# apache/datafusion-comet

Hardware: NVIDIA H100
Metric: rows/sec on TPC-H Q1 filter+agg (higher is better)
Workload: dtype i128

## Files before the change

### datafusion-comet_b200/comet_b200/native.py

```python
import ctypes as C
import os

import pyarrow as pa

_PKG = os.path.dirname(os.path.dirname(os.path.abspath(__file__)))
_LIB_PATH = os.path.join(_PKG, "libcomet_b200.so")
_lib = None


class CometB200Error(RuntimeError):
    def __init__(self, code, error_class, message):
        super().__init__(f"[{code}{' ' + error_class if error_class else ''}] {message}")
        self.code, self.error_class, self.message = code, error_class, message


class Unsupported(CometB200Error):
    """The plan is outside the GPU hot path; a caller keeps its CPU path (CB200_ERR_UNSUPPORTED)."""


class _Error(C.Structure):
    _fields_ = [("code", C.c_int32), ("error_class", C.c_char * 64), ("message", C.c_char * 952)]


class ArrowSchema(C.Structure):
    pass


class ArrowArray(C.Structure):
    pass


ArrowSchema._fields_ = [("format", C.c_char_p), ("name", C.c_char_p), ("metadata", C.c_char_p), ("flags", C.c_int64),
                        ("n_children", C.c_int64), ("children", C.POINTER(C.POINTER(ArrowSchema))),
                        ("dictionary", C.POINTER(ArrowSchema)), ("release", C.c_void_p), ("private_data", C.c_void_p)]
ArrowArray._fields_ = [("length", C.c_int64), ("null_count", C.c_int64), ("offset", C.c_int64), ("n_buffers", C.c_int64),
                       ("n_children", C.c_int64), ("buffers", C.POINTER(C.c_void_p)),
                       ("children", C.POINTER(C.POINTER(ArrowArray))), ("dictionary", C.POINTER(ArrowArray)),
                       ("release", C.c_void_p), ("private_data", C.c_void_p)]


class ArrowArrayStream(C.Structure):
    _fields_ = [("get_schema", C.c_void_p), ("get_next", C.c_void_p), ("get_last_error", C.c_void_p),
                ("release", C.c_void_p), ("private_data", C.c_void_p)]


class DeviceColumn(C.Structure):
    _fields_ = [("type_id", C.c_int32), ("precision", C.c_int32), ("scale", C.c_int32), ("value_width", C.c_int32),
                ("values", C.c_void_p), ("validity", C.c_void_p), ("host_values", C.c_void_p),
                ("host_validity_bytes", C.c_void_p), ("validity_bytes", C.c_void_p), ("bool_bytes", C.c_void_p),
                ("n_dict", C.c_int32), ("pad", C.c_int32)]


class Stats(C.Structure):
    _fields_ = [("kernel_launches", C.c_int64), ("pipeline_launches", C.c_int64), ("pipeline_ms", C.c_double),
                ("pipeline_rows", C.c_int64), ("h2d_bytes", C.c_int64), ("d2h_bytes", C.c_int64),
                ("scan_pruned_row_groups", C.c_int64), ("scan_pruned_rows", C.c_int64), ("agg_strategies", C.c_int64)]
AGG_DENSE, AGG_TABLE, AGG_STREAM, AGG_MIGRATED = 1, 2, 4, 8


EXPORTED = ["cb200_comm_unique_id", "cb200_comm_create", "cb200_comm_destroy", "cb200_comm_rank", "cb200_comm_world", "cb200_nccl_info", "cb200_exchange",
            "cb200_exchange_layout", "cb200_comm_allgather_small", "cb200_plan_stats", "cb200_register_memory_file", "cb200_parquet_describe", "cb200_table_add_column_bytes", "cb200_plan_dict_value", "cb200_plan_partition_starts", "cb200_compile_plan_assume", "cb200_version", "cb200_supports", "cb200_create_plan", "cb200_plan_num_columns", "cb200_execute",
            "cb200_release", "cb200_table_create", "cb200_table_add_column", "cb200_plan_bind_table",
            "cb200_table_release", "cb200_execute_device", "cb200_plan_kernel_launches", "cb200_compile_plan",
            "cb200_plan_kernel_source"]


def lib():
    global _lib
    if _lib is None:
        if not os.path.exists(_LIB_PATH):
            raise ImportError(f"{_LIB_PATH} is missing: build it with `python -c 'import __graft_entry__ as g; g.build()'` "
                              "(make -C datafusion-comet_b200/csrc).  comet_b200 has no CPU fallback.")
        l = C.CDLL(_LIB_PATH)
        l.cb200_version.restype = C.c_char_p
        l.cb200_supports.argtypes = [C.c_char_p, C.c_size_t, C.POINTER(_Error)]
        l.cb200_create_plan.restype = C.c_void_p
        l.cb200_create_plan.argtypes = [C.c_char_p, C.c_size_t, C.c_char_p, C.c_size_t, C.POINTER(C.c_void_p), C.c_int32,
                                        C.c_int32, C.c_int32, C.c_int32, C.c_int32, C.POINTER(_Error)]
        l.cb200_plan_num_columns.argtypes = [C.c_void_p]
        l.cb200_execute.restype = C.c_int64
        l.cb200_execute.argtypes = [C.c_void_p, C.POINTER(ArrowArray), C.POINTER(ArrowSchema), C.c_int32, C.POINTER(_Error)]
        l.cb200_release.argtypes = [C.c_void_p]
        l.cb200_table_create.restype = C.c_void_p
        l.cb200_table_create.argtypes = [C.c_int64]
        l.cb200_table_add_column.argtypes = [C.c_void_p, C.c_int32, C.c_int32, C.c_int32, C.c_int32, C.c_void_p, C.c_void_p,
                                             C.c_int64, C.POINTER(C.c_char_p), C.c_int32, C.POINTER(_Error)]
        l.cb200_plan_bind_table.argtypes = [C.c_void_p, C.c_int32, C.c_void_p, C.POINTER(_Error)]
        l.cb200_table_release.argtypes = [C.c_void_p]
        l.cb200_execute_device.restype = C.c_int64
        l.cb200_execute_device.argtypes = [C.c_void_p, C.POINTER(DeviceColumn), C.c_int32, C.POINTER(_Error)]
        l.cb200_plan_kernel_launches.restype = C.c_int64
        l.cb200_plan_kernel_launches.argtypes = [C.c_void_p]
        l.cb200_plan_stats.argtypes = [C.c_void_p, C.POINTER(Stats)]
        l.cb200_compile_plan.argtypes = [C.c_char_p, C.c_size_t, C.c_char_p, C.c_size_t, C.POINTER(_Error)]
        l.cb200_plan_kernel_source.argtypes = [C.c_char_p, C.c_size_t, C.c_int32, C.c_char_p, C.c_size_t, C.POINTER(_Error)]
        _lib = l
    return _lib


def _raise(err):
    cls = Unsupported if err.code == 1 else CometB200Error
    raise cls(err.code, err.error_class.decode(), err.message.decode(errors="replace"))


def version():
    return lib().cb200_version().decode()


def supports(op_bytes):
    err = _Error()
    ok = lib().cb200_supports(op_bytes, len(op_bytes), C.byref(err))
    return bool(ok), err.message.decode(errors="replace")


def compile_plan(op_bytes):
    err = _Error()
    buf = C.create_string_buffer(4096)
    n = lib().cb200_compile_plan(op_bytes, len(op_bytes), buf, 4096, C.byref(err))
    if n < 0:
        _raise(err)
    return [k for k in buf.value.decode().split(",") if k]


def compile_plan_assume(op_bytes, assume_bits, source_index=-1):
    err = _Error()
    arr = (C.c_int32 * len(assume_bits))(*assume_bits)
    cap = 1 << 20
    buf = C.create_string_buffer(cap)
    lib().cb200_compile_plan_assume.argtypes = [C.c_char_p, C.c_size_t, C.POINTER(C.c_int32), C.c_int32, C.c_int32, C.c_char_p, C.c_size_t, C.POINTER(_Error)]
    n = lib().cb200_compile_plan_assume(op_bytes, len(op_bytes), arr, len(assume_bits), source_index, buf, cap, C.byref(err))
    if n < 0:
        _raise(err)
    return buf.value.decode()


_MEMFILES = {}


def register_memory_file(name, buf):
# ... 288 lines not shown
```

### datafusion-comet_b200/csrc/abi.cpp

```cpp
#include "../../include/comet_b200.h"

#include "abi_internal.h"
#include "parquet_kernels.h"
#include "exec.h"
#include "jit.h"
#include "plan.h"
#include "proto_wire.h"

#include <cstring>
#include <functional>
#include <map>
#include <mutex>

using namespace cb200;

namespace {

struct CtxRes {
    cudaStream_t stream;
    int* d_err;
    int* h_err;
    cudaEvent_t ev0, ev1;
};
std::mutex g_pool_mu;
std::map<int, std::vector<CtxRes>> g_pool;

void parse_config(const uint8_t* cfg, size_t len, ExecContext& ctx) {
    if (!cfg || !len) return;
    PbReader r(cfg, len);
    while (r.next()) {
        if (r.field != 1 || r.wire != 2) { r.skip(); continue; }
        PbReader e = r.sub();
        std::string k, v;
        while (e.next()) {
            if (e.field == 1) k = e.bytes();
            else if (e.field == 2) v = e.bytes();
            else e.skip();
        }
        if (k == "spark.comet.b200.chunkRows") ctx.chunk_rows = std::max<int64_t>(1024, atoll(v.c_str()));
        else if (k == "spark.comet.batchSize") ctx.batch_size = atoi(v.c_str());
        else if (k == "spark.comet.b200.streamAgg.minRows") ctx.stream_agg_min_rows = atoll(v.c_str());
        else if (k == "spark.comet.b200.streamAgg.maxRatio") ctx.stream_agg_max_ratio = atof(v.c_str());
        else if (k == "spark.comet.b200.hashThreads") { int t = atoi(v.c_str()); if (t == 256 || t == 512 || t == 768 || t == 960) ctx.hash_threads = t; }
    }
}

void start(cb200_plan* p) {
    if (p->started) return;
    TraceSpan ts("plan.start");
    ExecContext& ctx = p->ctx;
    cuda_check(cudaSetDevice(ctx.device), "cudaSetDevice");
    {
        struct DevInfo { int major = 0, minor = 0, sms = 0; bool known = false; };
        static DevInfo info[64];
        static std::mutex info_mu;
        std::lock_guard<std::mutex> lk(info_mu);
        if (ctx.device < 0 || ctx.device >= 64) throw ExecError(CB200_ERR_CUDA, "", "device ordinal out of range");
        DevInfo& di = info[ctx.device];
        if (!di.known) {
            cuda_check(cudaDeviceGetAttribute(&di.major, cudaDevAttrComputeCapabilityMajor, ctx.device), "cudaDeviceGetAttribute");
            cuda_check(cudaDeviceGetAttribute(&di.minor, cudaDevAttrComputeCapabilityMinor, ctx.device), "cudaDeviceGetAttribute");
            cuda_check(cudaDeviceGetAttribute(&di.sms, cudaDevAttrMultiProcessorCount, ctx.device), "cudaDeviceGetAttribute");
            di.known = true;
        }
        if (di.major != 9 || di.minor != 0) throw ExecError(CB200_ERR_CUDA, "", "comet_b200 kernels are built for sm_90a; device is sm_" + std::to_string(di.major * 10 + di.minor));
        ctx.num_sms = di.sms;
    }
    {
        std::lock_guard<std::mutex> lk(g_pool_mu);
        auto& fl = g_pool[ctx.device];
        if (!fl.empty()) {
            CtxRes r = fl.back();
            fl.pop_back();
            ctx.stream = r.stream; ctx.d_err = r.d_err; ctx.h_err = r.h_err; ctx.ev0 = r.ev0; ctx.ev1 = r.ev1;
        }
    }
    if (!ctx.stream) {
        cuda_check(cudaStreamCreateWithFlags(&ctx.stream, cudaStreamNonBlocking), "cudaStreamCreate");
        cudaMemPool_t pool;
        if (cudaDeviceGetDefaultMemPool(&pool, ctx.device) == cudaSuccess) {
            unsigned long long keep = ~0ull;
            cudaMemPoolSetAttribute(pool, cudaMemPoolAttrReleaseThreshold, &keep);
        }
        cuda_check(cudaMalloc((void**)&ctx.d_err, 64), "cudaMalloc err");
        cuda_check(cudaMallocHost((void**)&ctx.h_err, 64), "cudaMallocHost err");
        cuda_check(cudaEventCreate(&ctx.ev0), "cudaEventCreate");
        cuda_check(cudaEventCreate(&ctx.ev1), "cudaEventCreate");
    }
    cuda_check(cudaMemsetAsync(ctx.d_err, 0, 64, ctx.stream), "memset err");
    set_alloc_stream(ctx.stream);
    p->root = build_exec(p->op, &ctx, &p->inputs);
    p->started = true;
}

DType dtype_from_ids(int type_id, int precision, int scale) {
    if (type_id < 0 || type_id > 13) throw Unsupported("type id " + std::to_string(type_id));
    DType d;
    d.id = (TypeId)type_id;
    d.precision = precision;
    d.scale = scale;
    return d;
}

}

extern "C" {

const char* cb200_version(void) { return "comet_b200 0.1.0 (sm_90a; reference apache/datafusion-comet 1.1.0 @2699f59b)"; }

int cb200_supports(const uint8_t* op_proto, size_t op_len, cb200_error* why) {
    return cb200_guarded(why, [&]() -> int {
        OperatorP op = decode_plan(op_proto, op_len);
        plan_kernels_for_build(op);
        return 1;
    }, 0);
}

cb200_plan* cb200_create_plan(const uint8_t* op_proto, size_t op_len, const uint8_t* cfg_proto, size_t cfg_len, struct ArrowArrayStream** inputs,
                              int32_t n_inputs, int32_t partition, int32_t partition_count, int32_t batch_size, int32_t device_ordinal, cb200_error* err) {
    TraceSpan ts("create_plan");
    return cb200_guarded(err, [&]() -> cb200_plan* {
        auto p = std::unique_ptr<cb200_plan>(new cb200_plan());
        p->op = decode_plan(op_proto, op_len);
        p->ctx.device = device_ordinal;
        if (batch_size > 0) p->ctx.batch_size = batch_size;
        parse_config(cfg_proto, cfg_len, p->ctx);
        p->partition = partition;
        p->partition_count = partition_count;
        for (int i = 0; i < n_inputs; i++) {
            p->inputs.streams.push_back(inputs ? inputs[i] : nullptr);
            p->inputs.tables.push_back(nullptr);
        }
        return p.release();
    }, (cb200_plan*)nullptr);
}

int32_t cb200_plan_num_columns(cb200_plan* plan) { return plan ? (int32_t)plan->op->schema.size() : -1; }

static int64_t execute_common(cb200_plan* plan, cb200_error* err, const std::function<void(Batch&)>& sink) {
    TraceSpan ts("execute");
    return cb200_guarded(err, [&]() -> int64_t {
        if (!plan) throw PlanError("null plan handle");
        if (plan->finished) return -1;
        start(plan);
        cuda_check(cudaSetDevice(plan->ctx.device), "cudaSetDevice");
        set_alloc_stream(plan->ctx.stream);
        Batch b;
        if (!plan->root->next(b)) { plan->finished = true; return -1; }
        plan->last = std::move(b);
        sink(plan->last);
        return plan->last.n_rows;
    }, (int64_t)-2);
}

int64_t cb200_execute(cb200_plan* plan, struct ArrowArray* out_arrays, struct ArrowSchema* out_schemas, int32_t n_cols, cb200_error* err) {
    if (plan && plan->export_pending) {
        TraceSpan ts("execute(slice)");
        return cb200_guarded(err, [&]() -> int64_t {
            cuda_check(cudaSetDevice(plan->ctx.device), "cudaSetDevice");
            set_alloc_stream(plan->ctx.stream);
            const int64_t n = std::min<int64_t>(std::max(plan->ctx.batch_size, 1), plan->last.n_rows - plan->export_pos);
            export_batch(plan->last, &plan->ctx, out_arrays, out_schemas, n_cols, plan->export_pos, n);
            plan->export_pos += n;
            plan->export_pending = plan->export_pos < plan->last.n_rows;
            return n;
        }, (int64_t)-2);
    }
    int64_t first = 0;
    const int64_t rc = execute_common(plan, err, [&](Batch& b) {
        const bool whole = plan->op->kind == OpKind::ShuffleWriter;
        first = whole ? b.n_rows : std::min<int64_t>(std::max(plan->ctx.batch_size, 1), b.n_rows);
        export_batch(b, &plan->ctx, out_arrays, out_schemas, n_cols, 0, first);
        plan->export_pos = first;
        plan->export_pending = first < b.n_rows;
    });
    return rc < 0 ? rc : first;
}

int64_t cb200_execute_device(cb200_plan* plan, cb200_device_column* cols, int32_t n_cols, cb200_error* err) {
    if (plan && plan->export_pending)
        return cb200_guarded(err, [&]() -> int64_t { throw PlanError("cb200_execute_device: the current batch is still being handed out by cb200_execute"); }, (int64_t)-2);
    return execute_common(plan, err, [&](Batch& b) {
        if ((int)b.cols.size() != n_cols) throw PlanError("execute_device: plan produces " + std::to_string(b.cols.size()) + " columns");
        for (int i = 0; i < n_cols; i++) {
            Column& c = b.cols[(size_t)i];
            cb200_device_column& o = cols[i];
            memset(&o, 0, sizeof(o));
            o.type_id = (int)c.type.id;
            o.precision = c.type.precision;
            o.scale = c.type.scale;
            o.value_width = c.type.id == TypeId::Bool ? 1 : c.type.arrow_width();
            if (c.on_host) {
                o.host_values = c.h_data.data();
                o.host_validity_bytes = c.h_valid.empty() ? nullptr : c.h_valid.data();
            } else {
                o.values = c.data ? c.data->ptr : nullptr;
                o.validity = c.validity ? c.validity->ptr : nullptr;
                o.validity_bytes = c.valid_bytes ? c.valid_bytes->ptr : nullptr;
                o.bool_bytes = c.bool_bytes ? c.bool_bytes->ptr : nullptr;
                if (c.is_dict) { o.n_dict = (int)c.dict->values.size(); o.value_width = phys_bytes(c.phys == Phys::I32 ? Phys::Dict32 : c.phys); }
            }
        }
    });
}

void cb200_release(cb200_plan* plan) {
    if (!plan) return;
    TraceSpan ts("release");
    try {
        if (plan->started) cudaSetDevice(plan->ctx.device);
        plan->last = Batch();
        plan->root.reset();
        if (plan->ctx.stream) {
            cudaStreamSynchronize(plan->ctx.stream);
            std::lock_guard<std::mutex> lk(g_pool_mu);
            g_pool[plan->ctx.device].push_back(CtxRes{plan->ctx.stream, plan->ctx.d_err, plan->ctx.h_err, plan->ctx.ev0, plan->ctx.ev1});
        }
        for (auto* s : plan->inputs.streams) if (s && s->release) s->release(s);
    } catch (...) {
    }
    delete plan;
}

cb200_table* cb200_table_create(int64_t n_rows) {
    auto* t = new cb200_table();
    t->t = std::make_shared<DeviceTable>();
    t->t->n_rows = n_rows;
    return t;
}

int cb200_table_add_column(cb200_table* t, int32_t type_id, int32_t precision, int32_t scale, int32_t value_width, const void* dev_values,
                           const void* dev_validity, int64_t null_count, const char* const* dict_values, int32_t n_dict, cb200_error* err) {
    return cb200_guarded(err, [&]() -> int {
        if (!t) throw PlanError("null table handle");
        Column c;
        c.type = dtype_from_ids(type_id, precision, scale);
        size_t n = (size_t)t->t->n_rows;
        if (n_dict > 0) {
            if (!c.type.is_string()) throw PlanError("dictionary values on a non-string column");
            c.is_dict = true;
            c.dict = std::make_shared<Dictionary>();
            for (int i = 0; i < n_dict; i++) c.dict->values.push_back(dict_values[i]);
            c.phys = value_width == 1 ? Phys::I8 : value_width == 2 ? Phys::I16 : Phys::I32;
            if (value_width != 1 && value_width != 2 && value_width != 4) throw PlanError("dictionary codes must be 1, 2 or 4 bytes wide");
        } else if (c.type.is_string()) {
            throw Unsupported("device string columns must be dictionary-encoded");
        } else if (c.type.is_decimal() && value_width == 8) {
            if (c.type.precision > 18) throw PlanError("8-byte decimals need precision <= 18");
            c.phys = Phys::I64;
        } else {
            int w = c.type.arrow_width();
            if (value_width != w) throw PlanError("value_width " + std::to_string(value_width) + " does not match " + c.type.str());
            switch (c.type.id) {
            case TypeId::Bool: c.phys = Phys::Bitmap; break;
            case TypeId::Int8: c.phys = Phys::I8; break;
            case TypeId::Int16: c.phys = Phys::I16; break;
            case TypeId::Int32: case TypeId::Date: c.phys = Phys::I32; break;
            case TypeId::Float32: c.phys = Phys::F32; break;
            case TypeId::Float64: c.phys = Phys::F64; break;
            case TypeId::Decimal: c.phys = Phys::I128; break;
            default: c.phys = Phys::I64; break;
            }
        }
        if (((uintptr_t)dev_values & 15) || ((uintptr_t)dev_validity & 15)) throw PlanError("device buffers must be 16-byte aligned");
        size_t bytes = value_width == 0 ? (n + 7) / 8 : n * (size_t)value_width;
        c.data = std::make_shared<DeviceBuf>((void*)dev_values, bytes);
        if (dev_validity && null_count != 0) c.validity = std::make_shared<DeviceBuf>((void*)dev_validity, (n + 7) / 8);
        c.null_count = null_count;
        t->t->cols.push_back(c);
        return 0;
    }, -1);
}

const char* cb200_plan_dict_value(cb200_plan* plan, int32_t col, int32_t i, int32_t* len) {
    if (!plan || col < 0 || col >= (int)plan->last.cols.size()) return nullptr;
    const Column& c = plan->last.cols[(size_t)col];
    if (!c.is_dict || !c.dict || i < 0 || i >= (int)c.dict->values.size()) return nullptr;
    if (len) *len = (int32_t)c.dict->values[(size_t)i].size();
    return c.dict->values[(size_t)i].data();
}

int cb200_table_add_column_bytes(cb200_table* t, int32_t type_id, int32_t precision, int32_t scale, int32_t value_width, const void* dev_values,
                                 const void* dev_validity_bytes, const char* const* dict_values, int32_t n_dict, cb200_error* err) {
    return cb200_guarded(err, [&]() -> int {
        if (!t) throw PlanError("null table handle");
        size_t n = (size_t)t->t->n_rows;
        bool is_bool = type_id == (int)TypeId::Bool;
        int rc = cb200_table_add_column(t, type_id, precision, scale, is_bool ? 0 : value_width, is_bool ? nullptr : dev_values, nullptr, 0, dict_values, n_dict, err);
        if (rc != 0) throw PlanError(err ? err->message : "add_column failed");
        Column& c = t->t->cols.back();
        if (is_bool) {
            if (value_width != 1) throw PlanError("byte-per-row booleans need value_width 1");
            c.data = nullptr;
            c.bool_bytes = std::make_shared<DeviceBuf>((void*)dev_values, n);
            t->t->needs_packing = true;
        }
        if (dev_validity_bytes) {
            c.valid_bytes = std::make_shared<DeviceBuf>((void*)dev_validity_bytes, n);
            c.null_count = -1;
            t->t->needs_packing = true;
        }
        return 0;
    }, -1);
}

int cb200_plan_bind_table(cb200_plan* plan, int32_t input_index, cb200_table* t, cb200_error* err) {
    return cb200_guarded(err, [&]() -> int {
        if (!plan || !t) throw PlanError("null handle");
        if (plan->started) throw PlanError("tables must be bound before the first execute");
        if (input_index < 0 || input_index >= (int)plan->inputs.tables.size()) throw PlanError("input index out of range");
        plan->inputs.tables[(size_t)input_index] = t->t;
        return 0;
    }, -1);
}

void cb200_table_release(cb200_table* t) { delete t; }

int32_t cb200_plan_partition_starts(cb200_plan* plan, int64_t* starts, int32_t cap) {
    if (!plan) return -1;
    const auto& ps = plan->ctx.partition_starts;
    for (size_t i = 0; i < ps.size() && (int32_t)i < cap; i++) starts[i] = ps[i];
    return (int32_t)ps.size();
}

int64_t cb200_plan_kernel_launches(cb200_plan* plan) { return plan ? plan->ctx.kernel_launches : -1; }

int64_t cb200_release_cached_memory(int32_t device_ordinal) {
    try {
        if (cudaSetDevice(device_ordinal) != cudaSuccess) return 0;
        return (int64_t)release_cached_device_memory();
    } catch (...) { return 0; }
}

int cb200_plan_stats(cb200_plan* plan, cb200_stats* out) {
    if (!plan || !out) return -1;
    const ExecContext& c = plan->ctx;
    out->kernel_launches = c.kernel_launches;
    out->pipeline_launches = c.pipeline_launches;
    out->pipeline_ms = c.pipeline_ms;
    out->pipeline_rows = c.pipeline_rows;
    out->h2d_bytes = c.h2d_bytes;
    out->d2h_bytes = c.d2h_bytes;
    out->scan_pruned_row_groups = c.scan_pruned_row_groups;
    out->scan_pruned_rows = c.scan_pruned_rows;
    out->agg_strategies = c.agg_strategies;
    return 0;
}

int cb200_compile_plan(const uint8_t* op_proto, size_t op_len, char* keys_out, size_t keys_cap, cb200_error* err) {
    return cb200_guarded(err, [&]() -> int {
        OperatorP op = decode_plan(op_proto, op_len);
        auto ks = plan_kernels_for_build(op);
        std::string keys;
        for (auto& g : ks) {
            jit_get(g, false);
            keys += (keys.empty() ? "" : ",") + g.key;
        }
        if (keys_out && keys_cap) snprintf(keys_out, keys_cap, "%s", keys.c_str());
        return (int)ks.size();
    }, -1);
}

int cb200_compile_plan_assume(const uint8_t* op_proto, size_t op_len, const int32_t* assume_bits, int32_t n_assume, int32_t source_index,
                              char* src_out, size_t src_cap, cb200_error* err) {
    return cb200_guarded(err, [&]() -> int {
        OperatorP op = decode_plan(op_proto, op_len);
        std::vector<int> as(assume_bits, assume_bits + n_assume);
        auto ks = plan_kernels_for_build(op, as);
        for (auto& g : ks) jit_get(g, false);
        if (src_out && src_cap && source_index >= 0 && source_index < (int)ks.size()) snprintf(src_out, src_cap, "%s", ks[(size_t)source_index].source.c_str());
        return (int)ks.size();
    }, -1);
}

int cb200_register_memory_file(const char* name, const void* data, size_t len) {
    if (!name) return -1;
    register_memory_file(name, (const uint8_t*)data, len);
    return 0;
}

int64_t cb200_snappy_decompress(const uint8_t* comp, size_t comp_len, uint8_t* out, size_t uncompressed_len, int32_t device_ordinal, int32_t* path_taken,
                                cb200_error* err) {
    return cb200_guarded(err, [&]() -> int64_t {
        if (!comp || (!out && uncompressed_len) || comp_len >= ((size_t)1 << 31) || uncompressed_len >= ((size_t)1 << 31)) throw PlanError("cb200_snappy_decompress: bad arguments");
        cuda_check(cudaSetDevice(device_ordinal), "cudaSetDevice");
        cudaStream_t st = nullptr;
        set_alloc_stream(st);
        DeviceBuf dcomp(comp_len + 64), dout(uncompressed_len + 64), dpage(sizeof(PqPage)), derr(64);
        const int n_segs = (int)((uncompressed_len + PQ_SNAPPY_SEG - 1) / PQ_SNAPPY_SEG);
        DeviceBuf dck((size_t)(n_segs + 1) * 4);
        PqPage pg;
        memset(&pg, 0, sizeof(pg));
        pg.body = (unsigned char*)dout.ptr;
        pg.body_bytes = (int)uncompressed_len;
        pg.comp = (const unsigned char*)dcomp.ptr;
        pg.comp_bytes = (int)comp_len;
        pg.seg_base = 0;
        pg.n_segs = n_segs;
        cuda_check(cudaMemsetAsync(dcomp.ptr, 0, comp_len + 64, st), "memset");
        cuda_check(cudaMemcpyAsync(dcomp.ptr, comp, comp_len, cudaMemcpyHostToDevice, st), "copy in");
        cuda_check(cudaMemcpyAsync(dpage.ptr, &pg, sizeof(pg), cudaMemcpyHostToDevice, st), "copy page");
        cuda_check(cudaMemsetAsync(derr.ptr, 0, 64, st), "memset err");
        launch_pq_snappy_segmented((PqPage*)dpage.ptr, 1, (unsigned*)dck.ptr, n_segs, (int*)derr.ptr, st);
        int e = 0;
        cuda_check(cudaMemcpyAsync(&e, derr.ptr, 4, cudaMemcpyDeviceToHost, st), "read err");
        cuda_check(cudaMemcpyAsync(&pg, dpage.ptr, sizeof(pg), cudaMemcpyDeviceToHost, st), "read page");
        if (uncompressed_len) cuda_check(cudaMemcpyAsync(out, dout.ptr, uncompressed_len, cudaMemcpyDeviceToHost, st), "copy out");
        cuda_check(cudaStreamSynchronize(st), "sync");
        if (path_taken) *path_taken = (pg.flags & PQ_PAGE_SN_SERIAL) ? 1 : 0;
        if (e) throw ExecError(14, "", "malformed Snappy stream (device error flags " + std::to_string(e) + ")");
        return (int64_t)uncompressed_len;
    }, (int64_t)-1);
}

int cb200_parquet_describe(const char* path, char* out, size_t cap, cb200_error* err) {
    return cb200_guarded(err, [&]() -> int {
        std::string s = describe_parquet(path ? path : "");
        if (out && cap) snprintf(out, cap, "%s", s.c_str());
        return (int)s.size();
    }, -1);
}

int cb200_plan_kernel_source(const uint8_t* op_proto, size_t op_len, int32_t index, char* out, size_t cap, cb200_error* err) {
    return cb200_guarded(err, [&]() -> int {
        OperatorP op = decode_plan(op_proto, op_len);
        auto ks = plan_kernels_for_build(op);
        if (index < 0 || index >= (int)ks.size()) throw PlanError("kernel index out of range");
        const std::string& s = ks[(size_t)index].source;
// ... 7 lines not shown
```

### datafusion-comet_b200/csrc/agg.cpp

```cpp
#include "exec_internal.h"
#include "../../include/comet_b200.h"

#include "aot_kernels.h"
#include "ranges.h"

#include <algorithm>
#include <mutex>

namespace cb200 {

static std::mutex g_profile_mu;
static std::map<std::string, std::vector<int>> g_range_profile;

namespace {

enum class Strategy { Undecided, Dense, Table, Stream };
enum Level { SAFE = 0, TYPE = 1, TIGHT = 2 };
constexpr int DENSE_MAX_GROUPS = 64;

constexpr int GK = CB_GID_RANGES;
struct HashFlags { int w[CB_HFLAG_WORDS]; };
int64_t round_ids(int64_t n) { return (n + GK - 1) / GK * GK; }

using ValueMasks = uint64_t[CB_MAX_COLS * 2];

uint64_t identity_word(int kind) { return kind == W_MIN ? 0x7fffffffffffffffull : kind == W_MAX ? 0x8000000000000000ull : 0; }

std::vector<int> decode_gid(int g, const std::vector<int>& cards) {
    std::vector<int> code(cards.size());
    for (int k = (int)cards.size() - 1; k >= 0; k--) { code[(size_t)k] = g % cards[(size_t)k]; g /= cards[(size_t)k]; }
    return code;
}

int grid_for(const ExecContext* ctx, int n_tiles) { return std::max(1, std::min(ctx->num_sms, n_tiles)); }

struct Kernel {
    PipelineSpec spec;
    GeneratedKernel g;
    std::shared_ptr<CompiledModule> mod;
};

void launch_named(ExecContext* ctx, const Kernel& k, const char* name, dim3 grid, dim3 block, void** args) {
    cuda_check(cudaLaunchKernel((const void*)k.mod->kernel(name), grid, block, args, 0, ctx->stream), name);
    ctx->kernel_launches++;
}

struct DenseState {
    std::vector<int> cards;
    std::vector<bool> has_null;
    DeviceBufP totals, spill, partials;
    int groups = 0;

    void regroup(ExecContext* ctx, int n_words, const std::vector<int>& word_kinds, const std::vector<int>& new_cards) {
        int new_groups = 1;
        for (int c : new_cards) new_groups *= c;
        std::vector<uint64_t> oldt((size_t)groups * n_words * 2), newt((size_t)new_groups * n_words * 2);
        cuda_check(cudaMemcpy(oldt.data(), totals->ptr, oldt.size() * 8, cudaMemcpyDeviceToHost), "regroup D2H");
        for (size_t i = 0; i < (size_t)new_groups * n_words; i++) newt[i * 2] = identity_word(word_kinds[i % (size_t)n_words]);
        for (int g = 0; g < groups; g++) {
            const std::vector<int> code = decode_gid(g, cards);
            int ng = 0, mul = 1;
            for (int k = (int)cards.size() - 1; k >= 0; k--) {
                int cd = code[(size_t)k];
                if (has_null[(size_t)k] && cd == cards[(size_t)k] - 1) cd = new_cards[(size_t)k] - 1;
                ng += cd * mul;
                mul *= new_cards[(size_t)k];
            }
            memcpy(&newt[(size_t)ng * n_words * 2], &oldt[(size_t)g * n_words * 2], (size_t)n_words * 16);
        }
        totals = std::make_shared<DeviceBuf>(newt.size() * 8);
        cuda_check(cudaMemcpyAsync(totals->ptr, newt.data(), newt.size() * 8, cudaMemcpyHostToDevice, ctx->stream), "regroup H2D");
        cuda_check(cudaStreamSynchronize(ctx->stream), "regroup sync");
        groups = new_groups;
    }

    void finalize(ExecContext* ctx, const Kernel& last, cb::FinParams fp, bool ungrouped, const std::vector<DType>& schema,
                  const std::vector<DictionaryP>& key_dicts, Batch& out) const {
        TraceSpan ts("agg.finalize");
        const GeneratedKernel& g = last.g;
        const int ng = groups;
        fp.totals = (cb::u64*)totals->ptr;
        fp.n_groups = ng;
        std::vector<size_t> off_v, off_n;
        size_t total_bytes = 0;
        auto take = [&](size_t n) { size_t o = total_bytes; total_bytes += (n + 15) / 16 * 16; return o; };
        for (size_t i = 0; i < g.out_cols.size(); i++) { off_v.push_back(take((size_t)ng * g.out_bytes[i])); off_n.push_back(take((size_t)ng)); }
        size_t off_present = take((size_t)ng);
        auto dbuf = std::make_shared<DeviceBuf>(total_bytes);
        for (size_t i = 0; i < g.out_cols.size(); i++) {
            fp.out[i] = (cb::u8*)dbuf->ptr + off_v[i];
            fp.outv[i] = (cb::u8*)dbuf->ptr + off_n[i];
        }
        fp.present = (cb::u8*)dbuf->ptr + off_present;
        void* args[] = {&fp};
        cuda_check(cudaLaunchKernel((const void*)last.mod->kernel(g.finalize_entry), dim3((ng + 127) / 128), dim3(128), args, 0, ctx->stream), "finalize launch");
        ctx->kernel_launches++;
        std::vector<uint8_t> hbuf(total_bytes);
        cuda_check(cudaMemcpyAsync(hbuf.data(), dbuf->ptr, total_bytes, cudaMemcpyDeviceToHost, ctx->stream), "agg results D2H"); ctx->d2h_bytes += (int64_t)(total_bytes);
        ctx->check_device_errors();
        const uint8_t* pres = hbuf.data() + off_present;
        std::vector<int> rows;
        for (int gi = 0; gi < ng; gi++) if (ungrouped || pres[(size_t)gi]) rows.push_back(gi);
        out.n_rows = (int64_t)rows.size();
        out.cols.clear();
        for (size_t k = 0; k < key_dicts.size(); k++) {
            Column c;
            c.type = schema[k];
            c.on_host = true;
            bool any_null = false;
            std::vector<int> codes;
            for (int gi : rows) codes.push_back(decode_gid(gi, cards)[k]);
            c.h_valid.assign(rows.size(), 1);
            const bool is_bool = c.type.id == TypeId::Bool;
            if (!is_bool) c.h_offsets.push_back(0);
            for (size_t r = 0; r < rows.size(); r++) {
                const bool isnull = has_null[k] && codes[r] == cards[k] - 1;
                if (isnull) { c.h_valid[r] = 0; any_null = true; }
                if (is_bool) c.h_data.push_back(isnull ? 0 : (uint8_t)codes[r]);
                else {
                    if (!isnull) { const std::string& s = key_dicts[k]->values.at((size_t)codes[r]); c.h_data.insert(c.h_data.end(), s.begin(), s.end()); }
                    c.h_offsets.push_back((int32_t)c.h_data.size());
                }
            }
            if (!any_null) c.h_valid.clear();
            out.cols.push_back(c);
        }
        for (size_t i = 0; i < g.out_cols.size(); i++) {
            Column c;
            c.type = g.out_cols[i].type;
            c.on_host = true;
            int w = g.out_bytes[i];
            const uint8_t* all = hbuf.data() + off_v[i];
            const uint8_t* allv = hbuf.data() + off_n[i];
            c.h_data.resize(rows.size() * w);
            c.h_valid.resize(rows.size());
            bool any_null = false;
            for (size_t r = 0; r < rows.size(); r++) {
                memcpy(&c.h_data[r * w], &all[(size_t)rows[r] * w], (size_t)w);
                c.h_valid[r] = allv[(size_t)rows[r]];
                if (!c.h_valid[r]) any_null = true;
            }
            if (!any_null) c.h_valid.clear();
            out.cols.push_back(c);
        }
    }
};

struct IdRows {
    DeviceBufP hkey_of_gid, htotals, hflags;
    int64_t max_groups = 0;

    void ensure_flags(ExecContext* ctx) {
        if (hflags) return;
        hflags = std::make_shared<DeviceBuf>(sizeof(HashFlags));
        cuda_check(cudaMemsetAsync(hflags->ptr, 0, sizeof(HashFlags), ctx->stream), "memset hash flags");
    }
    void write_flags(ExecContext* ctx, const HashFlags& hf) {
        cuda_check(cudaMemcpyAsync(hflags->ptr, &hf, sizeof(hf), cudaMemcpyHostToDevice, ctx->stream), "write hash flags");
        cuda_check(cudaStreamSynchronize(ctx->stream), "flags sync");
    }
    int64_t read_flags(ExecContext* ctx, HashFlags& hf, int64_t cnt[GK]) {
        memset(&hf, 0, sizeof(hf));
        if (hflags) {
            cuda_check(cudaMemcpyAsync(&hf, hflags->ptr, sizeof(hf), cudaMemcpyDeviceToHost, ctx->stream), "read hash flags"); ctx->d2h_bytes += (int64_t)sizeof(hf);
            cuda_check(cudaStreamSynchronize(ctx->stream), "hash flags sync");
        }
        const int64_t R = max_groups / GK;
        int64_t total = 0;
        bool overshoot = false;
        for (int r = 0; r < GK; r++) {
            if (hf.w[CB_HFLAG_CTR + r] > R || hf.w[CB_HFLAG_CTR + r] < 0) overshoot = true;
            cnt[r] = std::min<int64_t>(std::max(hf.w[CB_HFLAG_CTR + r], 0), R);
            if (hf.w[CB_HFLAG_CTR + r] < 0) cnt[r] = R;
            total += cnt[r];
        }
        if (overshoot && hflags) {
            for (int r = 0; r < GK; r++) hf.w[CB_HFLAG_CTR + r] = (int)cnt[r];
            write_flags(ctx, hf);
        }
        return total;
    }
    static void init_totals(ExecContext* ctx, const Kernel& k, cb::u64* totals, int64_t first, int64_t n) {
        if (n <= 0) return;
        const int n_words = k.g.n_words;
        if (std::none_of(k.g.word_kinds.begin(), k.g.word_kinds.end(), identity_word)) {
            cuda_check(cudaMemsetAsync(totals + first * n_words * 2, 0, (size_t)n * n_words * 16, ctx->stream), "memset totals");
        } else {
            long long f = first, nn = n;
            void* a1[] = {&totals, &f, &nn};
            launch_named(ctx, k, "cb_hash_init", dim3((unsigned)((n + 255) / 256)), dim3(256), a1);
        }
    }
    void grow(ExecContext* ctx, const Kernel& k, const int64_t cnt[GK], int64_t nm, bool zero_fill) {
        cudaStream_t st = ctx->stream;
        const int n_words = k.g.n_words, key_words = k.g.key_words;
        if (nm + 2 >= INT32_MAX) throw ExecError(16, "", "more than 2^31 groups in one partition; lower spark.comet.b200.chunkRows");
        const int64_t Ro = max_groups / GK, Rn = nm / GK;
        auto ntot = std::make_shared<DeviceBuf>((size_t)(nm + 2) * n_words * 16);
        auto nkog = std::make_shared<DeviceBuf>((size_t)nm * 8 * key_words + 16);
        cb::u64* tp = (cb::u64*)ntot->ptr;
        if (zero_fill) init_totals(ctx, k, tp, 0, nm + 2);
        else if (!htotals) init_totals(ctx, k, tp, nm, 2);
        if (htotals) {
            for (int r = 0; r < GK; r++) {
                if (cnt[r] <= 0) continue;
                cuda_check(cudaMemcpyAsync(tp + (size_t)r * Rn * n_words * 2, (cb::u64*)htotals->ptr + (size_t)r * Ro * n_words * 2, (size_t)cnt[r] * n_words * 16,
                                           cudaMemcpyDeviceToDevice, st), "copy totals");
                cuda_check(cudaMemcpyAsync((cb::u64*)nkog->ptr + (size_t)r * Rn * key_words, (cb::u64*)hkey_of_gid->ptr + (size_t)r * Ro * key_words,
                                           (size_t)cnt[r] * 8 * key_words, cudaMemcpyDeviceToDevice, st), "copy group keys");
            }
            cuda_check(cudaMemcpyAsync(tp + (size_t)nm * n_words * 2, (cb::u64*)htotals->ptr + (size_t)max_groups * n_words * 2, (size_t)2 * n_words * 16,
                                       cudaMemcpyDeviceToDevice, st), "copy reserved groups");
        }
        cuda_check(cudaStreamSynchronize(st), "table growth");
        htotals = ntot; hkey_of_gid = nkog; max_groups = nm;
    }

    void finalize(ExecContext* ctx, const Kernel& last, cb::FinParams fp, const std::vector<DictionaryP>& key_dicts, Batch& out) {
        TraceSpan ts("agg.finalize_hash");
        const GeneratedKernel& g = last.g;
        HashFlags hfl;
        int64_t cnt[GK];
        const int64_t ng = read_flags(ctx, hfl, cnt);
        const int* flags = hfl.w;
        const int64_t n_out = ng + ((flags[0] & CB_HF_SENTINEL) ? 1 : 0) + ((flags[0] & CB_HF_NULL_GROUP) ? 1 : 0);
        fp.totals = (cb::u64*)htotals->ptr;
        fp.hkeys = (const cb::u64*)hkey_of_gid->ptr;
        fp.sentinel_used = flags[0] & CB_HF_SENTINEL;
        fp.null_group_used = (flags[0] & CB_HF_NULL_GROUP) ? 1 : 0;
        fp.n_hash_groups = (int)ng;
        fp.max_groups = (int)max_groups;
        fp.gid_range = (int)(max_groups / GK);
        int64_t run = 0;
        for (int r = 0; r < GK; r++) { fp.gid_prefix[r] = (int)run; run += cnt[r]; }
        fp.gid_prefix[GK] = (int)run;
        fp.n_groups = (int)n_out;
        if (g.out_cols.size() > CB_MAX_OUT) throw Unsupported("too many output columns");
        out.n_rows = n_out;
        out.cols.clear();
        std::vector<DeviceBufP> vbytes;
        size_t rows_alloc = (size_t)std::max<int64_t>(n_out, 1);
        for (size_t i = 0; i < g.out_cols.size(); i++) {
            Column c;
            c.type = g.out_cols[i].type;
            c.phys = c.type.id == TypeId::Bool ? Phys::I8 : (c.type.is_string() ? Phys::I32 : phys_of(c.type));
            c.data = std::make_shared<DeviceBuf>(rows_alloc * g.out_bytes[i]);
            vbytes.push_back(std::make_shared<DeviceBuf>(rows_alloc));
            fp.out[i] = (cb::u8*)c.data->ptr;
            fp.outv[i] = (cb::u8*)vbytes.back()->ptr;
            if ((int)i < g.n_key_cols && c.type.is_string()) { c.is_dict = true; c.dict = key_dicts[i]; }
            out.cols.push_back(c);
        }
        auto present = std::make_shared<DeviceBuf>(rows_alloc);
        fp.present = (cb::u8*)present->ptr;
        if (n_out > 0) {
            void* args[] = {&fp};
            launch_named(ctx, last, g.finalize_entry.c_str(), dim3((unsigned)((n_out + 127) / 128)), dim3(128), args);
            for (size_t i = 0; i < out.cols.size(); i++) {
                Column& c = out.cols[i];
                c.valid_bytes = vbytes[i];
                c.validity = std::make_shared<DeviceBuf>((size_t)(n_out + 31) / 32 * 4 + 8);
                launch_bytes_to_bitmap((const unsigned char*)vbytes[i]->ptr, n_out, (uint32_t*)c.validity->ptr, ctx->stream);
                ctx->kernel_launches++;
                c.null_count = -1;
                if (c.type.id == TypeId::Bool) c.bool_bytes = c.data;
            }
        }
        ctx->check_device_errors();
    }
};

struct KeyTable {
    DeviceBufP hkeys;
    int64_t hcap = 0;

    void ensure(ExecContext* ctx, const Kernel& k, IdRows& rows, int64_t incoming, int64_t remaining, int64_t rows_scanned, bool merging) {
        cudaStream_t st = ctx->stream;
        rows.ensure_flags(ctx);
        HashFlags hf;
        int64_t cnt[GK];
        const int64_t cur = rows.read_flags(ctx, hf, cnt);
        const int64_t need = cur + incoming;
        if (need + 2 >= INT32_MAX) throw ExecError(16, "", "more than 2^31 groups in one partition; lower spark.comet.b200.chunkRows");
        bool relocated = false;
        if (need > rows.max_groups) {
            int64_t nm = std::max<int64_t>(need, rows.max_groups + rows.max_groups / 4);
            if (remaining > 0 && rows_scanned == 0 && merging) {
                nm = std::max(nm, need + remaining);
            }
            if (remaining > 0 && rows_scanned > 0 && cur > 0) {
                const double ratio = std::min(1.0, 1.3 * (double)cur / (double)rows_scanned);
                const int64_t est = cur + incoming + (int64_t)(ratio * (double)remaining);
                nm = std::max(nm, std::min<int64_t>(est, cur + incoming + remaining));
            }
            if (nm + 2 + GK >= INT32_MAX) nm = INT32_MAX - 3 - GK;
            relocated = cur > 0;
            rows.grow(ctx, k, cnt, round_ids(nm), true);
        }
        int64_t cap = std::max<int64_t>(hcap, 1 << 16);
        while (cap < 2 * std::max(need, rows.max_groups)) cap <<= 1;
        if (cap != hcap || relocated) {
            auto nkeys = cap != hcap ? std::make_shared<DeviceBuf>((size_t)cap * 16) : hkeys;
            cuda_check(cudaMemsetAsync(nkeys->ptr, 0xff, (size_t)cap * 16, st), "memset key slots");
            if (cur > 0) {
                const cb::u64* kog = (const cb::u64*)rows.hkey_of_gid->ptr;
                int rr = (int)(rows.max_groups / GK);
                const int* ctr = (const int*)rows.hflags->ptr + CB_HFLAG_CTR;
                cb::u64* kp = (cb::u64*)nkeys->ptr;
                cb::u32 mask = (cb::u32)(cap - 1);
                void* a2[] = {&kog, &rr, &ctr, &kp, &mask};
                launch_named(ctx, k, "cb_hash_rehash", dim3((unsigned)((rows.max_groups + 255) / 256)), dim3(256), a2);
                cuda_check(cudaStreamSynchronize(st), "rehash");
            }
            hkeys = nkeys; hcap = cap;
        }
    }
};

struct StreamState {
    double ratio = 1.0;
    DeviceBufP reserved_snap;

    void ensure_rows(ExecContext* ctx, const Kernel& k, IdRows& rows, const int64_t cnt[GK], int64_t want_groups) {
        rows.ensure_flags(ctx);
        if (rows.htotals && want_groups <= rows.max_groups) return;
        rows.grow(ctx, k, cnt, round_ids(std::max<int64_t>(want_groups, rows.max_groups + rows.max_groups / 2)), false);
    }
    void snapshot_reserved(ExecContext* ctx, const IdRows& rows, int n_words, bool restore) {
        const size_t bytes = (size_t)2 * n_words * 16;
        if (!reserved_snap || reserved_snap->bytes < bytes) reserved_snap = std::make_shared<DeviceBuf>(bytes);
        cb::u64* tail = (cb::u64*)rows.htotals->ptr + (size_t)rows.max_groups * n_words * 2;
        if (restore) cuda_check(cudaMemcpyAsync(tail, reserved_snap->ptr, bytes, cudaMemcpyDeviceToDevice, ctx->stream), "restore reserved groups");
        else cuda_check(cudaMemcpyAsync(reserved_snap->ptr, tail, bytes, cudaMemcpyDeviceToDevice, ctx->stream), "snapshot reserved groups");
    }
};

struct AggNode : FusedBase {
    std::vector<ExprP> keys;
    std::vector<AggExpr> aggs;
    std::vector<std::vector<int>> state_cols;
    AggMode mode = AggMode::Partial;
    bool ungrouped = false;
    bool emitted = false;
    std::vector<Batch> outq;
    size_t outq_pos = 0;
    std::vector<int> assume_bits;

    std::vector<bool> key_has_null;
    std::vector<DictionaryP> key_dicts;
    struct DevDict { StringDictDev d; std::vector<DeviceBufP> bufs; int host_known = 0; };
    std::vector<std::shared_ptr<DevDict>> dev_dicts;

    int n_words = 0, key_words = 1;
    std::vector<int> word_kinds;
    Kernel last;
    bool have_totals() const { return last.mod != nullptr; }

    Strategy strategy = Strategy::Undecided;
    DenseState dense;
    KeyTable table;
    IdRows rows;

    std::vector<int> observed_bits;
    int64_t rows_scanned = 0;
    std::string profile_key;
    DeviceBufP vmask;
    StreamState stream;

    int assume_for(int child_col, Level lv) const {
        const DType& t = child->schema[(size_t)child_col];
        if (!t.is_decimal() || lv == SAFE || mode != AggMode::Partial) return 0;
        int k = r_bitlen(r_prec_max(t.precision));
        if ((size_t)child_col < assume_bits.size() && assume_bits[(size_t)child_col] > 0) k = std::min(k, assume_bits[(size_t)child_col]);
        if (lv == TIGHT && !observed_bits.empty() && observed_bits[(size_t)child_col] >= 0) k = std::min(k, observed_bits[(size_t)child_col] + 2);
        return std::min(k, 126);
    }

    PipelineSpec make_spec(const Batch* b, Strategy st, int n_groups, Level lv = TYPE) const {
        const bool hash = st == Strategy::Table || st == Strategy::Stream;
        PipelineSpec s;
        s.cols = stage_cols(b);
        for (auto& c : s.cols) c.assume_bits = assume_for(c.src_index, lv);
        s.predicates = to_slots(predicates, slot_of);
        s.sink = SinkKind::Agg;
        s.mode = mode;
        s.ungrouped = ungrouped;
        s.hash = hash;
        s.keys = to_slots(keys, slot_of);
        for (size_t k = 0; k < keys.size(); k++) s.key_nullable.push_back(b ? key_has_null[k] : false);
        for (auto& a : aggs) {
            AggExpr c = a;
            if (mode == AggMode::Partial) {
                c.children = to_slots(a.children, slot_of);
                if (a.filter) c.filter = to_slots({a.filter}, slot_of)[0];
            }
            s.aggs.push_back(c);
        }
        for (auto& sc : state_cols) {
            std::vector<int> v;
            for (int ci : sc) v.push_back(slot_of.at(ci));
            s.state_slots.push_back(v);
        }
        if (hash) {
            s.threads = ctx->hash_threads;
            s.tile = 2 * ctx->hash_threads;
            s.stream = st == Strategy::Stream;
        }
        GeneratedKernel probe = generate_pipeline(s);
        size_t acc = (!ungrouped && !hash) ? (size_t)std::max(n_groups, 1) * probe.n_words * s.threads * 8 : 0;
        while (acc + 2 * (size_t)probe.stage_bytes + 1024 > SMEM_BUDGET && s.threads > 32) {
            s.threads /= 2;
            acc /= 2;
        }
        if (acc + 2 * (size_t)probe.stage_bytes + 1024 > SMEM_BUDGET)
            throw Unsupported("too many groups x aggregates for the thread-private accumulators of the dense path");
        s.stages = (int)std::max<size_t>(2, std::min<size_t>(6, (SMEM_BUDGET - 1024 - acc) / (size_t)probe.stage_bytes));
        return s;
    }

    std::vector<PipelineSpec> build_specs() const override {
        bool hash = false;
        for (auto& k : keys) if (!k->type.is_string() && k->type.id != TypeId::Bool) hash = true;
        std::vector<PipelineSpec> out{make_spec(nullptr, hash ? Strategy::Table : Strategy::Dense, ungrouped ? 1 : 6)};
        if (hash && mode == AggMode::Partial) out.push_back(make_spec(nullptr, Strategy::Stream, 6));
        return out;
    }

    Kernel compile(const PipelineSpec& spec) {
        Kernel k{spec, generate_pipeline(spec), nullptr};
        k.mod = jit_get(k.g, true);
        if (have_totals() && (k.g.n_words != n_words || k.g.word_kinds != word_kinds)) throw ExecError(15, "", "internal: accumulator layout changed between launches");
        if (have_totals() && k.g.key_words != key_words) throw ExecError(15, "", "internal: group key packing changed between launches");
        n_words = k.g.n_words;
        word_kinds = k.g.word_kinds;
        key_words = k.g.key_words;
        return k;
    }

    void clear_vmask() {
        if (!vmask) vmask = std::make_shared<DeviceBuf>(CB_MAX_COLS * 16);
        cuda_check(cudaMemsetAsync(vmask->ptr, 0, CB_MAX_COLS * 16, ctx->stream), "memset vmask");
    }
    void copy_vmask(ValueMasks& masks) {
        cuda_check(cudaMemcpyAsync(masks, vmask->ptr, sizeof(ValueMasks), cudaMemcpyDeviceToHost, ctx->stream), "read value masks"); ctx->d2h_bytes += (int64_t)(sizeof(ValueMasks));
    }
    static std::vector<int> mask_bits(const PipelineSpec& spec, const ValueMasks& masks) {
        std::vector<int> seen(spec.cols.size(), -1);
        for (size_t i = 0; i < spec.cols.size(); i++) {
            if (!spec.cols[i].type.is_decimal()) continue;
            uint64_t lo = masks[2 * i], hi = masks[2 * i + 1];
            seen[i] = hi ? 64 + r_bitlen(hi) : r_bitlen(lo);
        }
        return seen;
    }
    void observe(const std::vector<int>& seen) {
        for (size_t i = 0; i < seen.size(); i++)
            if (seen[i] >= 0) observed_bits[(size_t)used_cols[i]] = std::max(observed_bits[(size_t)used_cols[i]], seen[i]);
    }

    int prepare_key(Batch& b, size_t k) {
        int ci = keys[k]->index;
        Column& c = b.cols[ci];
        if (c.type.id == TypeId::Bool) return 2;
        if (!c.type.is_string()) return -1;
        if (c.is_dict) {
            key_dicts[k] = c.dict;
            return (int)c.dict->values.size();
        }
        if (!dev_dicts[k]) {
            auto dd = std::make_shared<DevDict>();
            const int64_t cap = 1 << 16;
            const int max_codes = 4096;
            const int64_t bytes_cap = 1 << 20;
            auto alloc = [&](size_t n) { auto bfr = std::make_shared<DeviceBuf>(n); cuda_check(cudaMemsetAsync(bfr->ptr, 0, bfr->bytes, ctx->stream), "memset dict"); dd->bufs.push_back(bfr); return bfr->ptr; };
            dd->d.tags = (unsigned long long*)alloc((size_t)cap * 8);
            dd->d.slot_code = (int*)alloc((size_t)cap * 4);
            dd->d.capacity = cap;
            dd->d.n_codes = (int*)alloc(64);
            dd->d.bytes_used = (unsigned long long*)((char*)dd->d.n_codes + 16);
            dd->d.err = (int*)((char*)dd->d.n_codes + 32);
            dd->d.max_codes = max_codes;
            dd->d.code_off = (long long*)alloc((size_t)max_codes * 8);
            dd->d.code_len = (int*)alloc((size_t)max_codes * 4);
            dd->d.bytes = (unsigned char*)alloc((size_t)bytes_cap);
            dd->d.bytes_cap = bytes_cap;
            dev_dicts[k] = dd;
            key_dicts[k] = std::make_shared<Dictionary>();
        }
        DevDict& dd = *dev_dicts[k];
        if (!c.offsets || !c.chars) throw Unsupported("string key column without offsets/chars buffers");
        auto row_slot = std::make_shared<DeviceBuf>((size_t)b.n_rows * 4);
        auto codes = std::make_shared<DeviceBuf>((size_t)b.n_rows * 4);
        launch_dict_encode(dd.d, (const int*)c.offsets->ptr, (const unsigned char*)c.chars->ptr, c.validity ? (const unsigned char*)c.validity->ptr : nullptr,
                           b.n_rows, (int*)row_slot->ptr, (int*)codes->ptr, ctx->stream);
        ctx->kernel_launches += 2;
        int hdr[12];
        cuda_check(cudaMemcpyAsync(hdr, dd.d.n_codes, sizeof(hdr), cudaMemcpyDeviceToHost, ctx->stream), "dict header");
        cuda_check(cudaStreamSynchronize(ctx->stream), "dict encode");
        int n_codes = hdr[0], derr = hdr[8];
        if (derr & CB_DICT_FULL) throw Unsupported("plain Utf8 group key with more distinct values than the device dictionary holds (dictionary-encode the column)");
        if (derr & CB_DICT_COLLISION) throw ExecError(14, "", "64-bit hash collision between distinct group key strings");
        if (n_codes > dd.host_known) {
            std::vector<long long> off((size_t)n_codes);
            std::vector<int> len((size_t)n_codes);
            cuda_check(cudaMemcpy(off.data(), dd.d.code_off, (size_t)n_codes * 8, cudaMemcpyDeviceToHost), "dict offsets");
            cuda_check(cudaMemcpy(len.data(), dd.d.code_len, (size_t)n_codes * 4, cudaMemcpyDeviceToHost), "dict lengths");
            for (int i = dd.host_known; i < n_codes; i++) {
                std::string s((size_t)len[(size_t)i], '\0');
                if (len[(size_t)i]) cuda_check(cudaMemcpy(&s[0], dd.d.bytes + off[(size_t)i], (size_t)len[(size_t)i], cudaMemcpyDeviceToHost), "dict bytes");
                key_dicts[k]->values.push_back(s);
            }
            dd.host_known = n_codes;
        }
        c.data = codes;
        c.phys = Phys::I32;
        c.is_dict = true;
        c.dict = key_dicts[k];
        return n_codes;
    }

    void consume(Batch& b) {
        std::vector<int> nc(keys.size());
        std::vector<bool> hn(keys.size());
        for (size_t k = 0; k < keys.size(); k++) {
            int card = prepare_key(b, k);
            const Column& c = b.cols[keys[k]->index];
            hn[k] = key_has_null[k] || c.validity != nullptr;
            nc[k] = card < 0 ? -1 : std::max(card, 1) + (hn[k] ? 1 : 0);
            if (!dense.cards.empty() && nc[k] >= 0) nc[k] = std::max(nc[k], dense.cards[k]);
        }
        bool densifiable = true;
        for (int c : nc) if (c < 0) densifiable = false;
        int n_groups = 1;
        if (densifiable) for (int c : nc) { n_groups *= c; if (n_groups > 1 << 20) break; }
        const bool needs_hash = !ungrouped && (!densifiable || n_groups > DENSE_MAX_GROUPS);
        key_has_null = hn;
        if (observed_bits.empty()) observed_bits.assign(child->schema.size(), -1);
        if (strategy == Strategy::Undecided || (strategy == Strategy::Dense && needs_hash)) {
            if (strategy == Strategy::Dense) {
                leave_dense();
                ctx->agg_strategies |= CB200_AGG_MIGRATED;
            }
            strategy = !needs_hash ? Strategy::Dense : sample_stream(b) ? Strategy::Stream : Strategy::Table;
            ctx->agg_strategies |= strategy == Strategy::Dense ? CB200_AGG_DENSE : strategy == Strategy::Stream ? CB200_AGG_STREAM : CB200_AGG_TABLE;
        }
        if (strategy == Strategy::Dense) consume_dense(b, nc, n_groups);
        else if (strategy == Strategy::Table) consume_table(b);
        else consume_stream(b);
    }

    void consume_dense(Batch& b, const std::vector<int>& nc, int n_groups) {
        if (have_totals() && nc != dense.cards) {
            if (n_words == 0) throw ExecError(15, "", "internal: regroup before layout");
            dense.regroup(ctx, n_words, word_kinds, nc);
        }
        dense.cards = nc;
        dense.has_null = key_has_null;
        const int64_t SAMPLE = 1 << 20;
        bool have_obs = false;
        for (int ci : used_cols) if (child->schema[(size_t)ci].is_decimal() && observed_bits[(size_t)ci] >= 0) have_obs = true;
        if (mode == AggMode::Partial && !have_obs && b.n_rows > 2 * SAMPLE) {
            profile_key = pipeline_signature(make_spec(&b, Strategy::Dense, n_groups, SAFE));
            std::lock_guard<std::mutex> lk(g_profile_mu);
            auto it = g_range_profile.find(profile_key);
            if (it != g_range_profile.end() && it->second.size() == observed_bits.size()) {
                observed_bits = it->second;
                for (int ci : used_cols) if (child->schema[(size_t)ci].is_decimal() && observed_bits[(size_t)ci] >= 0) have_obs = true;
            }
        }
        if (mode != AggMode::Partial) {
            run_range(b, 0, b.n_rows, n_groups, SAFE);
        } else if (!have_obs && b.n_rows > 2 * SAMPLE) {
            run_range(b, 0, SAMPLE, n_groups, TYPE);
            run_range(b, SAMPLE, b.n_rows, n_groups, TIGHT);
        } else {
            run_range(b, 0, b.n_rows, n_groups, have_obs ? TIGHT : TYPE);
        }
        if (!profile_key.empty()) {
            std::lock_guard<std::mutex> lk(g_profile_mu);
            if (g_range_profile.size() > 256) g_range_profile.clear();
            g_range_profile[profile_key] = observed_bits;
        }
    }

    void leave_dense() {
        if (mode == AggMode::Final) throw Unsupported("group cardinality grew past the dense path mid-stream in a Final aggregate");
        if (have_totals()) {
            Batch early;
            dense.finalize(ctx, last, certified_params(), ungrouped, schema, key_dicts, early);
            if (early.n_rows > 0) outq.push_back(std::move(early));
        }
        last = Kernel();
        dense = DenseState();
        n_words = 0; word_kinds.clear(); rows_scanned = 0;
    }

    void run_range(Batch& b, int64_t row0, int64_t row1, int n_groups, Level lv) {
        TraceSpan tsr("agg.run_range");
        while (true) {
            Kernel k;
            {
                TraceSpan ts("agg.codegen+jit");
                k = compile(make_spec(&b, Strategy::Dense, n_groups, lv));
            }
            const int64_t max_rows = (int64_t)ctx->num_sms * k.g.threads * (1ll << CB_RPT_LOG2) / 1024 * 1024;
            int64_t r0 = row0;
            while (r0 < row1 && launch_one(b, r0, std::min(row1, r0 + max_rows), n_groups, k)) r0 += max_rows;
            if (r0 >= row1) return;
            if (lv == SAFE) throw ExecError(15, "", "internal: value-mask validation failed without assumptions");
            lv = lv == TIGHT ? TYPE : SAFE;
            row0 = r0;
        }
    }

    bool launch_one(Batch& b, int64_t r0, int64_t r1, int n_groups, const Kernel& k) {
        cudaStream_t st = ctx->stream;
        size_t tot_bytes = (size_t)n_groups * n_words * 16;
        if (!have_totals()) {
            dense.totals = std::make_shared<DeviceBuf>(tot_bytes);
            dense.groups = n_groups;
        }
        if (!dense.spill || dense.spill->bytes < tot_bytes) {
            dense.spill = std::make_shared<DeviceBuf>(tot_bytes);
            cuda_check(cudaMemsetAsync(dense.spill->ptr, 0, dense.spill->bytes, st), "memset spill");
        }
        clear_vmask();
        cb::PipeParams p;
        fill_inputs(p, b, k.g.tile, r0, r1);
        int grid = grid_for(ctx, p.n_tiles);
        size_t part_bytes = (size_t)grid * tot_bytes;
        if (!dense.partials || dense.partials->bytes < part_bytes) dense.partials = std::make_shared<DeviceBuf>(part_bytes);
        p.n_groups = n_groups;
        for (size_t i = 0; i < dense.cards.size() && i < CB_MAX_KEYS; i++) p.key_card[i] = dense.cards[i];
        p.partials = (cb::u8*)dense.partials->ptr;
        p.spill = (cb::u64*)dense.spill->ptr;
        p.vmask = (cb::u64*)vmask->ptr;
        launch(k.mod->kernel(k.g.entry), dim3(grid), dim3(k.g.threads + 32), k.g.dyn_smem(n_groups), &p);
        ctx->pipeline_rows += r1 - r0;
        ValueMasks masks;
        copy_vmask(masks);
        ctx->check_device_errors();
        const std::vector<int> seen = mask_bits(k.spec, masks);
        bool ok = true;
        for (size_t i = 0; i < seen.size(); i++)
            if (k.spec.cols[i].assume_bits > 0 && seen[i] > k.spec.cols[i].assume_bits) ok = false;
        observe(seen);
        if (!ok) {
            cuda_check(cudaMemsetAsync(dense.spill->ptr, 0, dense.spill->bytes, st), "memset spill");
            return false;
        }
        rows_scanned += r1 - r0;
        cb::FinParams fp;
        memset(&fp, 0, sizeof(fp));
        fp.partials = (const cb::u64*)dense.partials->ptr;
        fp.spill = (cb::u64*)dense.spill->ptr;
        fp.totals = (cb::u64*)dense.totals->ptr;
        fp.n_ctas = grid;
        fp.n_groups = n_groups;
        fp.first = have_totals() ? 0 : 1;
        fp.err = ctx->d_err;
        int total_words = n_groups * n_words;
        void* args[] = {&fp};
        cuda_check(cudaLaunchKernel((const void*)k.mod->kernel("cb_fold"), dim3((total_words + 127) / 128), dim3(128), args, 0, st), "fold launch");
        ctx->kernel_launches++;
        last = k;
        return true;
    }

    void launch_id_rows(Batch& b, int64_t r0, int64_t r1, const Kernel& k, bool with_table) {
        clear_vmask();
        cb::PipeParams p;
        fill_inputs(p, b, k.g.tile, r0, r1);
        p.hkeys = with_table ? (cb::u64*)table.hkeys->ptr : nullptr;
        p.hkey_of_gid = (cb::u64*)rows.hkey_of_gid->ptr;
        p.htotals = (cb::u64*)rows.htotals->ptr;
        p.hmask = with_table ? (cb::u32)(table.hcap - 1) : 0;
        p.max_groups = (cb::i32)rows.max_groups;
        p.hflags = (cb::i32*)rows.hflags->ptr;
        p.vmask = (cb::u64*)vmask->ptr;
        p.n_groups = 2;
        launch(k.mod->kernel(k.g.entry), dim3(grid_for(ctx, p.n_tiles)), dim3(k.g.threads + 32), k.g.dyn_smem(0), &p);
    }

    void consume_table(Batch& b) {
        const Kernel k = compile(make_spec(&b, Strategy::Table, 2, SAFE));
        {
            TraceSpan ts("hash.ensure_table");
            table.ensure(ctx, k, rows, b.n_rows, child->rows_hint(), rows_scanned, mode != AggMode::Partial);
        }
        launch_id_rows(b, 0, b.n_rows, k, true);
        ctx->pipeline_rows += b.n_rows;
        ValueMasks masks;
        int flags[8];
        copy_vmask(masks);
        cuda_check(cudaMemcpyAsync(flags, rows.hflags->ptr, sizeof(flags), cudaMemcpyDeviceToHost, ctx->stream), "read hash flags"); ctx->d2h_bytes += (int64_t)(sizeof(flags));
        ctx->check_device_errors();
        if (flags[0] & CB_HF_FULL) throw ExecError(15, "", "internal: hash table full");
        if (flags[0] & CB_HF_WIDE_KEY) throw Unsupported("decimal(p > 18) group key whose value does not fit 64 bits");
        observe(mask_bits(k.spec, masks));
        rows_scanned += b.n_rows;
        last = k;
    }

    int64_t stream_launch(Batch& b, int64_t r0, int64_t r1, const Kernel& k, HashFlags& hf, int64_t cnt[GK]) {
        launch_id_rows(b, r0, r1, k, false);
        ValueMasks masks;
        copy_vmask(masks);
        ctx->check_device_errors();
        const int64_t total = rows.read_flags(ctx, hf, cnt);
        if (hf.w[0] & CB_HF_WIDE_KEY) throw Unsupported("decimal(p > 18) group key whose value does not fit 64 bits");
        if (!(hf.w[0] & CB_HF_FULL)) observe(mask_bits(k.spec, masks));
        return total;
    }
    bool sample_stream(Batch& b) {
        if (mode != AggMode::Partial || ctx->stream_agg_min_rows < 0) return false;
        if (b.n_rows + std::max<int64_t>(child->rows_hint(), 0) < ctx->stream_agg_min_rows || b.n_rows == 0) return false;
        const Kernel k = compile(make_spec(&b, Strategy::Stream, 2, SAFE));
        const int64_t sample = std::min<int64_t>(b.n_rows, 1 << 20);
        HashFlags hf;
        int64_t cnt[GK] = {0};
        stream.ensure_rows(ctx, k, rows, cnt, 2 * sample + 4096);
        const int64_t runs = stream_launch(b, 0, sample, k, hf, cnt);
        stream.ratio = (hf.w[0] & CB_HF_FULL) ? 1.0 : (double)runs / (double)sample;
        memset(&hf, 0, sizeof(hf));
        rows.write_flags(ctx, hf);
        IdRows::init_totals(ctx, k, (cb::u64*)rows.htotals->ptr, rows.max_groups, 2);
        if (stream.ratio <= ctx->stream_agg_max_ratio) return true;
        rows = IdRows();
        n_words = 0; word_kinds.clear();
        return false;
    }
    void consume_stream(Batch& b) {
        const Kernel k = compile(make_spec(&b, Strategy::Stream, 2, SAFE));
        HashFlags before, hf;
        int64_t cnt0[GK], cnt[GK];
        const int64_t cur = rows.read_flags(ctx, before, cnt0);
        const int64_t remaining = std::max<int64_t>(child->rows_hint(), 0);
        int64_t want = cur + std::min<int64_t>(b.n_rows, (int64_t)(1.25 * stream.ratio * (double)b.n_rows) + 65536);
        if (!rows.htotals || want > rows.max_groups) want += std::min<int64_t>(remaining, (int64_t)(1.25 * stream.ratio * (double)remaining));
        int64_t handed_out;
        while (true) {
            {
                TraceSpan ts("stream.ensure_rows");
                stream.ensure_rows(ctx, k, rows, cnt0, want);
            }
            stream.snapshot_reserved(ctx, rows, n_words, false);
            handed_out = stream_launch(b, 0, b.n_rows, k, hf, cnt);
            if (!(hf.w[0] & CB_HF_FULL)) break;
            stream.snapshot_reserved(ctx, rows, n_words, true);
            for (int r = 0; r < GK; r++) before.w[CB_HFLAG_CTR + r] = (int)cnt0[r];
            rows.write_flags(ctx, before);
            want = cur + b.n_rows + GK;
        }
        ctx->pipeline_rows += b.n_rows;
        if (b.n_rows > 0) stream.ratio = std::max(stream.ratio, (double)(handed_out - cur) / (double)b.n_rows);
        rows_scanned += b.n_rows;
        last = k;
    }

    u128r certificate(size_t ai) const {
        const AggExpr& a = aggs[ai];
        if (!(a.kind == AggKind::Sum || a.kind == AggKind::Avg) || !a.datatype.is_decimal()) return 0;
        std::vector<u128r> bounds(child->schema.size(), RSAT);
        for (size_t c = 0; c < bounds.size(); c++)
            if (child->schema[c].is_decimal() && !observed_bits.empty())
                bounds[c] = observed_bits[c] < 0 ? 0 : (observed_bits[c] >= 127 ? RSAT : (u128r)1 << observed_bits[c]);
        if (mode == AggMode::Partial) return expr_maxabs(*a.children[0], bounds);
        return bounds[(size_t)state_cols[ai][0]];
    }
    cb::FinParams certified_params() const {
        cb::FinParams fp;
        memset(&fp, 0, sizeof(fp));
        fp.err = ctx->d_err;
        for (size_t ai = 0; ai < aggs.size() && ai < CB_MAX_OUT; ai++) {
            const u128r b = certificate(ai);
            fp.cert_b[ai][0] = b >= RSAT ? ~0ull : (uint64_t)b;
            fp.cert_b[ai][1] = b >= RSAT ? ~0ull : (uint64_t)(b >> 64);
            const bool direct = mode != AggMode::Partial || aggs[ai].children[0]->kind == ExprKind::Bound;
            if (b < RSAT && b != 0 && direct) fp.cert_b[ai][1] |= 1ull << 63;
        }
        return fp;
    }

    bool next(Batch& out) override {
        if (!emitted) aggregate_input();
        if (outq_pos >= outq.size()) return false;
        out = std::move(outq[outq_pos++]);
        return true;
    }
    void aggregate_input() {
        if (keys.size() > CB_MAX_KEYS) throw Unsupported("more than 4 group keys");
        key_has_null.assign(keys.size(), false);
        key_dicts.assign(keys.size(), nullptr);
        dev_dicts.assign(keys.size(), nullptr);
        Batch in;
        while (child->next(in)) {
            if (in.n_rows == 0) continue;
            consume(in);
            ctx->check_device_errors();
        }
        emitted = true;
        if (!have_totals()) {
            if (!ungrouped) return;
            last = compile(make_spec(nullptr, Strategy::Dense, 1));
            std::vector<uint64_t> id((size_t)n_words * 2, 0);
            for (int w = 0; w < n_words; w++) id[(size_t)w * 2] = identity_word(word_kinds[(size_t)w]);
            dense.totals = std::make_shared<DeviceBuf>(id.size() * 8);
            cuda_check(cudaMemcpyAsync(dense.totals->ptr, id.data(), id.size() * 8, cudaMemcpyHostToDevice, ctx->stream), "identity totals");
            cuda_check(cudaStreamSynchronize(ctx->stream), "identity totals sync");
            dense.groups = 1;
        }
        Batch result;
        if (strategy == Strategy::Table || strategy == Strategy::Stream) rows.finalize(ctx, last, certified_params(), key_dicts, result);
        else dense.finalize(ctx, last, certified_params(), ungrouped, schema, key_dicts, result);
        outq.push_back(std::move(result));
    }
};

}

ExecNodeP make_agg_node(const OperatorP& agg_op, const ExecNodeP& src, const std::vector<ExprP>& preds, const std::vector<ExprP>& cols, ExecContext* ctx,
                        const std::vector<int>& assume_bits) {
    auto n = std::make_shared<AggNode>();
    n->ctx = ctx;
    n->child = src;
    n->schema = agg_op->schema;
    n->predicates = preds;
    n->mode = agg_op->mode;
    n->ungrouped = agg_op->grouping.empty();
    n->assume_bits = assume_bits;
    std::vector<ExprP> roots = preds;
    for (auto& gexp : agg_op->grouping) {
        ExprP k = substitute(gexp, cols);
        if (k->kind != ExprKind::Bound) throw Unsupported("computed group keys (only plain column keys are fused)");
        n->keys.push_back(k);
        roots.push_back(k);
    }
    size_t state_at = agg_op->grouping.size();
    for (auto& a : agg_op->aggs) {
        AggExpr c = a;
        if (agg_op->mode == AggMode::Partial) {
            for (auto& ch : c.children) { ch = substitute(ch, cols); roots.push_back(ch); }
            if (c.filter) { c.filter = substitute(c.filter, cols); roots.push_back(c.filter); }
        } else {
            std::vector<int> sc;
            for (size_t k = 0; k < agg_state_types(a).size(); k++) {
                ExprP e = cols.at(state_at++);
                if (e->kind != ExprKind::Bound) throw Unsupported("final aggregate over computed state columns");
                sc.push_back(e->index);
                roots.push_back(e);
            }
            n->state_cols.push_back(sc);
        }
        n->aggs.push_back(c);
    }
    n->assign_slots(roots);
    if (n->used_cols.empty()) {
        int best = -1, best_w = 1 << 30;
        for (size_t c = 0; c < src->schema.size(); c++) {
            const DType& t = src->schema[c];
            if (t.is_string()) continue;
            int w = std::max(1, phys_bytes(phys_of(t)));
            if (w < best_w) { best = (int)c; best_w = w; }
        }
        if (best < 0) throw Unsupported("COUNT(*) over a child with only string columns");
        n->used_cols.push_back(best);
        n->slot_of[best] = 0;
    }
    return n;
}

}
```

### datafusion-comet_b200/csrc/codegen.cpp

```cpp
#include "codegen.h"
#include <mutex>
#include "ranges.h"

#include <climits>
#include <cstring>
#include <functional>
#include <sstream>

namespace cb200 {

int phys_bytes(Phys p) {
    switch (p) {
    case Phys::Bitmap: return 0;
    case Phys::I8: return 1;
    case Phys::I16: return 2;
    case Phys::I32: case Phys::F32: case Phys::Dict32: return 4;
    case Phys::I64: case Phys::F64: return 8;
    case Phys::I128: return 16;
    }
    return 0;
}

size_t GeneratedKernel::dyn_smem(int n_groups) const {
    size_t s = (entry == "cb_pipeline_agg" ? 128 : 256) + (size_t)stages * stage_bytes;
// ... 702 lines not shown
    GeneratedKernel g = generate_pipeline_uncached(spec);
    std::lock_guard<std::mutex> lk(g_memo_mu);
    if (g_memo.size() > 4096) g_memo.clear();
    g_memo[sig] = g;
    return g;
}

namespace {
GeneratedKernel generate_pipeline_uncached(const PipelineSpec& spec) {
    GeneratedKernel g;
    g.threads = spec.threads;
    g.tile = spec.tile;
    g.stages = spec.stages;
    g.stage_bytes = stage_bytes_of(spec);
    if (spec.cols.empty()) throw Unsupported("pipeline without input columns");
    if (spec.cols.size() > 24) throw Unsupported("more than 24 staged input columns");

    Emitter em(spec);
    if (spec.sink == SinkKind::Agg && spec.hash) em.base_guard = "in_range";
    std::string keep = "true";
    for (auto& p : spec.predicates) {
        Val v = em.emit(*p);
        keep += " && " + (v.n.empty() ? v.v : "(!" + v.n + " && " + v.v + ")");
    }
    std::ostringstream tu;

    if (spec.sink == SinkKind::Count) {
        em.body << "    return " << keep << ";\n";
        if (spec.ltile <= 0 || spec.tile % spec.ltile) throw PlanError("count pass: stage tile must be a multiple of the logical tile");
        tu << header(spec, "#define CB_KERNEL_SELECT 1\n#define CB_SELECT_COUNT 1\n#define CB_NOUT 0\n#define CB_LTILE " + std::to_string(spec.ltile) + "\n");
        tu << "#include \"cb_kernels.cuh\"\nnamespace cb {\n";
        tu << "CB_D bool cb_row_keep(const Tile& t, int r, i64 grow, const PipeParams& p) {\n    (void)grow; (void)p;\n" << em.body.str() << "}\n} // namespace cb\n";
        g.entry = "cb_select_count";
    } else if (spec.sink == SinkKind::Select) {
        if (spec.outputs.size() > 16) throw Unsupported("more than 16 output columns");
        em.body << "    if (!(" << keep << ")) return false;\n";
        std::ostringstream defs;
        defs << "#define CB_KERNEL_SELECT 1\n#define CB_NOUT " << spec.outputs.size() << "\n#define CB_SEL_MASKED " << (spec.masked ? 1 : 0) << "\n";
        std::vector<Val> outs;
        for (size_t i = 0; i < spec.outputs.size(); i++) {
            Val v = em.emit(*spec.outputs[i]);
            if (v.type.is_string() && spec.outputs[i]->kind != ExprKind::Bound) throw Unsupported("string expressions in a fused projection");
            outs.push_back(v);
            em.body << "    " << to_slot(v, "o.v[" + std::to_string(i) + "]") << " o.valid[" << i << "] = "
                    << (v.n.empty() ? "true" : "!" + v.n) << ";\n";
            OutCol oc;
            oc.type = v.type;
            oc.nullable = v.nullable();
            g.out_cols.push_back(oc);
            g.out_bytes.push_back(v.type.is_string() ? 4 : out_width(v.type));
        }
        em.body << "    return true;\n";
        tu << header(spec, defs.str());
        tu << "constexpr __host__ __device__ int cb_out_bytes(int c) { return ";
        for (size_t i = 0; i < outs.size(); i++) tu << "c == " << i << " ? " << g.out_bytes[i] << " : ";
        tu << "0; }\n";
        tu << "constexpr __host__ __device__ bool cb_out_nullable(int c) { return ";
        for (size_t i = 0; i < outs.size(); i++) tu << "c == " << i << " ? " << (g.out_cols[i].nullable ? "true" : "false") << " : ";
        tu << "false; }\n";
        tu << "#include \"cb_kernels.cuh\"\nnamespace cb {\n";
        tu << "CB_D bool cb_row_select(const Tile& t, int r, i64 grow, const PipeParams& p, SelOut& o) {\n    (void)grow; (void)p;\n"
           << em.body.str() << "}\n} // namespace cb\n";
        g.entry = "cb_pipeline_select";
    } else {
        if (spec.hash) {
            em.body << "    const bool keep_ = in_range && (" << keep << ");\n";
            em.base_guard = "keep_";
        } else em.body << "    (void)in_range;\n    if (!(" << keep << ")) return;\n";
        SlotPlan slots;
        std::vector<AggLayout> layout(spec.aggs.size());
        const bool H = spec.hash;
        auto upd = [&](const std::string& op, const std::string& cond, int w, const std::string& val = "") {
            std::ostringstream o;
            const std::string ws = std::to_string(w);
            if (H) {
                if (op == "count") o << "acc.h_count(" << cond << ", " << ws << ");";
                else if (op == "wrap") o << "acc.h_add_wrap(" << cond << ", " << ws << ", " << val << ");";
                else if (op == "wide") o << "acc.h_add_i64_wide(" << cond << ", " << ws << ", " << val << ");";
                else if (op == "i128") o << "acc.h_add_i128(" << cond << ", " << ws << ", " << val << ");";
                else if (op == "f64") o << "acc.h_add_f64(" << cond << ", " << ws << ", " << val << ");";
                else if (op == "min") o << "acc.h_min(" << cond << ", " << ws << ", " << val << ");";
                else o << "acc.h_max(" << cond << ", " << ws << ", " << val << ");";
            } else {
                o << "if (" << cond << ") ";
                if (op == "count") o << "acc.add_i64_wrap(g, " << ws << ", 1);";
                else if (op == "wrap") o << "acc.add_i64_wrap(g, " << ws << ", " << val << ");";
                else if (op == "wide") o << "acc.add_i64_wide(g, " << ws << ", " << val << ");";
                else if (op == "i128") o << "acc.add_i128(g, " << ws << ", " << val << ");";
                else if (op == "f64") o << "acc.add_f64(g, " << ws << ", " << val << ");";
                else if (op == "min") o << "acc.min_i64(g, " << ws << ", " << val << ");";
                else o << "acc.max_i64(g, " << ws << ", " << val << ");";
            }
            em.body << "    " << o.str() << "\n";
        };
        auto absval = [&](const std::string& iv) { return "cb::i128_abs_of_i64(" + iv + ")"; };
        std::string gid = "0";
        std::string null_group_cond;
        std::ostringstream unpack;
        if (spec.hash) {
            struct KeyPlan { Val v; int bits; bool nullable; int word; };
            std::vector<KeyPlan> kp;
            int n_words_k = 1, used = 0;
            for (size_t k = 0; k < spec.keys.size(); k++) {
                KeyPlan q;
                q.v = em.emit(*spec.keys[k]);
                const DType& kt = spec.keys[k]->type;
                q.bits = key_bits(kt);
                q.nullable = true;
                if (q.bits == 0) throw Unsupported("group key of type " + kt.str() + " cannot be packed into 64-bit hash key words");
                if (q.bits == 64 && spec.keys.size() == 1) {
                    null_group_cond = q.v.n;
                    q.nullable = false;
                }
                int need = q.bits + (q.nullable ? 1 : 0);
                if (need > 64) {
                    if (used > 0) { n_words_k++; used = 0; }
                    q.word = n_words_k - 1;
                    used = 64;
                    kp.push_back(q);
                    continue;
                }
                if (used + need > 64) { n_words_k++; used = 0; }
                q.word = n_words_k - 1;
                used += need;
                kp.push_back(q);
            }
            std::vector<size_t> wide_nullable;
            for (size_t k = 0; k < kp.size(); k++) if (kp[k].nullable && kp[k].bits == 64) wide_nullable.push_back(k);
            int flags_word = -1;
            if (!wide_nullable.empty()) flags_word = n_words_k++;
            if (n_words_k > 4) throw Unsupported("group keys need more than 256 packed bits");
            g.key_words = n_words_k;
            std::vector<std::string> pk(n_words_k);
            for (int w = 0; w < n_words_k; w++) { pk[w] = em.fresh("pk"); em.body << "    cb::u64 " << pk[w] << " = 0;\n"; }
            std::vector<std::string> unpack_steps;
            for (size_t k = 0; k < kp.size(); k++) {
                const KeyPlan& q = kp[k];
                const Val& kv = q.v;
                const DType& kt = spec.keys[k]->type;
                const int bits = q.bits;
                const bool wide_null = q.nullable && bits == 64;
                const bool inline_null = q.nullable && !wide_null;
                const std::string& packed = pk[q.word];
                const std::string isn = kv.n.empty() ? "false" : kv.n;
                std::string raw;
                if (kt.is_decimal()) {
                    if (kv.narrow) raw = "(cb::u64)" + kv.v;
                    else {
                        const std::string valid = kv.n.empty() ? "" : " && !" + kv.n;
                        em.body << "    if (keep_" << valid << " && !cb::i128_fits_i64(" << kv.v << ")) atomicOr(p.hflags, 4);\n";
                        raw = kv.v + ".lo";
                    }
                } else if (kt.id == TypeId::Bool) raw = "(" + kv.v + " ? 1ull : 0ull)";
                else raw = "(cb::u64)(cb::i64)" + kv.v;
                std::string mask = bits == 64 ? "0xffffffffffffffffull" : u64lit((1ull << bits) - 1);
                if (q.nullable && !kv.n.empty()) raw = "(" + kv.n + " ? 0ull : " + raw + ")";
                if (bits == 64) em.body << "    " << packed << " = " << raw << ";\n";
                else em.body << "    " << packed << " = (" << packed << " << " << bits << ") | (" << raw << " & " << mask << ");\n";
                if (inline_null) em.body << "    " << packed << " = (" << packed << " << 1) | (" << isn << " ? 1ull : 0ull);\n";
                if (wide_null) em.body << "    " << pk[flags_word] << " = (" << pk[flags_word] << " << 1) | (" << isn << " ? 1ull : 0ull);\n";
                std::ostringstream u;
                std::string kc = std::to_string(k), kwv = "k" + std::to_string(q.word);
                u << "    {\n";
                if (inline_null) u << "      bool isnull = (" << kwv << " & 1ull) != 0; " << kwv << " >>= 1;\n";
                else if (wide_null) u << "      bool isnull = (k" << flags_word << " & 1ull) != 0; k" << flags_word << " >>= 1;\n";
                else u << "      bool isnull = null_group;\n";
                if (bits == 64) u << "      cb::u64 raw = " << kwv << "; " << kwv << " = 0;\n";
                else u << "      cb::u64 raw = " << kwv << " & " << mask << "; " << kwv << " >>= " << bits << ";\n";
                if (kt.is_decimal()) u << "      cb::fin_store_i128(fp, " << kc << ", g, cb::i128_from_i64((cb::i64)raw), !isnull);\n";
                else if (kt.id == TypeId::Bool) u << "      cb::fin_store_u8(fp, " << kc << ", g, (int)raw, !isnull);\n";
                else if (bits == 64) u << "      cb::fin_store_i64(fp, " << kc << ", g, (cb::i64)raw, !isnull);\n";
                else {
                    int w = kt.is_string() ? 4 : kt.arrow_width();
                    std::string sx = bits == 8 ? "(cb::i32)(signed char)raw" : bits == 16 ? "(cb::i32)(short)raw" : "(cb::i32)raw";
                    u << "      cb::fin_store_i32(fp, " << kc << ", g, " << sx << ", !isnull, " << w << ");\n";
                }
                u << "    }\n";
                unpack_steps.push_back(u.str());
            }
            for (int w = 0; w < n_words_k; w++) unpack << "    cb::u64 k" << w << " = kw[" << w << "]; (void)k" << w << ";\n";
            for (auto it = unpack_steps.rbegin(); it != unpack_steps.rend(); ++it) unpack << *it;
            {
                std::string arr = em.fresh("kw");
                em.body << "    cb::u64 " << arr << "[" << n_words_k << "] = {";
                for (int w = 0; w < n_words_k; w++) em.body << (w ? ", " : "") << pk[w];
                em.body << "};\n";
                if (!null_group_cond.empty()) em.body << "    if (keep_ && " << null_group_cond << ") atomicOr(p.hflags, 8);\n";
                em.body << "    acc.begin(keep_, " << arr << ", " << (null_group_cond.empty() ? "false" : null_group_cond) << ");\n";
            }
        } else if (!spec.ungrouped) {
            for (size_t k = 0; k < spec.keys.size(); k++) {
                Val kv = em.emit(*spec.keys[k]);
                std::string code = kv.type.id == TypeId::Bool && spec.cols[spec.keys[k]->index].phys == Phys::Bitmap ? "(" + kv.v + " ? 1 : 0)" : kv.v;
                if (kv.nullable()) code = "(" + kv.n + " ? p.key_card[" + std::to_string(k) + "] - 1 : " + code + ")";
                gid = "(" + gid + ") * p.key_card[" + std::to_string(k) + "] + " + code;
            }
        }
        if (!spec.hash) em.body << "    const int g = " << gid << ";\n";
        int w_rows = slots.add(W_WRAP64, "cnt|true");
        upd("count", "true", w_rows);

        for (size_t ai = 0; ai < spec.aggs.size(); ai++) {
            const AggExpr& a = spec.aggs[ai];
            AggLayout& L = layout[ai];
            if (spec.mode == AggMode::Partial) {
                std::string cond = "true";
                if (a.filter) {
                    Val f = em.emit(*a.filter);
                    cond = f.n.empty() ? f.v : "(!" + f.n + " && " + f.v + ")";
                }
                std::vector<Val> cv;
                for (auto& c : a.children) cv.push_back(em.emit(*c));
                for (auto& v : cv) if (v.nullable()) cond += " && !" + v.n;
                std::string condkey = cond;
                const Val& v = cv[0];
                std::string use = cond == "true" ? "true" : em.declb(cond);
                auto cnt_slot = [&]() {
                    std::string k = "cnt|" + condkey;
                    bool first = slots.dedup.count(std::to_string((int)W_WRAP64) + "|" + k) == 0;
                    int w = slots.add(W_WRAP64, k);
                    if (first) upd("count", use, w);
                    return w;
                };
                switch (a.kind) {
                case AggKind::Count:
                    L.w_cnt = cnt_slot();
                    break;
                case AggKind::Sum: case AggKind::Avg: {
                    bool dec = a.datatype.is_decimal();
                    bool f64 = !dec && (a.kind == AggKind::Avg || a.datatype.is_float());
                    L.w_cnt = cnt_slot();
                    if (dec) {
                        bool first = slots.dedup.count(std::to_string((int)W_SUM128) + "|sum|" + v.v + "|" + condkey) == 0;
                        L.w_sum = slots.add(W_SUM128, "sum|" + v.v + "|" + condkey);
                        if (first) {
                            u128r vb = em.bound_of(*a.children[0]);
                            if (spec.hash) upd(v.narrow ? "wide" : "i128", use, L.w_sum, v.v);
                            else if (v.narrow && vb < (R63 >> CB_RPT_LOG2)) upd("wrap", use, L.w_sum, v.v);
                            else if (v.narrow) upd("wide", use, L.w_sum, v.v);
                            else upd("i128", use, L.w_sum, v.v);
                        }
                    } else if (f64) {
                        L.is_f64_sum = true;
                        std::string dv = v.type.id == TypeId::Float64 ? v.v : "(double)" + v.v;
                        bool first = slots.dedup.count(std::to_string((int)W_DD_HI) + "|dd|" + dv + "|" + condkey) == 0;
                        L.w_sum = slots.add(W_DD_HI, "dd|" + dv + "|" + condkey, 2);
                        if (first) upd("f64", use, L.w_sum, dv);
                    } else if (a.eval_mode != EvalMode::Legacy) {
                        std::string iv = "(cb::i64)" + v.v;
                        bool first = slots.dedup.count(std::to_string((int)W_SUM128) + "|csum|" + v.v + "|" + condkey) == 0;
                        L.w_sum = slots.add(W_SUM128, "csum|" + v.v + "|" + condkey);
                        L.w_abs = slots.add(W_SUM128, "cabs|" + v.v + "|" + condkey);
                        if (first) { upd("wide", use, L.w_sum, iv); upd("i128", use, L.w_abs, absval(iv)); }
                    } else {
                        bool first = slots.dedup.count(std::to_string((int)W_WRAP64) + "|isum|" + v.v + "|" + condkey) == 0;
                        L.w_sum = slots.add(W_WRAP64, "isum|" + v.v + "|" + condkey);
                        if (first) upd("wrap", use, L.w_sum, "(cb::i64)" + v.v);
                    }
                    break;
                }
                case AggKind::Min: case AggKind::Max: {
                    L.w_cnt = cnt_slot();
                    std::string key = v.type.is_decimal() ? (v.narrow ? v.v : "(cb::i64)" + v.v + ".lo")
                                      : v.type.id == TypeId::Float64 ? "cb::f64_total_key((cb::u64)__double_as_longlong(" + v.v + "))"
                                                                     : "(cb::i64)" + v.v;
                    bool mn = a.kind == AggKind::Min;
                    std::string sk = std::string(mn ? "min|" : "max|") + v.v + "|" + condkey;
                    bool first = slots.dedup.count(std::to_string((int)(mn ? W_MIN : W_MAX)) + "|" + sk) == 0;
                    L.w_minmax = slots.add(mn ? W_MIN : W_MAX, sk);
                    if (first) upd(mn ? "min" : "max", use, L.w_minmax, key);
                    break;
                }
                }
            } else {
                const std::vector<int>& sc = spec.state_slots.at(ai);
                auto col = [&](int i) { Expr b; b.kind = ExprKind::Bound; b.index = sc[i]; b.type = spec.cols[sc[i]].type; return em.emit(b); };
                std::string tag = "agg" + std::to_string(ai);
                switch (a.kind) {
                case AggKind::Count: {
                    Val c = col(0);
                    L.w_cnt = slots.add(W_WRAP64, tag + "cnt");
                    upd("wrap", c.n.empty() ? "true" : "!" + c.n, L.w_cnt, c.v);
                    break;
                }
                case AggKind::Sum:
                    if (a.datatype.is_decimal()) {
                        Val s = col(0), e = col(1);
                        std::string snull = s.n.empty() ? "false" : s.n;
                        L.w_sum = slots.add(W_SUM128, tag + "sum");
                        L.w_cnt = slots.add(W_WRAP64, tag + "cnt");
                        L.w_bad = slots.add(W_WRAP64, tag + "bad");
                        std::string bad = em.declb("!" + e.v + " && " + snull), ok = em.declb("!" + e.v + " && !(" + snull + ")");
                        upd("count", bad, L.w_bad);
                        upd("i128", ok, L.w_sum, Emitter::W(s));
                        upd("count", ok, L.w_cnt);
                    } else if (a.datatype.is_integer() && a.eval_mode != EvalMode::Legacy) {
                        Val s = col(0);
                        std::string snull = s.n.empty() ? "false" : s.n;
                        L.w_sum = slots.add(W_SUM128, tag + "sum");
                        L.w_abs = slots.add(W_SUM128, tag + "abs");
                        L.w_cnt = slots.add(W_WRAP64, tag + "cnt");
                        std::string ok;
                        if (a.eval_mode == EvalMode::Try) {
                            Val e = col(1);
                            L.w_bad = slots.add(W_WRAP64, tag + "bad");
                            upd("count", em.declb("!" + e.v + " && " + snull), L.w_bad);
                            ok = em.declb("!" + e.v + " && !(" + snull + ")");
                        } else ok = em.declb("!(" + snull + ")");
                        upd("wide", ok, L.w_sum, s.v);
                        upd("i128", ok, L.w_abs, absval(s.v));
                        upd("count", ok, L.w_cnt);
                    } else if (a.datatype.is_integer()) {
                        Val s = col(0);
                        L.w_sum = slots.add(W_WRAP64, tag + "sum");
                        L.w_cnt = slots.add(W_WRAP64, tag + "cnt");
                        const std::string ok = s.n.empty() ? "true" : "!" + s.n;
                        upd("wrap", ok, L.w_sum, s.v);
                        upd("count", ok, L.w_cnt);
                    } else {
                        Val s = col(0);
                        L.is_f64_sum = true;
                        L.w_sum = slots.add(W_DD_HI, tag + "sum", 2);
                        L.w_cnt = slots.add(W_WRAP64, tag + "cnt");
// ... 203 lines not shown
```

### datafusion-comet_b200/csrc/codegen.h

```cpp
#pragma once
#include "plan.h"

#include <map>
#include <string>
#include <vector>

namespace cb200 {

enum class Phys { Bitmap, I8, I16, I32, I64, F32, F64, I128, Dict32 };
int phys_bytes(Phys p);

struct SourceCol {
    int src_index;
    DType type;
    Phys phys;
    bool has_validity;
    int assume_bits = 0;
};

#define CB_RPT_LOG2 14

enum class SinkKind { Select, Agg, Count };

enum WordKind { W_SUM128 = 0, W_DD_HI = 1, W_DD_LO = 2, W_WRAP64 = 3, W_MIN = 4, W_MAX = 5 };

struct OutCol {
    DType type;
    bool nullable;
};

struct PipelineSpec {
    std::vector<SourceCol> cols;
    std::vector<ExprP> predicates;
    SinkKind sink = SinkKind::Select;
    std::vector<ExprP> outputs;
    std::vector<ExprP> keys;
    std::vector<bool> key_nullable;
    std::vector<AggExpr> aggs;
    std::vector<std::vector<int>> state_slots;
    AggMode mode = AggMode::Partial;
    bool ungrouped = false;
    bool hash = false;
    bool masked = false;
    bool stream = false;
    int tile = 512, stages = 3, threads = 256;
    int ltile = 0;
};

struct GeneratedKernel {
    std::string source;
    std::string key;
    std::string entry;
    std::string finalize_entry;
    int stage_bytes = 0;
    int n_words = 0;
    std::vector<int> word_kinds;
    std::vector<OutCol> out_cols;
    std::vector<int> out_bytes;
    int threads = 256, tile = 512, stages = 3;
    bool hash = false;
    bool ungrouped = false;
    int n_key_cols = 0;
    int key_words = 1;
    size_t dyn_smem(int n_groups) const;
};

GeneratedKernel generate_pipeline(const PipelineSpec& spec);
std::string pipeline_signature(const PipelineSpec& spec);

}
```

### datafusion-comet_b200/csrc/device/cb_kernels.cuh

```cuda
#ifndef CB_KERNELS_CUH
#define CB_KERNELS_CUH

namespace cb {

}
#include "cb_params.h"
namespace cb {

CB_D u32 smem_u32(const void* p) { return (u32)__cvta_generic_to_shared(p); }
CB_D void mbar_init(u64* bar, u32 count) {
    asm volatile("mbarrier.init.shared::cta.b64 [%0], %1;" ::"r"(smem_u32(bar)), "r"(count));
}
CB_D void mbar_fence_init() { asm volatile("fence.mbarrier_init.release.cluster;" ::: "memory"); }
CB_D void mbar_expect_tx(u64* bar, u32 bytes) {
    asm volatile("mbarrier.arrive.expect_tx.shared::cta.b64 _, [%0], %1;" ::"r"(smem_u32(bar)), "r"(bytes) : "memory");
}
CB_D void mbar_wait(u64* bar, u32 parity) {
    asm volatile(
        "{\n"
        ".reg .pred p;\n"
        "CB_WAIT_%=:\n"
        "mbarrier.try_wait.parity.shared::cta.b64 p, [%0], %1;\n"
        "@p bra CB_DONE_%=;\n"
        "bra CB_WAIT_%=;\n"
// ... 549 lines not shown
                out[((size_t)g * CB_WORDS + w) * 2 + 1] = t.b;
            }
            consumer_bar();
        }
    }
#endif
}

}
#endif


#ifdef CB_KERNEL_AGG
namespace cb {


CB_D void set_err_raw(i32* err, int bit) { atomicOr(err, 1 << bit); }
CB_D i128 fin_i128(const u64* T, int w) { return mk128(T[w * 2], (i64)T[w * 2 + 1]); }
CB_D double fin_dd(const u64* T, int w) { return __longlong_as_double((i64)T[w * 2]); }
CB_D void fin_store_i128(const FinParams& fp, int c, int g, i128 v, bool valid) {
    reinterpret_cast<i128*>(fp.out[c])[g] = v; fp.outv[c][g] = valid ? 1 : 0;
}
CB_D void fin_store_i64(const FinParams& fp, int c, int g, i64 v, bool valid) {
    reinterpret_cast<i64*>(fp.out[c])[g] = v; fp.outv[c][g] = valid ? 1 : 0;
}
CB_D void fin_store_f64(const FinParams& fp, int c, int g, double v, bool valid) {
    reinterpret_cast<double*>(fp.out[c])[g] = v; fp.outv[c][g] = valid ? 1 : 0;
}
CB_D void fin_store_f32(const FinParams& fp, int c, int g, float v, bool valid) {
    reinterpret_cast<float*>(fp.out[c])[g] = v; fp.outv[c][g] = valid ? 1 : 0;
}
CB_D void fin_store_u8(const FinParams& fp, int c, int g, int v, bool valid) {
    fp.out[c][g] = (u8)v; fp.outv[c][g] = valid ? 1 : 0;
}
CB_D void fin_store_i32(const FinParams& fp, int c, int g, i32 v, bool valid, int width) {
    if (width == 4) reinterpret_cast<i32*>(fp.out[c])[g] = v;
    else if (width == 2) reinterpret_cast<short*>(fp.out[c])[g] = (short)v;
    else reinterpret_cast<signed char*>(fp.out[c])[g] = (signed char)v;
    fp.outv[c][g] = valid ? 1 : 0;
}

CB_D void cb_finalize_group(const FinParams& fp, int g, const u64* T);
#if CB_HASH
CB_D void cb_unpack_key(const FinParams& fp, int g, const u64* kw, bool null_group);

extern "C" __global__ void cb_hash_init(u64* totals, long long first, long long n) {
    long long i = (long long)blockIdx.x * blockDim.x + threadIdx.x;
    if (i >= n) return;
    i += first;
#pragma unroll
    for (int w = 0; w < CB_WORDS; w++) { totals[(i * CB_WORDS + w) * 2] = acc_identity(cb_word_kind(w)); totals[(i * CB_WORDS + w) * 2 + 1] = 0; }
}
extern "C" __global__ void cb_hash_rehash(const u64* key_of_gid, int range_rows, const i32* counters, u64* hkeys, u32 mask) {
    const long long idx = (long long)blockIdx.x * blockDim.x + threadIdx.x;
    if (idx >= (long long)range_rows * CB_GID_RANGES) return;
    const int r = (int)(idx / range_rows), l = (int)(idx % range_rows);
    if (l >= counters[r]) return;
    const int g = (int)idx;
#if CB_KEY_WORDS > 1
    u64 kw[CB_KEY_WORDS];
#pragma unroll
    for (int i = 0; i < CB_KEY_WORDS; i++) kw[i] = key_of_gid[(size_t)g * CB_KEY_WORDS + i];
    const u64 key = Acc::key_tag(kw);
    u32 s = (u32)(key ^ (key >> 32)) & mask;
#else
    u64 key = key_of_gid[g];
    u32 s = (u32)Acc::mix64(key) & mask;
#endif
    while (true) {
        u64 prev = atomicCAS((unsigned long long*)&hkeys[2 * (size_t)s], (unsigned long long)CB_EMPTY_KEY, (unsigned long long)key);
        if (prev == CB_EMPTY_KEY) { *((i32*)&hkeys[2 * (size_t)s + 1]) = g; return; }
        s = (s + 1u) & mask;
    }
}
#endif

extern "C" __global__ void cb_fold(const __grid_constant__ FinParams fp) {
    int idx = blockIdx.x * blockDim.x + threadIdx.x;
    int total = fp.n_groups * CB_WORDS;
    if (idx >= total) return;
    int w = idx % CB_WORDS;
    int kind = cb_word_kind(w);
    if (kind == 2) return;
    u64 a, b;
    if (fp.first) { a = acc_identity(kind); b = 0; if (kind == 0) b = 0; }
    else { a = fp.totals[idx * 2]; b = fp.totals[idx * 2 + 1]; }
    for (int c = 0; c < fp.n_ctas; c++) {
        const u64* P = fp.partials + ((size_t)c * total + idx) * 2;
        u64 pa = P[0], pb = P[1];
        if (kind == 0) { i128 s = i128_add(mk128(a, (i64)b), mk128(pa, (i64)pb)); a = s.lo; b = (u64)s.hi; }
        else if (kind == 1) {
            dd A, B;
            A.hi = __longlong_as_double((i64)a); A.lo = __longlong_as_double((i64)b);
            B.hi = __longlong_as_double((i64)pa); B.lo = __longlong_as_double((i64)pb);
            dd_add_dd(A, B);
            a = (u64)__double_as_longlong(A.hi); b = (u64)__double_as_longlong(A.lo);
        }
        else if (kind == 3) a += pa;
        else if (kind == 4) a = (u64)(((i64)pa < (i64)a) ? (i64)pa : (i64)a);
        else a = (u64)(((i64)pa > (i64)a) ? (i64)pa : (i64)a);
    }
    if (kind == 0) {
        i128 s = i128_add(mk128(a, (i64)b), mk128(fp.spill[idx * 2], (i64)fp.spill[idx * 2 + 1]));
        a = s.lo; b = (u64)s.hi;
        fp.spill[idx * 2] = 0; fp.spill[idx * 2 + 1] = 0;
    }
    fp.totals[idx * 2] = a;
    fp.totals[idx * 2 + 1] = b;
}

extern "C" __global__ void cb_finalize(const __grid_constant__ FinParams fp) {
    int g = blockIdx.x * blockDim.x + threadIdx.x;
    if (g >= fp.n_groups) return;
    const u64* T = fp.totals + (size_t)g * CB_WORDS * 2;
#if CB_HASH
    int gid = g;
    bool is_sentinel = false, is_null_group = false;
    if (g < fp.n_hash_groups) {
        int lo = 0, hi = CB_GID_RANGES - 1;
        while (lo < hi) { const int mid = (lo + hi + 1) >> 1; if (fp.gid_prefix[mid] <= g) lo = mid; else hi = mid - 1; }
        gid = lo * fp.gid_range + (g - fp.gid_prefix[lo]);
    }
    if (g >= fp.n_hash_groups) {
        int extra = g - fp.n_hash_groups;
        if (fp.sentinel_used && extra == 0) is_sentinel = true;
        else is_null_group = true;
        gid = is_sentinel ? fp.max_groups : fp.max_groups + 1;
    }
    const u64* TH = fp.totals + (size_t)gid * CB_WORDS * 2;
    fp.present[g] = 1;
    u64 kw[CB_KEY_WORDS];
#pragma unroll
    for (int i = 0; i < CB_KEY_WORDS; i++) kw[i] = (is_sentinel || is_null_group) ? (is_sentinel ? CB_EMPTY_KEY : 0ull) : fp.hkeys[(size_t)gid * CB_KEY_WORDS + i];
    cb_unpack_key(fp, g, kw, is_null_group);
    cb_finalize_group(fp, g, TH);
    return;
#else
    fp.present[g] = (i64)T[CB_W_ROWS * 2] > 0 ? 1 : 0;
#endif
    cb_finalize_group(fp, g, T);
}

}
#endif

#ifdef CB_KERNEL_SELECT
namespace cb {

#ifndef CB_SEL_MASKED
#define CB_SEL_MASKED 0
#endif
#define CB_BAR_BYTES 256
#ifndef CB_LTILE
#define CB_LTILE CB_TILE
#endif
constexpr int SEL_NW = CB_THREADS / 32;
constexpr int SEL_RPW = CB_LTILE / SEL_NW;
constexpr int SEL_ROUNDS = SEL_RPW / 32;
constexpr int SEL_SUB = CB_TILE / CB_LTILE;
static_assert(CB_LTILE % (SEL_NW * 32) == 0 && CB_TILE % CB_LTILE == 0, "tile must be a multiple of 32 rows per warp");

#define CB_SELECT_PROLOGUE()                                                                                          \
    extern __shared__ __align__(128) u8 smem[];                                                                       \
    constexpr int SB = stage_bytes();                                                                                 \
    u64* full = reinterpret_cast<u64*>(smem);                                                                         \
    u64* empty = full + CB_STAGES;                                                                                    \
// ... 170 lines not shown
```

### datafusion-comet_b200/csrc/device/cb_params.h

```cpp
#ifndef CB_PARAMS_H
#define CB_PARAMS_H
#include "cb_math.h"
namespace cb {

#define CB_MAX_COLS 24
#define CB_MAX_OUT 24
#define CB_MAX_KEYS 4

#define CB_SCAN_CHUNK 4096

struct PipeParams {
    const u8* col[CB_MAX_COLS];
    const u8* val[CB_MAX_COLS];
    i64 n_rows;
    i32 n_tiles;
    i32 n_groups;
    i32 key_card[CB_MAX_KEYS];
    u8* out[CB_MAX_OUT];
    u32* out_valid[CB_MAX_OUT];
    u32* sel_off;
    u32* sel_chunk;
    u32* sel_mask;
    i64* out_count;
    u8* partials;
    u64* spill;
    i32* err;
    u64* vmask;
    u64* hkeys;
    u64* hkey_of_gid;
    u64* htotals;
    u32 hmask;
    i32 max_groups;
    i32* hflags;
};
#define CB_GID_RANGES 64
#define CB_HFLAG_CTR 16
#define CB_HFLAG_WORDS (CB_HFLAG_CTR + CB_GID_RANGES)
#define CB_HF_SENTINEL 1
#define CB_HF_FULL 2
#define CB_HF_WIDE_KEY 4
#define CB_HF_NULL_GROUP 8


struct FinParams {
    const u64* partials;
    u64* spill;
    u64* totals;
    i32 n_ctas, n_groups, first;
    u8* out[CB_MAX_OUT];
    u8* outv[CB_MAX_OUT];
    u8* present;
    i32* err;
    const u64* hkeys;
    i32 n_hash_groups;
    i32 max_groups;
    i32 sentinel_used;
    i32 null_group_used;
    i32 gid_range;
    i32 gid_prefix[CB_GID_RANGES + 1];
    u64 cert_b[CB_MAX_OUT][2];
};

}
#endif
```

### datafusion-comet_b200/csrc/exec.cpp

```cpp
#include "exec_internal.h"

#include "aot_kernels.h"

#include <algorithm>
#include <cstdlib>
#include <ctime>
#include <mutex>

namespace cb200 {

enum { ERR_I128_OVERFLOW = 0, ERR_ANSI_OVERFLOW = 1, ERR_ORDER_DEPENDENT = 2, ERR_DIVIDE_BY_ZERO = 3, ERR_ARROW_DIVIDE_BY_ZERO = 4 };

bool trace_on() {
    static int on = -1;
    if (on < 0) { const char* e = getenv("CB200_TRACE"); on = (e && *e && *e != '0') ? 1 : 0; }
    return on == 1;
}
double now_ms() {
    struct timespec ts;
    clock_gettime(CLOCK_MONOTONIC, &ts);
    return ts.tv_sec * 1e3 + ts.tv_nsec * 1e-6;
}
TraceSpan::TraceSpan(const char* n) : name(n), t0(trace_on() ? now_ms() : 0) {}
TraceSpan::~TraceSpan() {
    if (trace_on()) { static const double tz = now_ms(); const double t1 = now_ms(); fprintf(stderr, "[cb200 trace] %-28s %8.3f ms   (ends at +%.3f ms)\n", name, t1 - t0, t1 - tz); }
}

void cuda_check(cudaError_t e, const char* what) {
    if (e != cudaSuccess) throw ExecError(2, "", std::string("CUDA error in ") + what + ": " + cudaGetErrorString(e));
}

static thread_local cudaStream_t tl_alloc_stream = nullptr;
void set_alloc_stream(cudaStream_t s) { tl_alloc_stream = s; }

namespace {
struct CachedBlock { void* ptr; cudaStream_t stream; cudaEvent_t ev; };
struct BlockCache {
    std::mutex mu;
    std::multimap<size_t, CachedBlock> free_blocks;
    size_t cached_bytes = 0;
};
BlockCache g_block_cache[64];
const size_t BLOCK_CACHE_MIN = 1 << 20;
size_t block_cache_limit() {
    static size_t lim = 0;
    if (!lim) { const char* e = getenv("CB200_BLOCK_CACHE_BYTES"); lim = e && *e ? (size_t)atoll(e) : (size_t)32 << 30; if (!lim) lim = 1; }
    return lim;
}
size_t size_class(size_t n) {
    size_t p2 = (size_t)1 << 20;
    while ((p2 << 1) <= n) p2 <<= 1;
    const size_t step = p2 >> 3;
    return (n + step - 1) / step * step;
}
int current_device() { int d = 0; cudaGetDevice(&d); return d >= 0 && d < 64 ? d : 0; }
size_t block_cache_flush(int dev) {
    BlockCache& c = g_block_cache[dev];
    std::multimap<size_t, CachedBlock> take;
    size_t freed = 0;
    {
        std::lock_guard<std::mutex> lk(c.mu);
        take.swap(c.free_blocks);
        freed = c.cached_bytes;
        c.cached_bytes = 0;
    }
    for (auto& kv : take) { cudaEventSynchronize(kv.second.ev); cudaFreeAsync(kv.second.ptr, nullptr); cudaEventDestroy(kv.second.ev); }
    return freed;
}
}
size_t release_cached_device_memory() { return block_cache_flush(current_device()); }

DeviceBuf::DeviceBuf(size_t n) {
    bytes = (n + 255) / 256 * 256 + 256;
    stream = tl_alloc_stream;
    if (bytes >= BLOCK_CACHE_MIN) {
        bytes = size_class(bytes);
        BlockCache& c = g_block_cache[current_device()];
        CachedBlock blk{nullptr, nullptr, nullptr};
        {
            std::lock_guard<std::mutex> lk(c.mu);
            auto it = c.free_blocks.find(bytes);
            if (it != c.free_blocks.end()) { blk = it->second; c.free_blocks.erase(it); c.cached_bytes -= bytes; }
        }
        if (blk.ptr) {
            if (blk.stream != stream) cudaStreamWaitEvent(stream, blk.ev, 0);
            cudaEventDestroy(blk.ev);
            ptr = blk.ptr;
            return;
        }
    }
    cudaError_t e = cudaMallocAsync(&ptr, bytes, stream);
    if (e == cudaErrorMemoryAllocation) {
        cudaGetLastError();
        block_cache_flush(current_device());
        cudaStreamSynchronize(stream);
        e = cudaMallocAsync(&ptr, bytes, stream);
    }
    cuda_check(e, "cudaMallocAsync");
}
DeviceBuf::~DeviceBuf() {
    if (!(owned && ptr)) return;
    if (bytes >= BLOCK_CACHE_MIN && bytes == size_class(bytes)) {
        BlockCache& c = g_block_cache[current_device()];
        cudaEvent_t ev = nullptr;
        if (cudaEventCreateWithFlags(&ev, cudaEventDisableTiming) == cudaSuccess && cudaEventRecord(ev, stream) == cudaSuccess) {
            std::lock_guard<std::mutex> lk(c.mu);
            if (c.cached_bytes + bytes <= block_cache_limit()) {
                c.free_blocks.insert({bytes, CachedBlock{ptr, stream, ev}});
                c.cached_bytes += bytes;
                return;
            }
        }
        if (ev) cudaEventDestroy(ev);
    }
    cudaFreeAsync(ptr, stream);
}

void ExecContext::collect_timing() {
    if (!ev_pending) return;
    float ms = 0;
    if (cudaEventElapsedTime(&ms, ev0, ev1) == cudaSuccess) { pipeline_ms += ms; pipeline_launches++; }
    ev_pending = false;
}

void ExecContext::check_device_errors() {
    cuda_check(cudaMemcpyAsync(h_err, d_err, sizeof(int), cudaMemcpyDeviceToHost, stream), "error flag copy");
    cuda_check(cudaStreamSynchronize(stream), "stream sync");
    collect_timing();
    int e = *h_err;
    if (!e) return;
    cudaMemsetAsync(d_err, 0, sizeof(int), stream);
    if (e & (1 << ERR_ANSI_OVERFLOW))
        throw ExecError(10, "ARITHMETIC_OVERFLOW", "[ARITHMETIC_OVERFLOW] overflow in ANSI mode");
    if (e & (1 << ERR_DIVIDE_BY_ZERO))
        throw ExecError(10, "DIVIDE_BY_ZERO", "[DIVIDE_BY_ZERO] Division by zero. Use `try_divide` to tolerate divisor being 0 and return NULL instead. "
                                              "If necessary set \"spark.sql.ansi.enabled\" to \"false\" to bypass this error.");
    if (e & (1 << ERR_ARROW_DIVIDE_BY_ZERO)) throw ExecError(11, "", "Arrow error: Divide by zero error");
    if (e & (1 << ERR_I128_OVERFLOW))
        throw ExecError(11, "", "Arrow error: Arithmetic overflow: Overflow happened on decimal arithmetic");
    if (e & (1 << ERR_ORDER_DEPENDENT))
        throw ExecError(12, "", "SUM/AVG overflow here depends on the row order (some orderings of these rows overflow, others do not); "
                                "the reference adds in row order -- the row-ordered fallback is not built yet, so the plan is refused rather than guessed");
    throw ExecError(13, "", "device error flags " + std::to_string(e));
}

static DType dtype_from_format(const char* f) {
    std::string s = f ? f : "";
    if (s == "b") return mk_type(TypeId::Bool);
    if (s == "c") return mk_type(TypeId::Int8);
    if (s == "s") return mk_type(TypeId::Int16);
    if (s == "i") return mk_type(TypeId::Int32);
    if (s == "l") return mk_type(TypeId::Int64);
    if (s == "f") return mk_type(TypeId::Float32);
    if (s == "g") return mk_type(TypeId::Float64);
    if (s == "u") return mk_type(TypeId::String);
    if (s == "z") return mk_type(TypeId::Binary);
    if (s == "tdD") return mk_type(TypeId::Date);
    if (s.rfind("tsu:", 0) == 0) return mk_type(s.size() > 4 ? TypeId::Timestamp : TypeId::TimestampNtz);
    if (s.rfind("d:", 0) == 0) {
        int p = 0, sc = 0, bits = 128;
        if (sscanf(s.c_str(), "d:%d,%d,%d", &p, &sc, &bits) < 2) throw PlanError("bad decimal format " + s);
        if (bits != 128) throw Unsupported("decimal bit width " + std::to_string(bits));
        return mk_decimal(p, sc);
    }
    throw Unsupported("Arrow format '" + s + "' is outside the GPU hot path");
}

struct SchemaOnlySource : ExecNode {
    bool next(Batch&) override { return false; }
};

struct StreamSource : ExecNode {
    ExecContext* ctx;
    ArrowArrayStream* stream;
    bool schema_checked = false, eof = false;
    std::vector<bool> col_is_dict;
    std::vector<int> dict_index_width;
    std::vector<DictionaryP> dicts;

    StreamSource(ExecContext* c, ArrowArrayStream* s, const std::vector<DType>& fields) : ctx(c), stream(s) { schema = fields; }
    ~StreamSource() override {
        if (stream && stream->release) stream->release(stream);
    }

    void check_schema() {
        ArrowSchema sc;
        memset(&sc, 0, sizeof(sc));
        if (stream->get_schema(stream, &sc) != 0) {
            const char* m = stream->get_last_error ? stream->get_last_error(stream) : nullptr;
            throw ExecError(3, "", std::string("Failed to import ArrowArrayStream schema: ") + (m ? m : "?"));
        }
        if (sc.n_children != (int64_t)schema.size()) {
            int64_t n = sc.n_children;
            if (sc.release) sc.release(&sc);
            throw PlanError("scan declares " + std::to_string(schema.size()) + " fields but the stream has " + std::to_string(n));
        }
        col_is_dict.assign(schema.size(), false);
        dict_index_width.assign(schema.size(), 4);
        dicts.assign(schema.size(), nullptr);
        for (size_t i = 0; i < schema.size(); i++) {
            ArrowSchema* ch = sc.children[i];
            if (ch->dictionary) {
                DType vt = dtype_from_format(ch->dictionary->format);
                DType it = dtype_from_format(ch->format);
                if (!vt.is_string() || !it.is_integer()) throw Unsupported("dictionary column that is not int -> utf8");
                if (!schema[i].is_string()) throw PlanError("scan field " + std::to_string(i) + " is " + schema[i].str() + " but the stream column is a string dictionary");
                col_is_dict[i] = true;
                dict_index_width[i] = it.arrow_width();
                if (it.arrow_width() == 8) throw Unsupported("int64 dictionary indices");
                dicts[i] = std::make_shared<Dictionary>();
            } else {
                DType t = dtype_from_format(ch->format);
                bool ok = t == schema[i] || (t.is_decimal() && schema[i].is_decimal() && t.scale == schema[i].scale) ||
                          (t.id == TypeId::Timestamp && schema[i].id == TypeId::TimestampNtz) || (t.id == TypeId::TimestampNtz && schema[i].id == TypeId::Timestamp);
                if (!ok) throw PlanError("scan field " + std::to_string(i) + " is " + schema[i].str() + " but the stream column is " + t.str());
            }
        }
        if (sc.release) sc.release(&sc);
        schema_checked = true;
    }

    bool next(Batch& out) override {
        if (!schema_checked) check_schema();
        if (eof) return false;
        std::vector<ArrowArray> arrs;
        int64_t total = 0;
        while (total < ctx->chunk_rows) {
            ArrowArray a;
            memset(&a, 0, sizeof(a));
            if (stream->get_next(stream, &a) != 0) {
                const char* m = stream->get_last_error ? stream->get_last_error(stream) : nullptr;
                for (auto& x : arrs) if (x.release) x.release(&x);
                throw ExecError(3, "", std::string("ArrowArrayStream get_next failed: ") + (m ? m : "?"));
            }
            if (!a.release) { eof = true; break; }
            if (a.length > 0) { total += a.length; arrs.push_back(a); }
            else a.release(&a);
        }
        if (arrs.empty()) return false;
        try {
            upload(arrs, total, out);
        } catch (...) {
            for (auto& x : arrs) if (x.release) x.release(&x);
            throw;
        }
        cuda_check(cudaStreamSynchronize(ctx->stream), "H2D copies");
        for (auto& x : arrs) if (x.release) x.release(&x);
        return true;
    }

    std::vector<int32_t> unify_dict(size_t col, const ArrowArray* d) {
        Dictionary& g = *dicts[col];
        const int32_t* off = (const int32_t*)d->buffers[1] + d->offset;
        const char* chars = (const char*)d->buffers[2];
        std::vector<int32_t> remap((size_t)d->length);
        bool identity = true;
        for (int64_t k = 0; k < d->length; k++) {
            std::string v(chars + off[k], (size_t)(off[k + 1] - off[k]));
            auto it = std::find(g.values.begin(), g.values.end(), v);
            int32_t code;
            if (it == g.values.end()) { code = (int32_t)g.values.size(); g.values.push_back(v); }
            else code = (int32_t)(it - g.values.begin());
            remap[(size_t)k] = code;
            if (code != k) identity = false;
        }
        if (identity) remap.clear();
        return remap;
    }

    cudaError_t h2d(void* dst, const void* src, size_t n) {
        ctx->h2d_bytes += (int64_t)n;
        return cudaMemcpyAsync(dst, src, n, cudaMemcpyHostToDevice, ctx->stream);
    }

    void upload(std::vector<ArrowArray>& arrs, int64_t total, Batch& out) {
        TraceSpan ts("source.upload");
        out.n_rows = total;
        out.cols.clear();
        out.cols.resize(schema.size());
        cudaStream_t st = ctx->stream;
        for (size_t c = 0; c < schema.size(); c++) {
            Column& col = out.cols[c];
            col.type = schema[c];
            bool any_nulls = false;
            for (auto& a : arrs) {
                ArrowArray* ch = a.children[c];
                if (ch->null_count != 0 && ch->buffers[0]) any_nulls = true;
            }
            if (any_nulls) {
                col.validity = std::make_shared<DeviceBuf>((size_t)(total + 7) / 8 + 8);
                cuda_check(cudaMemsetAsync(col.validity->ptr, 0, col.validity->bytes, st), "memset validity");
            }
            std::vector<DeviceBufP> temps;
            if (col_is_dict[c]) {
                col.is_dict = true;
                col.dict = dicts[c];
                int w = dict_index_width[c];
                bool need_remap = false;
                std::vector<std::vector<int32_t>> remaps;
                for (auto& a : arrs) {
                    remaps.push_back(unify_dict(c, a.children[c]->dictionary));
                    if (!remaps.back().empty()) need_remap = true;
                }
                if (!need_remap) {
                    col.phys = w == 1 ? Phys::I8 : w == 2 ? Phys::I16 : Phys::I32;
                    col.data = std::make_shared<DeviceBuf>((size_t)total * w);
                } else {
                    col.phys = Phys::I32;
                    col.data = std::make_shared<DeviceBuf>((size_t)total * 4);
                }
                int64_t row = 0;
                for (size_t k = 0; k < arrs.size(); k++) {
                    ArrowArray* ch = arrs[k].children[c];
                    const char* src = (const char*)ch->buffers[1] + ch->offset * w;
                    if (!need_remap) {
                        cuda_check(h2d((char*)col.data->ptr + row * w, src, (size_t)ch->length * w), "H2D dict codes");
                    } else {
                        auto tmp = std::make_shared<DeviceBuf>((size_t)ch->length * w);
                        temps.push_back(tmp);
                        cuda_check(h2d(tmp->ptr, src, (size_t)ch->length * w), "H2D dict codes");
                        std::vector<int32_t> table = remaps[k];
                        if (table.empty()) { table.resize((size_t)ch->dictionary->length); for (size_t i = 0; i < table.size(); i++) table[i] = (int32_t)i; }
                        auto dt = std::make_shared<DeviceBuf>(table.size() * 4 + 4);
                        temps.push_back(dt);
                        cuda_check(h2d(dt->ptr, table.data(), table.size() * 4), "H2D remap table");
                        cuda_check(cudaStreamSynchronize(st), "remap table copy");
                        launch_remap_codes(tmp->ptr, w, ch->length, (const int*)dt->ptr, (int)table.size(), (int*)col.data->ptr + row, st);
                    }
                    row += ch->length;
                }
            } else if (schema[c].is_string()) {
                int64_t total_chars = 0;
                for (auto& a : arrs) {
                    ArrowArray* ch = a.children[c];
                    const int32_t* off = (const int32_t*)ch->buffers[1] + ch->offset;
                    total_chars += off[ch->length] - off[0];
                }
                if (total_chars > INT32_MAX) throw Unsupported("more than 2 GiB of string data in one chunk");
                col.offsets = std::make_shared<DeviceBuf>((size_t)(total + 1) * 4);
                col.chars = std::make_shared<DeviceBuf>((size_t)total_chars + 16);
                std::vector<int32_t> offs((size_t)total + 1);
                int64_t row = 0;
                int32_t base = 0;
                for (auto& a : arrs) {
                    ArrowArray* ch = a.children[c];
                    const int32_t* off = (const int32_t*)ch->buffers[1] + ch->offset;
                    for (int64_t i = 0; i < ch->length; i++) offs[(size_t)(row + i)] = base + (off[i] - off[0]);
                    int32_t nchars = off[ch->length] - off[0];
                    if (nchars) cuda_check(h2d((char*)col.chars->ptr + base, (const char*)ch->buffers[2] + off[0], (size_t)nchars), "H2D chars");
                    base += nchars;
                    row += ch->length;
                }
                offs[(size_t)total] = base;
                cuda_check(h2d(col.offsets->ptr, offs.data(), offs.size() * 4), "H2D offsets");
                cuda_check(cudaStreamSynchronize(st), "offsets copy");
                col.phys = Phys::I32;
            } else {
                col.phys = phys_of(schema[c]);
                int w = schema[c].arrow_width();
                if (w == 0) {
                    col.data = std::make_shared<DeviceBuf>((size_t)(total + 7) / 8 + 8);
                    cuda_check(cudaMemsetAsync(col.data->ptr, 0, col.data->bytes, st), "memset bool");
                    int64_t row = 0;
                    for (auto& a : arrs) {
                        ArrowArray* ch = a.children[c];
                        append_bits((uint32_t*)col.data->ptr, row, (const uint8_t*)ch->buffers[1], ch->offset, ch->length, temps);
                        row += ch->length;
                    }
                } else {
                    col.data = std::make_shared<DeviceBuf>((size_t)total * w);
                    int64_t row = 0;
                    for (auto& a : arrs) {
                        ArrowArray* ch = a.children[c];
                        cuda_check(h2d((char*)col.data->ptr + row * w, (const char*)ch->buffers[1] + ch->offset * w, (size_t)ch->length * w), "H2D column");
                        row += ch->length;
                    }
                }
            }
            if (any_nulls) {
                int64_t row = 0, nulls = 0;
                for (auto& a : arrs) {
                    ArrowArray* ch = a.children[c];
                    bool has = ch->null_count != 0 && ch->buffers[0];
                    append_bits((uint32_t*)col.validity->ptr, row, has ? (const uint8_t*)ch->buffers[0] : nullptr, ch->offset, ch->length, temps);
                    nulls += has ? (ch->null_count < 0 ? 1 : ch->null_count) : 0;
                    row += ch->length;
                }
                col.null_count = nulls;
            }
            if (!temps.empty()) cuda_check(cudaStreamSynchronize(st), "temp buffers");
        }
    }

    void append_bits(uint32_t* dst, int64_t row, const uint8_t* src, int64_t src_off, int64_t n, std::vector<DeviceBufP>& temps) {
        if (n <= 0) return;
        if (src && (row & 7) == 0 && (src_off & 7) == 0 && ((n & 7) == 0)) {
            cuda_check(h2d((char*)dst + (row >> 3), src + (src_off >> 3), (size_t)(n >> 3)), "H2D bitmap");
            return;
        }
        const uint8_t* dsrc = nullptr;
        int64_t doff = 0;
        if (src) {
            int64_t b0 = src_off >> 3, b1 = (src_off + n + 7) >> 3;
            auto tmp = std::make_shared<DeviceBuf>((size_t)(b1 - b0) + 8);
            temps.push_back(tmp);
            cuda_check(h2d(tmp->ptr, src + b0, (size_t)(b1 - b0)), "H2D bitmap");
            dsrc = (const uint8_t*)tmp->ptr;
            doff = src_off & 7;
        }
        launch_bitmap_append(dst, row, dsrc, doff, n, ctx->stream);
    }
};

struct TableSource : ExecNode {
    std::shared_ptr<DeviceTable> table;
    ExecContext* ctx = nullptr;
    bool done = false;
    TableSource(std::shared_ptr<DeviceTable> t, const std::vector<DType>& fields, ExecContext* c) : table(std::move(t)), ctx(c) {
        schema = fields;
        if (table->cols.size() != fields.size()) throw PlanError("bound device table has " + std::to_string(table->cols.size()) + " columns, scan declares " + std::to_string(fields.size()));
    }
    int64_t pos = 0;
    bool packed = false;
    int64_t rows_hint() const override { return table->n_rows - pos; }
    bool next(Batch& out) override {
        if (done) return false;
        if (table->needs_packing && !packed) {
            size_t n = (size_t)table->n_rows;
            for (auto& c : table->cols) {
                if (c.valid_bytes && !c.validity) {
                    c.validity = std::make_shared<DeviceBuf>((n + 31) / 32 * 4 + 8);
                    launch_bytes_to_bitmap((const unsigned char*)c.valid_bytes->ptr, table->n_rows, (uint32_t*)c.validity->ptr, ctx->stream);
                    ctx->kernel_launches++;
                }
                if (c.bool_bytes && !c.data) {
                    c.data = std::make_shared<DeviceBuf>((n + 31) / 32 * 4 + 8);
                    launch_bytes_to_bitmap((const unsigned char*)c.bool_bytes->ptr, table->n_rows, (uint32_t*)c.data->ptr, ctx->stream);
                    ctx->kernel_launches++;
                }
            }
            packed = true;
        }
        const int64_t chunk = std::max<int64_t>(1024, ctx->chunk_rows / 1024 * 1024);
        const int64_t r0 = pos, r1 = std::min(table->n_rows, pos + chunk);
        pos = r1;
        if (pos >= table->n_rows) done = true;
        out.n_rows = r1 - r0;
        out.cols = table->cols;
        if (r0 > 0 || r1 < table->n_rows) {
            for (auto& c : out.cols) {
                auto slice = [&](DeviceBufP& b, size_t num, size_t den) {
                    if (!b) return;
                    auto v = std::make_shared<DeviceBuf>((char*)b->ptr + (size_t)r0 * num / den, (size_t)(r1 - r0) * num / den + 1);
                    v->owner = b;
                    b = v;
                };
                const int w = phys_bytes(c.is_dict && c.phys == Phys::I32 ? Phys::Dict32 : c.phys);
                if (w == 0) slice(c.data, 1, 8);
                else slice(c.data, (size_t)w, 1);
                slice(c.validity, 1, 8);
                slice(c.valid_bytes, 1, 1);
                slice(c.bool_bytes, 1, 1);
                if (c.null_count > 0) c.null_count = -1;
            }
        }
        return out.n_rows > 0;
    }
};


struct SelectNode : FusedBase {
    std::vector<ExprP> outputs;
    DeviceBufP sel_off, sel_chunk, counters;
// ... 103 lines not shown
                c.null_count = -1;
            }
        }
        const int grid = std::min(ctx->num_sms, p.n_tiles);
        int64_t kept = in.n_rows;
        int64_t* h_kept = nullptr;
        if (!predicates.empty()) {
            GeneratedKernel cg = generate_pipeline(make_count_spec(&in));
            auto cmod = jit_get(cg, true);
            cb::PipeParams cp;
            fill_inputs_of(cp, in, pred_cols, cg.tile);
            const size_t m = (size_t)p.n_tiles * (size_t)(g.threads / 32);
            const size_t n_chunks = (m + CB_SCAN_CHUNK - 1) / CB_SCAN_CHUNK;
            if (!sel_off || sel_off->bytes < m * 4) sel_off = std::make_shared<DeviceBuf>(m * 4 + m / 2);
            if (!sel_chunk || sel_chunk->bytes < (n_chunks + 1) * 4) sel_chunk = std::make_shared<DeviceBuf>((n_chunks + 1) * 4 + n_chunks * 2);
            if (!counters) counters = std::make_shared<DeviceBuf>(64);
            cp.sel_off = (cb::u32*)sel_off->ptr;
            if (masked()) {
                const size_t words = (size_t)p.n_tiles * (size_t)g.tile / 32 + 64;
                if (!sel_mask || sel_mask->bytes < words * 4) sel_mask = std::make_shared<DeviceBuf>(words * 4 + words);
                cp.sel_mask = (cb::u32*)sel_mask->ptr;
                p.sel_mask = cp.sel_mask;
            }
            launch(cmod->kernel(cg.entry), dim3(std::min(ctx->num_sms, cp.n_tiles)), dim3(cg.threads + 32), cg.dyn_smem(0), &cp);
            launch_scan_u32((unsigned*)sel_off->ptr, (long long)m, CB_SCAN_CHUNK, (unsigned*)sel_chunk->ptr, (long long*)counters->ptr, st);
            ctx->kernel_launches += 2;
            p.sel_off = (cb::u32*)sel_off->ptr;
            p.sel_chunk = (cb::u32*)sel_chunk->ptr;
            h_kept = (int64_t*)ctx->h_err + 1;
            cuda_check(cudaMemcpyAsync(h_kept, counters->ptr, 8, cudaMemcpyDeviceToHost, st), "read kept count"); ctx->d2h_bytes += (int64_t)(8);
        }
        launch(mod->kernel(g.entry), dim3(grid), dim3(g.threads + 32), g.dyn_smem(0), &p);
        ctx->pipeline_rows += in.n_rows;
        ctx->check_device_errors();
        if (h_kept) kept = *h_kept;
        out.n_rows = kept;
    }
};


struct PartitionNode : ExecNode {
    ExecContext* ctx;
    ExecNodeP child;
    std::vector<int> key_cols;
    int n_parts = 1;

    bool next(Batch& out) override {
        Batch in;
        if (!child->next(in)) return false;
        TraceSpan ts("partition");
        to_device(in);
        int64_t n = in.n_rows;
        cudaStream_t st = ctx->stream;
        HashKeyCols kc;
        memset(&kc, 0, sizeof(kc));
        if (key_cols.size() > 8) throw Unsupported("more than 8 hash-partition keys");
        std::vector<DeviceBufP> keep;
        for (int ci : key_cols) {
            const Column& c = in.cols[(size_t)ci];
            HashKeyCol& k = kc.col[kc.n++];
            k.data = c.data ? c.data->ptr : nullptr;
            k.validity = c.validity ? (const unsigned char*)c.validity->ptr : nullptr;
            switch (c.type.id) {
            case TypeId::Bool: k.kind = HK_BOOL; break;
            case TypeId::Int8: k.kind = HK_I8; break;
            case TypeId::Int16: k.kind = HK_I16; break;
            case TypeId::Int32: case TypeId::Date: k.kind = HK_I32; break;
            case TypeId::Int64: case TypeId::Timestamp: case TypeId::TimestampNtz: k.kind = HK_I64; break;
            case TypeId::Float32: k.kind = HK_F32; break;
            case TypeId::Float64: k.kind = HK_F64; break;
            case TypeId::Decimal:
                if (c.phys == Phys::I64) k.kind = c.type.precision <= 18 ? HK_DEC_SMALL_64 : HK_DEC_LARGE_64;
                else k.kind = c.type.precision <= 18 ? HK_DEC_SMALL_128 : HK_DEC_LARGE_128;
                break;
            case TypeId::String: case TypeId::Binary:
                if (c.is_dict) {
                    k.kind = c.phys == Phys::I8 ? HK_DICT8 : c.phys == Phys::I16 ? HK_DICT16 : HK_DICT32;
                    std::vector<int32_t> off{0};
                    std::string chars;
                    for (auto& v : c.dict->values) { chars += v; off.push_back((int32_t)chars.size()); }
                    auto doff = std::make_shared<DeviceBuf>(off.size() * 4), dch = std::make_shared<DeviceBuf>(chars.size() + 16);
                    cuda_check(cudaMemcpyAsync(doff->ptr, off.data(), off.size() * 4, cudaMemcpyHostToDevice, st), "dict offsets");
                    if (!chars.empty()) cuda_check(cudaMemcpyAsync(dch->ptr, chars.data(), chars.size(), cudaMemcpyHostToDevice, st), "dict chars");
                    cuda_check(cudaStreamSynchronize(st), "dict upload");
                    keep.push_back(doff); keep.push_back(dch);
                    k.dict_offsets = (const int*)doff->ptr;
                    k.dict_chars = (const unsigned char*)dch->ptr;
                } else {
                    if (!c.offsets || !c.chars) throw Unsupported("string partition key without offsets/chars");
                    k.kind = HK_UTF8;
                    k.dict_offsets = (const int*)c.offsets->ptr;
                    k.dict_chars = (const unsigned char*)c.chars->ptr;
                }
                break;
            default: throw Unsupported("hash partitioning on " + c.type.str());
            }
        }
        size_t nb = (size_t)(n + 1023) / 1024 + 1;
        auto pids = std::make_shared<DeviceBuf>((size_t)n * 4 + 16);
        auto hist = std::make_shared<DeviceBuf>(nb * n_parts * 4);
        auto base = std::make_shared<DeviceBuf>(nb * n_parts * 8);
        auto starts = std::make_shared<DeviceBuf>((size_t)(n_parts + 1) * 8);
        auto row_idx = std::make_shared<DeviceBuf>((size_t)n * 8 + 16);
        cuda_check(cudaMemsetAsync(starts->ptr, 0, (size_t)(n_parts + 1) * 8, st), "memset starts");
        auto chunk_tmp = std::make_shared<DeviceBuf>((size_t)(partition_chunks(n) + 1) * n_parts * 8);
        launch_partition(kc, n, (unsigned)n_parts, nullptr, (unsigned*)pids->ptr, (int*)hist->ptr, (long long*)base->ptr, (long long*)chunk_tmp->ptr,
                         (long long*)starts->ptr, (long long*)row_idx->ptr, st);
        ctx->kernel_launches += 6;
        out.n_rows = n;
        out.cols.clear();
        for (auto& c : in.cols) {
            Column o = c;
            if (c.offsets) throw Unsupported("repartitioning plain string columns (dictionary-encode them first)");
            int w = phys_bytes(c.is_dict && c.phys == Phys::I32 ? Phys::Dict32 : c.phys);
            if (w == 0) {
                auto bytes = std::make_shared<DeviceBuf>((size_t)n + 16);
                launch_gather_bits(c.data->ptr, (const long long*)row_idx->ptr, n, bytes->ptr, st);
                o.data = std::make_shared<DeviceBuf>((size_t)(n + 31) / 32 * 4 + 8);
                launch_bytes_to_bitmap((const unsigned char*)bytes->ptr, n, (uint32_t*)o.data->ptr, st);
                o.bool_bytes = bytes;
                ctx->kernel_launches += 2;
            } else {
                o.data = std::make_shared<DeviceBuf>((size_t)std::max<int64_t>(n, 1) * w);
                launch_gather(c.data->ptr, w, (const long long*)row_idx->ptr, n, o.data->ptr, st);
                ctx->kernel_launches++;
                if (c.type.id == TypeId::Bool) o.bool_bytes = o.data;
            }
            if (c.validity) {
                auto bytes = std::make_shared<DeviceBuf>((size_t)n + 16);
                launch_gather_bits(c.validity->ptr, (const long long*)row_idx->ptr, n, bytes->ptr, st);
                o.validity = std::make_shared<DeviceBuf>((size_t)(n + 31) / 32 * 4 + 8);
                launch_bytes_to_bitmap((const unsigned char*)bytes->ptr, n, (uint32_t*)o.validity->ptr, st);
                o.valid_bytes = bytes;
                ctx->kernel_launches += 2;
            }
            out.cols.push_back(o);
        }
        ctx->partition_starts.assign((size_t)n_parts + 1, 0);
        cuda_check(cudaMemcpyAsync(ctx->partition_starts.data(), starts->ptr, (size_t)(n_parts + 1) * 8, cudaMemcpyDeviceToHost, st), "starts D2H"); ctx->d2h_bytes += (int64_t)((size_t)(n_parts + 1) * 8);
        ctx->check_device_errors();
        return true;
    }

    void to_device(Batch& b) {
        for (auto& c : b.cols) {
            if (!c.on_host) continue;
            size_t n = (size_t)b.n_rows;
            if (c.type.is_string()) {
                auto d = std::make_shared<Dictionary>();
                std::vector<int32_t> codes(n);
                for (size_t r = 0; r < n; r++) {
                    std::string v((const char*)c.h_data.data() + c.h_offsets[r], (size_t)(c.h_offsets[r + 1] - c.h_offsets[r]));
                    auto it = std::find(d->values.begin(), d->values.end(), v);
                    if (it == d->values.end()) { codes[r] = (int32_t)d->values.size(); d->values.push_back(v); }
                    else codes[r] = (int32_t)(it - d->values.begin());
                }
                c.data = std::make_shared<DeviceBuf>(n * 4 + 16);
                if (n) cuda_check(cudaMemcpyAsync(c.data->ptr, codes.data(), n * 4, cudaMemcpyHostToDevice, ctx->stream), "keys H2D");
                cuda_check(cudaStreamSynchronize(ctx->stream), "keys H2D sync");
                c.is_dict = true; c.dict = d; c.phys = Phys::I32;
            } else if (c.type.id == TypeId::Bool) {
                std::vector<uint8_t> bits((n + 7) / 8 + 8, 0);
                for (size_t r = 0; r < n; r++) if (c.h_data[r]) bits[r >> 3] |= (uint8_t)(1u << (r & 7));
                c.data = std::make_shared<DeviceBuf>(bits.size());
                cuda_check(cudaMemcpyAsync(c.data->ptr, bits.data(), bits.size(), cudaMemcpyHostToDevice, ctx->stream), "bool H2D");
                cuda_check(cudaStreamSynchronize(ctx->stream), "bool H2D sync");
                c.phys = Phys::Bitmap;
            } else {
                c.data = std::make_shared<DeviceBuf>(c.h_data.size() + 16);
                if (!c.h_data.empty()) cuda_check(cudaMemcpyAsync(c.data->ptr, c.h_data.data(), c.h_data.size(), cudaMemcpyHostToDevice, ctx->stream), "col H2D");
                cuda_check(cudaStreamSynchronize(ctx->stream), "col H2D sync");
                c.phys = phys_of(c.type);
            }
            if (!c.h_valid.empty()) {
                std::vector<uint8_t> bits((n + 7) / 8 + 8, 0);
                for (size_t r = 0; r < n; r++) if (c.h_valid[r]) bits[r >> 3] |= (uint8_t)(1u << (r & 7));
                c.validity = std::make_shared<DeviceBuf>(bits.size());
                cuda_check(cudaMemcpyAsync(c.validity->ptr, bits.data(), bits.size(), cudaMemcpyHostToDevice, ctx->stream), "validity H2D");
                cuda_check(cudaStreamSynchronize(ctx->stream), "validity H2D sync");
            }
            c.on_host = false;
        }
    }
};

static ExprP bound_ref(int i, const DType& t) {
    auto e = std::make_shared<Expr>();
    e->kind = ExprKind::Bound;
    e->index = i;
    e->type = t;
    return e;
}

static ExecNodeP build_node(const OperatorP& op, ExecContext* ctx, PlanInputs* inputs, bool build_only, const std::vector<int>& assume);

static ExecNodeP build_source(const OperatorP& op, ExecContext* ctx, PlanInputs* inputs, bool build_only, const std::vector<int>& assume) {
    const bool scan = op->kind == OpKind::Scan || op->kind == OpKind::ShuffleScan;
    if (build_only && (scan || op->kind == OpKind::NativeScan)) {
        auto s = std::make_shared<SchemaOnlySource>();
        s->schema = op->schema;
        return s;
    }
    if (scan) {
        if (inputs->streams.empty() && inputs->tables.empty()) throw PlanError("No input for scan");
        ArrowArrayStream* st = inputs->streams.empty() ? nullptr : inputs->streams.front();
        std::shared_ptr<DeviceTable> tb = inputs->tables.empty() ? nullptr : inputs->tables.front();
        if (!inputs->streams.empty()) inputs->streams.erase(inputs->streams.begin());
        if (!inputs->tables.empty()) inputs->tables.erase(inputs->tables.begin());
        if (tb) return std::make_shared<TableSource>(tb, op->schema, ctx);
        if (!st) throw PlanError("No input for scan");
        return std::make_shared<StreamSource>(ctx, st, op->schema);
    }
    if (op->kind == OpKind::NativeScan) return make_native_scan(op, ctx);
    return build_node(op, ctx, inputs, build_only, assume);
}

static ExecNodeP build_node(const OperatorP& op, ExecContext* ctx, PlanInputs* inputs, bool build_only, const std::vector<int>& assume) {
    OperatorP cur = op;
    OperatorP agg_op;
    if (cur->kind == OpKind::ShuffleWriter) {
        auto n = std::make_shared<PartitionNode>();
        n->ctx = ctx;
        n->child = build_node(cur->children[0], ctx, inputs, build_only, assume);
        n->schema = cur->schema;
        n->n_parts = cur->num_partitions;
        for (auto& e : cur->hash_exprs) {
            if (e->kind != ExprKind::Bound) throw Unsupported("computed hash-partition keys (only plain column keys)");
            n->key_cols.push_back(e->index);
        }
        return n;
    }
    if (cur->kind == OpKind::HashAgg) { agg_op = cur; cur = cur->children[0]; }
    std::vector<OperatorP> chain;
    while (cur->kind == OpKind::Filter || cur->kind == OpKind::Projection) { chain.push_back(cur); cur = cur->children[0]; }
    if (!agg_op && chain.empty()) return build_source(cur, ctx, inputs, build_only, assume);
    ExecNodeP src = build_source(cur, ctx, inputs, build_only, assume);
    std::vector<ExprP> cols;
    for (size_t i = 0; i < src->schema.size(); i++) cols.push_back(bound_ref((int)i, src->schema[i]));
    std::vector<ExprP> preds;
    for (auto it = chain.rbegin(); it != chain.rend(); ++it) {
        const OperatorP& o = *it;
        if (o->kind == OpKind::Filter) preds.push_back(substitute(o->predicate, cols));
        else {
            std::vector<ExprP> nc;
            for (auto& e : o->project_list) nc.push_back(substitute(e, cols));
            cols = nc;
        }
    }
    if (!preds.empty()) src->push_filters(preds);
    if (agg_op) return make_agg_node(agg_op, src, preds, cols, ctx, assume);
    auto n = std::make_shared<SelectNode>();
    n->ctx = ctx;
    n->child = src;
    n->schema = op->schema;
    n->predicates = preds;
    n->outputs = cols;
    for (auto& e : cols)
        if (e->type.is_string() && e->kind != ExprKind::Bound) throw Unsupported("string expressions through a fused filter/projection (only column references)");
    std::vector<ExprP> roots = preds;
    for (auto& e : cols) roots.push_back(e);
    n->assign_slots(roots);
    n->assign_pred_slots();
    if (n->used_cols.empty()) throw Unsupported("projection of constants only");
    return n;
}

ExecNodeP build_exec(const OperatorP& op, ExecContext* ctx, PlanInputs* inputs) { return build_node(op, ctx, inputs, false, {}); }

std::vector<GeneratedKernel> plan_kernels_for_build(const OperatorP& op, const std::vector<int>& assume) {
    ExecContext defaults;
    std::vector<GeneratedKernel> out;
    for (ExecNodeP n = build_node(op, &defaults, nullptr, true, assume); n;) {
        if (auto f = std::dynamic_pointer_cast<FusedBase>(n)) {
            for (const PipelineSpec& s : f->build_specs()) out.push_back(generate_pipeline(s));
            n = f->child;
        } else {
            auto pn = std::dynamic_pointer_cast<PartitionNode>(n);
            n = pn ? pn->child : nullptr;
        }
    }
    return out;
}

namespace {
struct ArrayHolder {
    std::vector<std::vector<uint8_t>> bufs;
    const void* ptrs[3] = {nullptr, nullptr, nullptr};
};
void release_array(ArrowArray* a) {
    delete (ArrayHolder*)a->private_data;
    a->release = nullptr;
}
struct SchemaHolder {
    std::string format, name;
};
void release_schema(ArrowSchema* s) {
    delete (SchemaHolder*)s->private_data;
    s->release = nullptr;
}
std::string arrow_format(const DType& t) {
    switch (t.id) {
    case TypeId::Bool: return "b";
    case TypeId::Int8: return "c";
    case TypeId::Int16: return "s";
    case TypeId::Int32: return "i";
    case TypeId::Int64: return "l";
    case TypeId::Float32: return "f";
    case TypeId::Float64: return "g";
    case TypeId::String: return "u";
    case TypeId::Binary: return "z";
    case TypeId::Date: return "tdD";
    case TypeId::Timestamp: return "tsu:UTC";
    case TypeId::TimestampNtz: return "tsu:";
    case TypeId::Decimal: return "d:" + std::to_string(t.precision) + "," + std::to_string(t.scale);
    default: throw Unsupported("export of " + t.str());
    }
}
std::vector<uint8_t> pack_bits(const uint8_t* bytes, size_t n) {
    std::vector<uint8_t> out((n + 7) / 8 + 8, 0);
    for (size_t i = 0; i < n; i++) if (bytes[i]) out[i >> 3] |= (uint8_t)(1u << (i & 7));
    return out;
}
}

static std::vector<uint8_t> fetch_bits(ExecContext* ctx, const void* dev_bitmap, int64_t row0, size_t n) {
    const size_t first = (size_t)row0 >> 3, shift = (size_t)row0 & 7, nbytes = (shift + n + 7) / 8;
    std::vector<uint8_t> raw(nbytes + 9, 0);
    if (n) {
        cuda_check(cudaMemcpyAsync(raw.data(), (const uint8_t*)dev_bitmap + first, nbytes, cudaMemcpyDeviceToHost, ctx->stream), "D2H validity");
        cuda_check(cudaStreamSynchronize(ctx->stream), "D2H sync");
        ctx->d2h_bytes += (int64_t)nbytes;
    }
    if (shift == 0) { raw.resize((n + 7) / 8 + 8); return raw; }
    std::vector<uint8_t> out((n + 7) / 8 + 8, 0);
    for (size_t i = 0; i < (n + 7) / 8; i++) out[i] = (uint8_t)((raw[i] >> shift) | (raw[i + 1] << (8 - shift)));
    return out;
}

void export_batch(Batch& b, ExecContext* ctx, ArrowArray* out_arrays, ArrowSchema* out_schemas, int n_cols, int64_t row0, int64_t n_rows) {
    TraceSpan ts("export_batch");
    if ((int)b.cols.size() != n_cols) throw PlanError("executePlan: caller passed " + std::to_string(n_cols) + " output slots, plan produces " + std::to_string(b.cols.size()) + " columns");
    if (row0 < 0 || n_rows < 0 || row0 + n_rows > b.n_rows) throw PlanError("export_batch: slice out of range");
    const size_t n = (size_t)n_rows, r0 = (size_t)row0;
    for (int i = 0; i < n_cols; i++) {
        Column& c = b.cols[(size_t)i];
        auto* h = new ArrayHolder();
        int64_t null_count = 0;
        std::vector<uint8_t> validity, data, offs;
        if (c.on_host) {
            if (!c.h_valid.empty()) {
                validity = pack_bits(c.h_valid.data() + r0, n);
                for (size_t r = 0; r < n; r++) null_count += c.h_valid[r0 + r] ? 0 : 1;
            }
            if (c.type.is_string()) {
                offs.resize((n + 1) * 4);
                const int32_t* ho = (const int32_t*)c.h_offsets.data();
                int32_t* o = (int32_t*)offs.data();
                for (size_t r = 0; r <= n; r++) o[r] = ho[r0 + r] - ho[r0];
                data.assign(c.h_data.begin() + ho[r0], c.h_data.begin() + ho[r0 + n]);
                data.resize(data.size() + 8);
            } else if (c.type.id == TypeId::Bool) data = pack_bits(c.h_data.data() + r0, n);
            else {
                const size_t w = (size_t)c.type.arrow_width();
                data.assign(c.h_data.begin() + (ptrdiff_t)(r0 * w), c.h_data.begin() + (ptrdiff_t)((r0 + n) * w));
                data.resize(data.size() + 8);
            }
        } else if (c.is_dict) {
            std::vector<int32_t> codes(n + 1);
            if (n) cuda_check(cudaMemcpyAsync(codes.data(), (const uint8_t*)c.data->ptr + r0 * 4, n * 4, cudaMemcpyDeviceToHost, ctx->stream), "D2H key codes");
            cuda_check(cudaStreamSynchronize(ctx->stream), "D2H sync");
            ctx->d2h_bytes += (int64_t)n * 4;
            std::vector<uint8_t> vb = c.validity && n ? fetch_bits(ctx, c.validity->ptr, row0, n) : std::vector<uint8_t>((n + 7) / 8 + 8, 0xff);
            offs.resize((n + 1) * 4);
            int32_t* o = (int32_t*)offs.data();
            o[0] = 0;
            for (size_t r = 0; r < n; r++) {
                bool valid = (vb[r >> 3] >> (r & 7)) & 1;
                if (valid) { const std::string& sv = c.dict->values.at((size_t)codes[r]); data.insert(data.end(), sv.begin(), sv.end()); }
                else null_count++;
                o[r + 1] = (int32_t)data.size();
            }
            data.resize(data.size() + 8);
            if (null_count) validity = vb;
        } else {
            if (c.type.is_string()) throw Unsupported("export of device string columns");
            int w = c.type.id == TypeId::Bool ? 1 : c.type.arrow_width();
            std::vector<uint8_t> raw(n * (size_t)w + 8);
            if (n) cuda_check(cudaMemcpyAsync(raw.data(), (const uint8_t*)c.data->ptr + r0 * (size_t)w, n * (size_t)w, cudaMemcpyDeviceToHost, ctx->stream), "D2H output");
            ctx->d2h_bytes += (int64_t)(n * (size_t)w);
            cuda_check(cudaStreamSynchronize(ctx->stream), "D2H sync");
            if (c.validity) {
                validity = fetch_bits(ctx, c.validity->ptr, row0, n);
                for (size_t r = 0; r < n; r++) null_count += ((validity[r >> 3] >> (r & 7)) & 1) ? 0 : 1;
                if (null_count == 0) validity.clear();
            }
            if (c.type.id == TypeId::Bool) data = pack_bits(raw.data(), n);
            else data = std::move(raw);
        }
        bool is_str = c.type.is_string();
        h->bufs.push_back(std::move(validity));
        if (is_str) h->bufs.push_back(std::move(offs));
        h->bufs.push_back(std::move(data));
        h->ptrs[0] = h->bufs[0].empty() ? nullptr : h->bufs[0].data();
        h->ptrs[1] = h->bufs[1].data();
        if (is_str) h->ptrs[2] = h->bufs[2].data();
        ArrowArray& a = out_arrays[i];
        memset(&a, 0, sizeof(a));
        a.length = (int64_t)n;
        a.null_count = null_count;
        a.offset = 0;
        a.n_buffers = is_str ? 3 : 2;
        a.buffers = h->ptrs;
        a.release = release_array;
        a.private_data = h;
        auto* sh = new SchemaHolder();
        sh->format = arrow_format(c.type);
        sh->name = "col_" + std::to_string(i);
        ArrowSchema& s = out_schemas[i];
        memset(&s, 0, sizeof(s));
        s.format = sh->format.c_str();
        s.name = sh->name.c_str();
        s.flags = ARROW_FLAG_NULLABLE;
        s.release = release_schema;
        s.private_data = sh;
    }
}

}
```

### datafusion-comet_b200/csrc/exec.h

```cpp
#pragma once
#include "arrow_abi.h"
#include "codegen.h"
#include "jit.h"
#include "plan.h"

#include <cuda_runtime.h>
#include <memory>
#include <string>
#include <vector>

namespace cb200 {

struct ExecError : std::runtime_error {
    int code;
    std::string error_class;
    ExecError(int c, const std::string& cls, const std::string& msg) : std::runtime_error(msg), code(c), error_class(cls) {}
};

void cuda_check(cudaError_t e, const char* what);

struct TraceSpan {
    const char* name;
    double t0;
    explicit TraceSpan(const char* n);
    ~TraceSpan();
};
bool trace_on();
double now_ms();
void set_alloc_stream(cudaStream_t s);
size_t release_cached_device_memory();

struct DeviceBuf {
    void* ptr = nullptr;
    size_t bytes = 0;
    bool owned = true;
    cudaStream_t stream = nullptr;
    std::shared_ptr<void> owner;
    DeviceBuf() {}
    DeviceBuf(size_t n);
    DeviceBuf(void* p, size_t n) : ptr(p), bytes(n), owned(false) {}
    ~DeviceBuf();
    DeviceBuf(const DeviceBuf&) = delete;
    DeviceBuf& operator=(const DeviceBuf&) = delete;
};
using DeviceBufP = std::shared_ptr<DeviceBuf>;

struct Dictionary {
    std::vector<std::string> values;
};
using DictionaryP = std::shared_ptr<Dictionary>;

struct Column {
    DType type;
    Phys phys = Phys::I32;
    bool is_dict = false;
    DictionaryP dict;
    DeviceBufP data, validity;
    DeviceBufP offsets, chars;
    DeviceBufP valid_bytes;
    DeviceBufP bool_bytes;
    int64_t null_count = 0;
    bool on_host = false;
    std::vector<uint8_t> h_data;
    std::vector<uint8_t> h_valid;
    std::vector<int32_t> h_offsets;
};

struct Batch {
    int64_t n_rows = 0;
    std::vector<Column> cols;
};

struct ExecContext {
    int device = 0;
    cudaStream_t stream = nullptr;
    int num_sms = 132;
    int64_t chunk_rows = 1ll << 26;
    int hash_threads = 512;
    int64_t stream_agg_min_rows = 4 << 20;
    double stream_agg_max_ratio = 0.5;
    int batch_size = 8192;
    int* d_err = nullptr;
    int* h_err = nullptr;
    int64_t kernel_launches = 0;
    cudaEvent_t ev0 = nullptr, ev1 = nullptr;
    bool ev_pending = false;
    double pipeline_ms = 0;
    int64_t pipeline_launches = 0;
    int64_t pipeline_rows = 0;
    int64_t h2d_bytes = 0, d2h_bytes = 0;
    int64_t scan_pruned_row_groups = 0, scan_pruned_rows = 0;
    int64_t agg_strategies = 0;
    std::vector<int64_t> partition_starts;
    void check_device_errors();
    void collect_timing();
};

struct ExecNode {
    std::vector<DType> schema;
    virtual ~ExecNode() {}
    virtual bool next(Batch& out) = 0;
    virtual void push_filters(const std::vector<ExprP>&) {}
    virtual int64_t rows_hint() const { return -1; }
};
using ExecNodeP = std::shared_ptr<ExecNode>;

struct DeviceTable {
    int64_t n_rows = 0;
    std::vector<Column> cols;
    bool needs_packing = false;
};

struct PlanInputs {
    std::vector<ArrowArrayStream*> streams;
    std::vector<std::shared_ptr<DeviceTable>> tables;
};
ExecNodeP build_exec(const OperatorP& op, ExecContext* ctx, PlanInputs* inputs);

ExecNodeP make_native_scan(const OperatorP& op, ExecContext* ctx);

void export_batch(Batch& b, ExecContext* ctx, ArrowArray* out_arrays, ArrowSchema* out_schemas, int n_cols, int64_t row0, int64_t n_rows);

void register_memory_file(const std::string& name, const uint8_t* p, size_t n);
std::string describe_parquet(const std::string& path);

std::vector<GeneratedKernel> plan_kernels_for_build(const OperatorP& op, const std::vector<int>& assume_bits = {});

}
```

### datafusion-comet_b200/csrc/exec_internal.h

```cpp
#pragma once
#include "exec.h"

#include "device/cb_params.h"

#include <cstring>
#include <map>
#include <set>

namespace cb200 {

static constexpr size_t SMEM_BUDGET = 220 * 1024;

inline Phys phys_of(const DType& t) {
    switch (t.id) {
    case TypeId::Bool: return Phys::Bitmap;
    case TypeId::Int8: return Phys::I8;
    case TypeId::Int16: return Phys::I16;
    case TypeId::Int32: case TypeId::Date: return Phys::I32;
    case TypeId::Int64: case TypeId::Timestamp: case TypeId::TimestampNtz: return Phys::I64;
    case TypeId::Float32: return Phys::F32;
    case TypeId::Float64: return Phys::F64;
    case TypeId::Decimal: return Phys::I128;
    default: return Phys::I32;
    }
// ... 7 lines not shown
inline ExprP substitute(const ExprP& e, const std::vector<ExprP>& cur) {
    if (e->kind == ExprKind::Bound) {
        if (e->index < 0 || e->index >= (int)cur.size()) throw PlanError("bound reference out of range while fusing");
        return clone_expr(cur[e->index]);
    }
    auto c = std::make_shared<Expr>(*e);
    for (auto& ch : c->children) ch = substitute(ch, cur);
    return c;
}
inline void collect_bound(const ExprP& e, std::vector<int>& order, std::set<int>& seen) {
    if (e->kind == ExprKind::Bound) {
        if (!seen.count(e->index)) { seen.insert(e->index); order.push_back(e->index); }
        return;
    }
    for (auto& c : e->children) collect_bound(c, order, seen);
}
inline void rewrite_bound(const ExprP& e, const std::map<int, int>& slot_of) {
    if (e->kind == ExprKind::Bound) { e->index = slot_of.at(e->index); return; }
    for (auto& c : e->children) rewrite_bound(c, slot_of);
}

struct FusedBase : ExecNode {
    ExecContext* ctx;
    ExecNodeP child;
    std::vector<ExprP> predicates;
    std::vector<int> used_cols;
    std::map<int, int> slot_of;

    virtual std::vector<PipelineSpec> build_specs() const = 0;

    std::vector<SourceCol> stage_cols(const Batch* b) const { return stage_cols_of(b, used_cols); }
    std::vector<SourceCol> stage_cols_of(const Batch* b, const std::vector<int>& which) const {
        std::vector<SourceCol> cols;
        for (int ci : which) {
            SourceCol sc;
            sc.src_index = ci;
            sc.type = child->schema[ci];
            if (b) {
                const Column& c = b->cols[ci];
                sc.phys = c.phys;
                sc.has_validity = c.validity != nullptr;
                if (c.is_dict) sc.phys = c.phys == Phys::I8 ? Phys::I8 : c.phys == Phys::I16 ? Phys::I16 : Phys::Dict32;
            } else {
                sc.phys = sc.type.is_string() ? Phys::Dict32 : phys_of(sc.type);
                sc.has_validity = false;
            }
            cols.push_back(sc);
        }
        return cols;
    }
    void assign_slots(const std::vector<ExprP>& roots) {
        std::set<int> seen;
        for (auto& e : roots) collect_bound(e, used_cols, seen);
        for (size_t i = 0; i < used_cols.size(); i++) slot_of[used_cols[i]] = (int)i;
    }
    static std::vector<ExprP> to_slots(const std::vector<ExprP>& es, const std::map<int, int>& slot_of) {
        std::vector<ExprP> out;
        for (auto& e : es) {
            ExprP c = clone_expr(e);
            rewrite_bound(c, slot_of);
            out.push_back(c);
        }
        return out;
    }
    void fill_inputs(cb::PipeParams& p, const Batch& b, int tile, int64_t row0 = 0, int64_t row1 = -1) const { fill_inputs_of(p, b, used_cols, tile, row0, row1); }
    void fill_inputs_of(cb::PipeParams& p, const Batch& b, const std::vector<int>& which, int tile, int64_t row0 = 0, int64_t row1 = -1) const {
        memset(&p, 0, sizeof(p));
        if (row1 < 0) row1 = b.n_rows;
        if (row0 & 1023) throw ExecError(15, "", "internal: launch range must start on a 1024-row boundary");
        for (size_t i = 0; i < which.size(); i++) {
            const Column& c = b.cols[which[i]];
            if (!c.data) throw Unsupported("column " + std::to_string(which[i]) + " (" + c.type.str() + ") has no fixed-width device representation");
            int w = phys_bytes(c.is_dict && c.phys == Phys::I32 ? Phys::Dict32 : c.phys);
            p.col[i] = (const cb::u8*)c.data->ptr + (w == 0 ? row0 / 8 : row0 * w);
            p.val[i] = c.validity ? (const cb::u8*)c.validity->ptr + row0 / 8 : nullptr;
        }
        p.n_rows = row1 - row0;
        p.n_tiles = (int)((p.n_rows + tile - 1) / tile);
        p.err = ctx->d_err;
    }
    void launch(cudaKernel_t k, dim3 grid, dim3 block, size_t smem, void* params) {
        cuda_check(cudaFuncSetAttribute((const void*)k, cudaFuncAttributeMaxDynamicSharedMemorySize, (int)smem), "cudaFuncSetAttribute(smem)");
        void* args[] = {params};
        if (ctx->ev_pending) { cuda_check(cudaStreamSynchronize(ctx->stream), "stream sync"); ctx->collect_timing(); }
        cuda_check(cudaEventRecord(ctx->ev0, ctx->stream), "event record");
        cuda_check(cudaLaunchKernel((const void*)k, grid, block, args, smem, ctx->stream), "kernel launch");
        cuda_check(cudaEventRecord(ctx->ev1, ctx->stream), "event record");
        ctx->ev_pending = true;
        ctx->kernel_launches++;
    }
};

ExecNodeP make_agg_node(const OperatorP& agg_op, const ExecNodeP& src, const std::vector<ExprP>& preds, const std::vector<ExprP>& cols, ExecContext* ctx,
                        const std::vector<int>& assume_bits);

}
```

### include/comet_b200.h

```cpp
#ifndef COMET_B200_H
#define COMET_B200_H

#include <stddef.h>
#include <stdint.h>

#ifdef __cplusplus
extern "C" {
#endif

struct ArrowArray;
struct ArrowSchema;
struct ArrowArrayStream;

typedef struct cb200_plan cb200_plan;
typedef struct cb200_table cb200_table;

#define CB200_OK 0
#define CB200_ERR_UNSUPPORTED 1
#define CB200_ERR_CUDA 2
#define CB200_ERR_INPUT 3
#define CB200_ERR_PLAN 4
#define CB200_ERR_JIT 5
#define CB200_ERR_SPARK 10

typedef struct cb200_error {
    int32_t code;
    char error_class[64];
    char message[952];
} cb200_error;

const char* cb200_version(void);

int cb200_supports(const uint8_t* op_proto, size_t op_len, cb200_error* why);

cb200_plan* cb200_create_plan(const uint8_t* op_proto, size_t op_len, const uint8_t* cfg_proto, size_t cfg_len,
                              struct ArrowArrayStream** inputs, int32_t n_inputs, int32_t partition,
                              int32_t partition_count, int32_t batch_size, int32_t device_ordinal, cb200_error* err);

int32_t cb200_plan_num_columns(cb200_plan* plan);

int64_t cb200_execute(cb200_plan* plan, struct ArrowArray* out_arrays, struct ArrowSchema* out_schemas,
                      int32_t n_cols, cb200_error* err);

void cb200_release(cb200_plan* plan);

cb200_table* cb200_table_create(int64_t n_rows);
int cb200_table_add_column(cb200_table* t, int32_t type_id, int32_t precision, int32_t scale, int32_t value_width,
                           const void* dev_values, const void* dev_validity, int64_t null_count,
                           const char* const* dict_values, int32_t n_dict, cb200_error* err);
int cb200_table_add_column_bytes(cb200_table* t, int32_t type_id, int32_t precision, int32_t scale, int32_t value_width,
                                 const void* dev_values, const void* dev_validity_bytes, const char* const* dict_values,
                                 int32_t n_dict, cb200_error* err);
int cb200_plan_bind_table(cb200_plan* plan, int32_t input_index, cb200_table* t, cb200_error* err);
void cb200_table_release(cb200_table* t);

typedef struct cb200_device_column {
    int32_t type_id, precision, scale, value_width;
    const void* values;
    const void* validity;
    const void* host_values;
    const uint8_t* host_validity_bytes;
    const void* validity_bytes;
    const void* bool_bytes;
    int32_t n_dict;
    int32_t pad;
} cb200_device_column;
const char* cb200_plan_dict_value(cb200_plan* plan, int32_t col, int32_t i, int32_t* len);
int64_t cb200_execute_device(cb200_plan* plan, cb200_device_column* cols, int32_t n_cols, cb200_error* err);

int32_t cb200_plan_partition_starts(cb200_plan* plan, int64_t* starts, int32_t cap);

#define CB200_UNIQUE_ID_BYTES 128
typedef struct cb200_comm cb200_comm;
int cb200_comm_unique_id(uint8_t* id_out , cb200_error* err);
cb200_comm* cb200_comm_create(const uint8_t* id, int32_t rank, int32_t world, int32_t device_ordinal, cb200_error* err);
void cb200_comm_destroy(cb200_comm* comm);
int32_t cb200_comm_rank(cb200_comm* comm);
int32_t cb200_comm_world(cb200_comm* comm);
const char* cb200_nccl_info(void);

typedef struct cb200_exchange_stats {
    int64_t rows_sent, rows_received;
    int64_t bytes_sent, bytes_received;
    double payload_ms;
} cb200_exchange_stats;
cb200_table* cb200_exchange(cb200_comm* comm, cb200_plan* map_plan, int64_t* n_rows_out, cb200_exchange_stats* stats, cb200_error* err);
int64_t cb200_exchange_layout(const int64_t* counts, int32_t world, int32_t me, int64_t* recv_counts, int64_t* recv_offsets);
int cb200_comm_allgather_small(cb200_comm* comm, const void* payload, int64_t n_bytes, int64_t slot_bytes, void* out, int64_t* sizes_out,
                               cb200_error* err);

int64_t cb200_plan_kernel_launches(cb200_plan* plan);

int cb200_register_memory_file(const char* name, const void* data, size_t len);
int64_t cb200_snappy_decompress(const uint8_t* comp, size_t comp_len, uint8_t* out, size_t uncompressed_len, int32_t device_ordinal, int32_t* path_taken,
                                cb200_error* err);
int cb200_parquet_describe(const char* path, char* out, size_t cap, cb200_error* err);

typedef struct cb200_stats {
    int64_t kernel_launches;
    int64_t pipeline_launches;
    double pipeline_ms;
    int64_t pipeline_rows;
    int64_t h2d_bytes;
    int64_t d2h_bytes;
    int64_t scan_pruned_row_groups;
    int64_t scan_pruned_rows;
    int64_t agg_strategies;
} cb200_stats;
#define CB200_AGG_DENSE 1
#define CB200_AGG_TABLE 2
#define CB200_AGG_STREAM 4
#define CB200_AGG_MIGRATED 8
int cb200_plan_stats(cb200_plan* plan, cb200_stats* out);

int64_t cb200_release_cached_memory(int32_t device_ordinal);

int cb200_compile_plan(const uint8_t* op_proto, size_t op_len, char* keys_out, size_t keys_cap, cb200_error* err);
int cb200_compile_plan_assume(const uint8_t* op_proto, size_t op_len, const int32_t* assume_bits, int32_t n_assume,
                              int32_t source_index, char* src_out, size_t src_cap, cb200_error* err);
int cb200_plan_kernel_source(const uint8_t* op_proto, size_t op_len, int32_t index, char* out, size_t cap, cb200_error* err);

#ifdef __cplusplus
}
#endif
#endif
```

Baseline: 40.65 billion.

## Defer value-mask validation to device fold and remove per-launch host syncs

Moves the speculative value-mask check from a per-launch host round trip into the fold kernel, which records the first failing launch in a device flag. All chunk launches are issued back to back and the host reads the mask once at the end. Per-launch event timing now uses a pool of events instead of a sync before each kernel, and input staging goes through a pinned scratch area to skip intermediate syncs. Rows-per-thread is also widened when value bounds allow. The risks are extra work on the device when speculation fails and more complex rollback logic.

```diff
diff --git a/datafusion-comet_b200/comet_b200/native.py b/datafusion-comet_b200/comet_b200/native.py
--- a/datafusion-comet_b200/comet_b200/native.py
+++ b/datafusion-comet_b200/comet_b200/native.py
@@ -54,7 +54,8 @@
 class Stats(C.Structure):
     _fields_ = [("kernel_launches", C.c_int64), ("pipeline_launches", C.c_int64), ("pipeline_ms", C.c_double),
                 ("pipeline_rows", C.c_int64), ("h2d_bytes", C.c_int64), ("d2h_bytes", C.c_int64),
-                ("scan_pruned_row_groups", C.c_int64), ("scan_pruned_rows", C.c_int64), ("agg_strategies", C.c_int64)]
+                ("scan_pruned_row_groups", C.c_int64), ("scan_pruned_rows", C.c_int64), ("agg_strategies", C.c_int64),
+                ("host_syncs", C.c_int64)]
 AGG_DENSE, AGG_TABLE, AGG_STREAM, AGG_MIGRATED = 1, 2, 4, 8
 
 
diff --git a/datafusion-comet_b200/csrc/abi.cpp b/datafusion-comet_b200/csrc/abi.cpp
--- a/datafusion-comet_b200/csrc/abi.cpp
+++ b/datafusion-comet_b200/csrc/abi.cpp
@@ -20,7 +20,7 @@
     cudaStream_t stream;
     int* d_err;
     int* h_err;
-    cudaEvent_t ev0, ev1;
+    std::vector<cudaEvent_t> events;
 };
 std::mutex g_pool_mu;
 std::map<int, std::vector<CtxRes>> g_pool;
@@ -72,7 +72,7 @@
         if (!fl.empty()) {
             CtxRes r = fl.back();
             fl.pop_back();
-            ctx.stream = r.stream; ctx.d_err = r.d_err; ctx.h_err = r.h_err; ctx.ev0 = r.ev0; ctx.ev1 = r.ev1;
+            ctx.stream = r.stream; ctx.d_err = r.d_err; ctx.h_err = r.h_err; ctx.events = r.events;
         }
     }
     if (!ctx.stream) {
@@ -83,9 +83,7 @@
             cudaMemPoolSetAttribute(pool, cudaMemPoolAttrReleaseThreshold, &keep);
         }
         cuda_check(cudaMalloc((void**)&ctx.d_err, 64), "cudaMalloc err");
-        cuda_check(cudaMallocHost((void**)&ctx.h_err, 64), "cudaMallocHost err");
-        cuda_check(cudaEventCreate(&ctx.ev0), "cudaEventCreate");
-        cuda_check(cudaEventCreate(&ctx.ev1), "cudaEventCreate");
+        cuda_check(cudaMallocHost((void**)&ctx.h_err, ExecContext::H_PINNED_BYTES), "cudaMallocHost err");
     }
     cuda_check(cudaMemsetAsync(ctx.d_err, 0, 64, ctx.stream), "memset err");
     set_alloc_stream(ctx.stream);
@@ -214,7 +212,7 @@
         if (plan->ctx.stream) {
             cudaStreamSynchronize(plan->ctx.stream);
             std::lock_guard<std::mutex> lk(g_pool_mu);
-            g_pool[plan->ctx.device].push_back(CtxRes{plan->ctx.stream, plan->ctx.d_err, plan->ctx.h_err, plan->ctx.ev0, plan->ctx.ev1});
+            g_pool[plan->ctx.device].push_back(CtxRes{plan->ctx.stream, plan->ctx.d_err, plan->ctx.h_err, plan->ctx.events});
         }
         for (auto* s : plan->inputs.streams) if (s && s->release) s->release(s);
     } catch (...) {
@@ -344,6 +342,7 @@
     out->scan_pruned_row_groups = c.scan_pruned_row_groups;
     out->scan_pruned_rows = c.scan_pruned_rows;
     out->agg_strategies = c.agg_strategies;
+    out->host_syncs = c.host_syncs;
     return 0;
 }
 
diff --git a/datafusion-comet_b200/csrc/agg.cpp b/datafusion-comet_b200/csrc/agg.cpp
--- a/datafusion-comet_b200/csrc/agg.cpp
+++ b/datafusion-comet_b200/csrc/agg.cpp
@@ -22,7 +22,7 @@
 struct HashFlags { int w[CB_HFLAG_WORDS]; };
 int64_t round_ids(int64_t n) { return (n + GK - 1) / GK * GK; }
 
-using ValueMasks = uint64_t[CB_MAX_COLS * 2];
+constexpr size_t VMASK_BYTES = CB_MAX_COLS * 16, VMASK_BUF_BYTES = VMASK_BYTES + 16;
 
 uint64_t identity_word(int kind) { return kind == W_MIN ? 0x7fffffffffffffffull : kind == W_MAX ? 0x8000000000000000ull : 0; }
 
@@ -70,7 +70,7 @@
         }
         totals = std::make_shared<DeviceBuf>(newt.size() * 8);
         cuda_check(cudaMemcpyAsync(totals->ptr, newt.data(), newt.size() * 8, cudaMemcpyHostToDevice, ctx->stream), "regroup H2D");
-        cuda_check(cudaStreamSynchronize(ctx->stream), "regroup sync");
+        ctx->sync("regroup sync");
         groups = new_groups;
     }
 
@@ -157,13 +157,13 @@
     }
     void write_flags(ExecContext* ctx, const HashFlags& hf) {
         cuda_check(cudaMemcpyAsync(hflags->ptr, &hf, sizeof(hf), cudaMemcpyHostToDevice, ctx->stream), "write hash flags");
-        cuda_check(cudaStreamSynchronize(ctx->stream), "flags sync");
+        ctx->sync("flags sync");
     }
     int64_t read_flags(ExecContext* ctx, HashFlags& hf, int64_t cnt[GK]) {
         memset(&hf, 0, sizeof(hf));
         if (hflags) {
             cuda_check(cudaMemcpyAsync(&hf, hflags->ptr, sizeof(hf), cudaMemcpyDeviceToHost, ctx->stream), "read hash flags"); ctx->d2h_bytes += (int64_t)sizeof(hf);
-            cuda_check(cudaStreamSynchronize(ctx->stream), "hash flags sync");
+            ctx->sync("hash flags sync");
         }
         const int64_t R = max_groups / GK;
         int64_t total = 0;
@@ -212,7 +212,7 @@
             cuda_check(cudaMemcpyAsync(tp + (size_t)nm * n_words * 2, (cb::u64*)htotals->ptr + (size_t)max_groups * n_words * 2, (size_t)2 * n_words * 16,
                                        cudaMemcpyDeviceToDevice, st), "copy reserved groups");
         }
-        cuda_check(cudaStreamSynchronize(st), "table growth");
+        ctx->sync("table growth");
         htotals = ntot; hkey_of_gid = nkog; max_groups = nm;
     }
 
@@ -310,7 +310,7 @@
                 cb::u32 mask = (cb::u32)(cap - 1);
                 void* a2[] = {&kog, &rr, &ctr, &kp, &mask};
                 launch_named(ctx, k, "cb_hash_rehash", dim3((unsigned)((rows.max_groups + 255) / 256)), dim3(256), a2);
-                cuda_check(cudaStreamSynchronize(st), "rehash");
+                ctx->sync("rehash");
             }
             hkeys = nkeys; hcap = cap;
         }
@@ -438,13 +438,15 @@
     }
 
     void clear_vmask() {
-        if (!vmask) vmask = std::make_shared<DeviceBuf>(CB_MAX_COLS * 16);
-        cuda_check(cudaMemsetAsync(vmask->ptr, 0, CB_MAX_COLS * 16, ctx->stream), "memset vmask");
-    }
-    void copy_vmask(ValueMasks& masks) {
-        cuda_check(cudaMemcpyAsync(masks, vmask->ptr, sizeof(ValueMasks), cudaMemcpyDeviceToHost, ctx->stream), "read value masks"); ctx->d2h_bytes += (int64_t)(sizeof(ValueMasks));
-    }
-    static std::vector<int> mask_bits(const PipelineSpec& spec, const ValueMasks& masks) {
+        if (!vmask) vmask = std::make_shared<DeviceBuf>(VMASK_BUF_BYTES);
+        cuda_check(cudaMemsetAsync(vmask->ptr, 0, VMASK_BUF_BYTES, ctx->stream), "memset vmask");
+    }
+    const uint64_t* copy_vmask() {
+        cuda_check(cudaMemcpyAsync(ctx->h_scratch(), vmask->ptr, VMASK_BUF_BYTES, cudaMemcpyDeviceToHost, ctx->stream), "read value masks");
+        ctx->d2h_bytes += (int64_t)VMASK_BUF_BYTES;
+        return (const uint64_t*)ctx->h_scratch();
+    }
+    static std::vector<int> mask_bits(const PipelineSpec& spec, const uint64_t* masks) {
         std::vector<int> seen(spec.cols.size(), -1);
         for (size_t i = 0; i < spec.cols.size(); i++) {
             if (!spec.cols[i].type.is_decimal()) continue;
@@ -496,7 +498,7 @@
         ctx->kernel_launches += 2;
         int hdr[12];
         cuda_check(cudaMemcpyAsync(hdr, dd.d.n_codes, sizeof(hdr), cudaMemcpyDeviceToHost, ctx->stream), "dict header");
-        cuda_check(cudaStreamSynchronize(ctx->stream), "dict encode");
+        ctx->sync("dict encode");
         int n_codes = hdr[0], derr = hdr[8];
         if (derr & CB_DICT_FULL) throw Unsupported("plain Utf8 group key with more distinct values than the device dictionary holds (dictionary-encode the column)");
         if (derr & CB_DICT_COLLISION) throw ExecError(14, "", "64-bit hash collision between distinct group key strings");
@@ -603,20 +605,34 @@
                 TraceSpan ts("agg.codegen+jit");
                 k = compile(make_spec(&b, Strategy::Dense, n_groups, lv));
             }
-            const int64_t max_rows = (int64_t)ctx->num_sms * k.g.threads * (1ll << CB_RPT_LOG2) / 1024 * 1024;
-            int64_t r0 = row0;
-            while (r0 < row1 && launch_one(b, r0, std::min(row1, r0 + max_rows), n_groups, k)) r0 += max_rows;
-            if (r0 >= row1) return;
-            if (lv == SAFE) throw ExecError(15, "", "internal: value-mask validation failed without assumptions");
+            const int64_t max_rows = (int64_t)ctx->num_sms * k.g.threads * (1ll << k.g.rpt_log2) / 1024 * 1024;
+            clear_vmask();
+            std::vector<int64_t> starts;
+            for (int64_t r0 = row0; r0 < row1; r0 += max_rows) {
+                launch_one(b, r0, std::min(row1, r0 + max_rows), n_groups, k, (int)starts.size());
+                starts.push_back(r0);
+            }
+            const uint64_t* masks = copy_vmask();
+            ctx->check_device_errors();
+            observe(mask_bits(k.spec, masks));
+            const int failed = *(const int32_t*)((const char*)masks + VMASK_BYTES);
+            const size_t kept = failed > 0 ? (size_t)failed - 1 : starts.size();
+            if (kept > 0) {
+                rows_scanned += (kept < starts.size() ? starts[kept] : row1) - row0;
+                last = k;
+            }
+            if (failed == 0) return;
+            if (lv == SAFE || kept >= starts.size()) throw ExecError(15, "", "internal: value-mask validation failed without assumptions");
             lv = lv == TIGHT ? TYPE : SAFE;
-            row0 = r0;
-        }
-    }
-
-    bool launch_one(Batch& b, int64_t r0, int64_t r1, int n_groups, const Kernel& k) {
+            row0 = starts[kept];
+        }
+    }
+
+    void launch_one(Batch& b, int64_t r0, int64_t r1, int n_groups, const Kernel& k, int i) {
         cudaStream_t st = ctx->stream;
         size_t tot_bytes = (size_t)n_groups * n_words * 16;
-        if (!have_totals()) {
+        const bool first = !have_totals() && i == 0;
+        if (first) {
             dense.totals = std::make_shared<DeviceBuf>(tot_bytes);
             dense.groups = n_groups;
         }
@@ -624,7 +640,6 @@
             dense.spill = std::make_shared<DeviceBuf>(tot_bytes);
             cuda_check(cudaMemsetAsync(dense.spill->ptr, 0, dense.spill->bytes, st), "memset spill");
         }
-        clear_vmask();
         cb::PipeParams p;
         fill_inputs(p, b, k.g.tile, r0, r1);
         int grid = grid_for(ctx, p.n_tiles);
@@ -637,19 +652,6 @@
         p.vmask = (cb::u64*)vmask->ptr;
         launch(k.mod->kernel(k.g.entry), dim3(grid), dim3(k.g.threads + 32), k.g.dyn_smem(n_groups), &p);
         ctx->pipeline_rows += r1 - r0;
-        ValueMasks masks;
-        copy_vmask(masks);
-        ctx->check_device_errors();
-        const std::vector<int> seen = mask_bits(k.spec, masks);
-        bool ok = true;
-        for (size_t i = 0; i < seen.size(); i++)
-            if (k.spec.cols[i].assume_bits > 0 && seen[i] > k.spec.cols[i].assume_bits) ok = false;
-        observe(seen);
-        if (!ok) {
-            cuda_check(cudaMemsetAsync(dense.spill->ptr, 0, dense.spill->bytes, st), "memset spill");
-            return false;
-        }
-        rows_scanned += r1 - r0;
         cb::FinParams fp;
         memset(&fp, 0, sizeof(fp));
         fp.partials = (const cb::u64*)dense.partials->ptr;
@@ -657,14 +659,16 @@
         fp.totals = (cb::u64*)dense.totals->ptr;
         fp.n_ctas = grid;
         fp.n_groups = n_groups;
-        fp.first = have_totals() ? 0 : 1;
+        fp.first = first ? 1 : 0;
         fp.err = ctx->d_err;
+        fp.vmask = (const cb::u64*)vmask->ptr;
+        fp.spec_failed = (cb::i32*)((char*)vmask->ptr + VMASK_BYTES);
+        fp.launch_index = i;
+        for (size_t c = 0; c < k.spec.cols.size() && c < CB_MAX_COLS; c++) fp.assume_bits[c] = (cb::u8)k.spec.cols[c].assume_bits;
         int total_words = n_groups * n_words;
         void* args[] = {&fp};
         cuda_check(cudaLaunchKernel((const void*)k.mod->kernel("cb_fold"), dim3((total_words + 127) / 128), dim3(128), args, 0, st), "fold launch");
         ctx->kernel_launches++;
-        last = k;
-        return true;
     }
 
     void launch_id_rows(Batch& b, int64_t r0, int64_t r1, const Kernel& k, bool with_table) {
@@ -690,9 +694,8 @@
         }
         launch_id_rows(b, 0, b.n_rows, k, true);
         ctx->pipeline_rows += b.n_rows;
-        ValueMasks masks;
         int flags[8];
-        copy_vmask(masks);
+        const uint64_t* masks = copy_vmask();
         cuda_check(cudaMemcpyAsync(flags, rows.hflags->ptr, sizeof(flags), cudaMemcpyDeviceToHost, ctx->stream), "read hash flags"); ctx->d2h_bytes += (int64_t)(sizeof(flags));
         ctx->check_device_errors();
         if (flags[0] & CB_HF_FULL) throw ExecError(15, "", "internal: hash table full");
@@ -704,8 +707,7 @@
 
     int64_t stream_launch(Batch& b, int64_t r0, int64_t r1, const Kernel& k, HashFlags& hf, int64_t cnt[GK]) {
         launch_id_rows(b, r0, r1, k, false);
-        ValueMasks masks;
-        copy_vmask(masks);
+        const uint64_t* masks = copy_vmask();
         ctx->check_device_errors();
         const int64_t total = rows.read_flags(ctx, hf, cnt);
         if (hf.w[0] & CB_HF_WIDE_KEY) throw Unsupported("decimal(p > 18) group key whose value does not fit 64 bits");
@@ -797,7 +799,6 @@
         while (child->next(in)) {
             if (in.n_rows == 0) continue;
             consume(in);
-            ctx->check_device_errors();
         }
         emitted = true;
         if (!have_totals()) {
@@ -807,7 +808,7 @@
             for (int w = 0; w < n_words; w++) id[(size_t)w * 2] = identity_word(word_kinds[(size_t)w]);
             dense.totals = std::make_shared<DeviceBuf>(id.size() * 8);
             cuda_check(cudaMemcpyAsync(dense.totals->ptr, id.data(), id.size() * 8, cudaMemcpyHostToDevice, ctx->stream), "identity totals");
-            cuda_check(cudaStreamSynchronize(ctx->stream), "identity totals sync");
+            ctx->sync("identity totals sync");
             dense.groups = 1;
         }
         Batch result;
diff --git a/datafusion-comet_b200/csrc/codegen.cpp b/datafusion-comet_b200/csrc/codegen.cpp
--- a/datafusion-comet_b200/csrc/codegen.cpp
+++ b/datafusion-comet_b200/csrc/codegen.cpp
@@ -808,6 +808,7 @@
                 else if (op == "min") o << "acc.h_min(" << cond << ", " << ws << ", " << val << ");";
                 else o << "acc.h_max(" << cond << ", " << ws << ", " << val << ");";
             } else {
+                if (op == "wide" || op == "i128") g.rpt_log2 = std::min(g.rpt_log2, CB_ESCAPE_RPT_LOG2);
                 o << "if (" << cond << ") ";
                 if (op == "count") o << "acc.add_i64_wrap(g, " << ws << ", 1);";
                 else if (op == "wrap") o << "acc.add_i64_wrap(g, " << ws << ", " << val << ");";
@@ -962,9 +963,12 @@
                         if (first) {
                             u128r vb = em.bound_of(*a.children[0]);
                             if (spec.hash) upd(v.narrow ? "wide" : "i128", use, L.w_sum, v.v);
-                            else if (v.narrow && vb < (R63 >> CB_RPT_LOG2)) upd("wrap", use, L.w_sum, v.v);
-                            else if (v.narrow) upd("wide", use, L.w_sum, v.v);
-                            else upd("i128", use, L.w_sum, v.v);
+                            else if (v.narrow && vb < (R63 >> CB_RPT_LOG2)) {
+                                upd("wrap", use, L.w_sum, v.v);
+                                int k = CB_RPT_LOG2;
+                                while (k < g.rpt_log2 && vb < (R63 >> (k + 1))) k++;
+                                g.rpt_log2 = k;
+                            } else upd(v.narrow ? "wide" : "i128", use, L.w_sum, v.v);
                         }
                     } else if (f64) {
                         L.is_f64_sum = true;
diff --git a/datafusion-comet_b200/csrc/codegen.h b/datafusion-comet_b200/csrc/codegen.h
--- a/datafusion-comet_b200/csrc/codegen.h
+++ b/datafusion-comet_b200/csrc/codegen.h
@@ -19,6 +19,8 @@
 };
 
 #define CB_RPT_LOG2 14
+#define CB_ESCAPE_RPT_LOG2 17
+#define CB_MAX_RPT_LOG2 24
 
 enum class SinkKind { Select, Agg, Count };
 
@@ -62,6 +64,7 @@
     bool ungrouped = false;
     int n_key_cols = 0;
     int key_words = 1;
+    int rpt_log2 = CB_MAX_RPT_LOG2;
     size_t dyn_smem(int n_groups) const;
 };
 
diff --git a/datafusion-comet_b200/csrc/device/cb_kernels.cuh b/datafusion-comet_b200/csrc/device/cb_kernels.cuh
--- a/datafusion-comet_b200/csrc/device/cb_kernels.cuh
+++ b/datafusion-comet_b200/csrc/device/cb_kernels.cuh
@@ -655,6 +655,19 @@
     int w = idx % CB_WORDS;
     int kind = cb_word_kind(w);
     if (kind == 2) return;
+    if (fp.spec_failed) {
+        bool keep = *(volatile const i32*)fp.spec_failed == 0;
+        for (int c = 0; c < CB_MAX_COLS && keep; c++) {
+            if (!fp.assume_bits[c]) continue;
+            const u64 lo = fp.vmask[2 * c], hi = fp.vmask[2 * c + 1];
+            const int bits = hi ? 128 - __clzll((long long)hi) : 64 - __clzll((long long)lo);
+            if (bits > fp.assume_bits[c]) { keep = false; atomicCAS(fp.spec_failed, 0, fp.launch_index + 1); }
+        }
+        if (!keep) {
+            if (kind == 0) { fp.spill[idx * 2] = 0; fp.spill[idx * 2 + 1] = 0; }
+            return;
+        }
+    }
     u64 a, b;
     if (fp.first) { a = acc_identity(kind); b = 0; if (kind == 0) b = 0; }
     else { a = fp.totals[idx * 2]; b = fp.totals[idx * 2 + 1]; }
diff --git a/datafusion-comet_b200/csrc/device/cb_params.h b/datafusion-comet_b200/csrc/device/cb_params.h
--- a/datafusion-comet_b200/csrc/device/cb_params.h
+++ b/datafusion-comet_b200/csrc/device/cb_params.h
@@ -58,6 +58,10 @@
     i32 null_group_used;
     i32 gid_range;
     i32 gid_prefix[CB_GID_RANGES + 1];
+    const u64* vmask;
+    i32* spec_failed;
+    i32 launch_index;
+    u8 assume_bits[CB_MAX_COLS];
     u64 cert_b[CB_MAX_OUT][2];
 };
 
diff --git a/datafusion-comet_b200/csrc/exec.cpp b/datafusion-comet_b200/csrc/exec.cpp
--- a/datafusion-comet_b200/csrc/exec.cpp
+++ b/datafusion-comet_b200/csrc/exec.cpp
@@ -6,6 +6,7 @@
 #include <cstdlib>
 #include <ctime>
 #include <mutex>
+#include <unordered_map>
 
 namespace cb200 {
 
@@ -116,17 +117,32 @@
     cudaFreeAsync(ptr, stream);
 }
 
-void ExecContext::collect_timing() {
-    if (!ev_pending) return;
-    float ms = 0;
-    if (cudaEventElapsedTime(&ms, ev0, ev1) == cudaSuccess) { pipeline_ms += ms; pipeline_launches++; }
-    ev_pending = false;
+void ExecContext::record_pipeline_launch(cudaKernel_t k, dim3 grid, dim3 block, size_t smem, void** args) {
+    while (events.size() < events_used + 2) {
+        cudaEvent_t e;
+        cuda_check(cudaEventCreate(&e), "cudaEventCreate");
+        events.push_back(e);
+    }
+    cuda_check(cudaEventRecord(events[events_used], stream), "event record");
+    cuda_check(cudaLaunchKernel((const void*)k, grid, block, args, smem, stream), "kernel launch");
+    cuda_check(cudaEventRecord(events[events_used + 1], stream), "event record");
+    events_used += 2;
+    kernel_launches++;
+}
+
+void ExecContext::sync(const char* what) {
+    cuda_check(cudaStreamSynchronize(stream), what);
+    host_syncs++;
+    for (size_t i = 0; i + 1 < events_used; i += 2) {
+        float ms = 0;
+        if (cudaEventElapsedTime(&ms, events[i], events[i + 1]) == cudaSuccess) { pipeline_ms += ms; pipeline_launches++; }
+    }
+    events_used = 0;
 }
 
 void ExecContext::check_device_errors() {
     cuda_check(cudaMemcpyAsync(h_err, d_err, sizeof(int), cudaMemcpyDeviceToHost, stream), "error flag copy");
-    cuda_check(cudaStreamSynchronize(stream), "stream sync");
-    collect_timing();
+    sync("stream sync");
     int e = *h_err;
     if (!e) return;
     cudaMemsetAsync(d_err, 0, sizeof(int), stream);
@@ -244,7 +260,7 @@
             for (auto& x : arrs) if (x.release) x.release(&x);
             throw;
         }
-        cuda_check(cudaStreamSynchronize(ctx->stream), "H2D copies");
+        if (!all_staged) ctx->sync("H2D copies");
         for (auto& x : arrs) if (x.release) x.release(&x);
         return true;
     }
@@ -268,13 +284,37 @@
         return remap;
     }
 
+    static constexpr int64_t STAGED_MAX_ROWS = 4096;
+    std::vector<int> host_encoded;
+    std::vector<std::unordered_map<std::string, int32_t>> code_of;
+    bool encode_on_host(size_t c) {
+        if (host_encoded.empty()) { host_encoded.assign(schema.size(), -1); code_of.resize(schema.size()); }
+        if (host_encoded[c] < 0) host_encoded[c] = staging ? 1 : 0;
+        return host_encoded[c] == 1;
+    }
+    bool staging = false, all_staged = false;
+    size_t staged = 0;
+    void begin_upload(int64_t total) {
+        staging = all_staged = total <= STAGED_MAX_ROWS;
+        staged = 0;
+        if (staging && ctx->staging_epoch == ctx->host_syncs) ctx->sync("staging reuse");
+    }
     cudaError_t h2d(void* dst, const void* src, size_t n) {
         ctx->h2d_bytes += (int64_t)n;
+        if (staging && staged + n <= ExecContext::H_PINNED_BYTES - ExecContext::H_STAGING_OFF) {
+            char* h = ctx->h_staging() + staged;
+            memcpy(h, src, n);
+            staged = (staged + n + 15) / 16 * 16;
+            ctx->staging_epoch = ctx->host_syncs;
+            return cudaMemcpyAsync(dst, h, n, cudaMemcpyHostToDevice, ctx->stream);
+        }
+        all_staged = false;
         return cudaMemcpyAsync(dst, src, n, cudaMemcpyHostToDevice, ctx->stream);
     }
 
     void upload(std::vector<ArrowArray>& arrs, int64_t total, Batch& out) {
         TraceSpan ts("source.upload");
+        begin_upload(total);
         out.n_rows = total;
         out.cols.clear();
         out.cols.resize(schema.size());
@@ -324,11 +364,38 @@
                         auto dt = std::make_shared<DeviceBuf>(table.size() * 4 + 4);
                         temps.push_back(dt);
                         cuda_check(h2d(dt->ptr, table.data(), table.size() * 4), "H2D remap table");
-                        cuda_check(cudaStreamSynchronize(st), "remap table copy");
+                        if (!all_staged) ctx->sync("remap table copy");
                         launch_remap_codes(tmp->ptr, w, ch->length, (const int*)dt->ptr, (int)table.size(), (int*)col.data->ptr + row, st);
                     }
                     row += ch->length;
                 }
+            } else if (schema[c].is_string() && encode_on_host(c)) {
+                if (!dicts[c]) dicts[c] = std::make_shared<Dictionary>();
+                std::vector<int32_t> codes((size_t)total);
+                int64_t row = 0;
+                for (auto& a : arrs) {
+                    ArrowArray* ch = a.children[c];
+                    const int32_t* off = (const int32_t*)ch->buffers[1] + ch->offset;
+                    const uint8_t* vb = ch->null_count != 0 ? (const uint8_t*)ch->buffers[0] : nullptr;
+                    for (int64_t i = 0; i < ch->length; i++) {
+                        const int64_t bit = ch->offset + i;
+                        if (vb && !((vb[bit >> 3] >> (bit & 7)) & 1)) { codes[(size_t)(row + i)] = 0; continue; }
+                        std::string v((const char*)ch->buffers[2] + off[i], (size_t)(off[i + 1] - off[i]));
+                        auto it = code_of[c].find(v);
+                        if (it == code_of[c].end()) {
+                            it = code_of[c].emplace(v, (int32_t)dicts[c]->values.size()).first;
+                            dicts[c]->values.push_back(v);
+                        }
+                        codes[(size_t)(row + i)] = it->second;
+                    }
+                    row += ch->length;
+                }
+                col.is_dict = true;
+                col.dict = dicts[c];
+                col.phys = Phys::I32;
+                col.data = std::make_shared<DeviceBuf>((size_t)total * 4);
+                cuda_check(h2d(col.data->ptr, codes.data(), codes.size() * 4), "H2D string codes");
+                if (!all_staged) ctx->sync("string codes copy");
             } else if (schema[c].is_string()) {
                 int64_t total_chars = 0;
                 for (auto& a : arrs) {
@@ -353,7 +420,7 @@
                 }
                 offs[(size_t)total] = base;
                 cuda_check(h2d(col.offsets->ptr, offs.data(), offs.size() * 4), "H2D offsets");
-                cuda_check(cudaStreamSynchronize(st), "offsets copy");
+                if (!all_staged) ctx->sync("offsets copy");
                 col.phys = Phys::I32;
             } else {
                 col.phys = phys_of(schema[c]);
@@ -388,7 +455,7 @@
                 }
                 col.null_count = nulls;
             }
-            if (!temps.empty()) cuda_check(cudaStreamSynchronize(st), "temp buffers");
+            if (!temps.empty() && !all_staged) ctx->sync("temp buffers");
         }
     }
 
@@ -658,7 +725,7 @@
                     auto doff = std::make_shared<DeviceBuf>(off.size() * 4), dch = std::make_shared<DeviceBuf>(chars.size() + 16);
                     cuda_check(cudaMemcpyAsync(doff->ptr, off.data(), off.size() * 4, cudaMemcpyHostToDevice, st), "dict offsets");
                     if (!chars.empty()) cuda_check(cudaMemcpyAsync(dch->ptr, chars.data(), chars.size(), cudaMemcpyHostToDevice, st), "dict chars");
-                    cuda_check(cudaStreamSynchronize(st), "dict upload");
+                    ctx->sync("dict upload");
                     keep.push_back(doff); keep.push_back(dch);
                     k.dict_offsets = (const int*)doff->ptr;
                     k.dict_chars = (const unsigned char*)dch->ptr;
@@ -733,19 +800,19 @@
                 }
                 c.data = std::make_shared<DeviceBuf>(n * 4 + 16);
                 if (n) cuda_check(cudaMemcpyAsync(c.data->ptr, codes.data(), n * 4, cudaMemcpyHostToDevice, ctx->stream), "keys H2D");
-                cuda_check(cudaStreamSynchronize(ctx->stream), "keys H2D sync");
+                ctx->sync("keys H2D sync");
                 c.is_dict = true; c.dict = d; c.phys = Phys::I32;
             } else if (c.type.id == TypeId::Bool) {
                 std::vector<uint8_t> bits((n + 7) / 8 + 8, 0);
                 for (size_t r = 0; r < n; r++) if (c.h_data[r]) bits[r >> 3] |= (uint8_t)(1u << (r & 7));
                 c.data = std::make_shared<DeviceBuf>(bits.size());
                 cuda_check(cudaMemcpyAsync(c.data->ptr, bits.data(), bits.size(), cudaMemcpyHostToDevice, ctx->stream), "bool H2D");
-                cuda_check(cudaStreamSynchronize(ctx->stream), "bool H2D sync");
+                ctx->sync("bool H2D sync");
                 c.phys = Phys::Bitmap;
             } else {
                 c.data = std::make_shared<DeviceBuf>(c.h_data.size() + 16);
                 if (!c.h_data.empty()) cuda_check(cudaMemcpyAsync(c.data->ptr, c.h_data.data(), c.h_data.size(), cudaMemcpyHostToDevice, ctx->stream), "col H2D");
-                cuda_check(cudaStreamSynchronize(ctx->stream), "col H2D sync");
+                ctx->sync("col H2D sync");
                 c.phys = phys_of(c.type);
             }
             if (!c.h_valid.empty()) {
@@ -753,7 +820,7 @@
                 for (size_t r = 0; r < n; r++) if (c.h_valid[r]) bits[r >> 3] |= (uint8_t)(1u << (r & 7));
                 c.validity = std::make_shared<DeviceBuf>(bits.size());
                 cuda_check(cudaMemcpyAsync(c.validity->ptr, bits.data(), bits.size(), cudaMemcpyHostToDevice, ctx->stream), "validity H2D");
-                cuda_check(cudaStreamSynchronize(ctx->stream), "validity H2D sync");
+                ctx->sync("validity H2D sync");
             }
             c.on_host = false;
         }
@@ -904,7 +971,7 @@
     std::vector<uint8_t> raw(nbytes + 9, 0);
     if (n) {
         cuda_check(cudaMemcpyAsync(raw.data(), (const uint8_t*)dev_bitmap + first, nbytes, cudaMemcpyDeviceToHost, ctx->stream), "D2H validity");
-        cuda_check(cudaStreamSynchronize(ctx->stream), "D2H sync");
+        ctx->sync("D2H sync");
         ctx->d2h_bytes += (int64_t)nbytes;
     }
     if (shift == 0) { raw.resize((n + 7) / 8 + 8); return raw; }
@@ -944,7 +1011,7 @@
         } else if (c.is_dict) {
             std::vector<int32_t> codes(n + 1);
             if (n) cuda_check(cudaMemcpyAsync(codes.data(), (const uint8_t*)c.data->ptr + r0 * 4, n * 4, cudaMemcpyDeviceToHost, ctx->stream), "D2H key codes");
-            cuda_check(cudaStreamSynchronize(ctx->stream), "D2H sync");
+            ctx->sync("D2H sync");
             ctx->d2h_bytes += (int64_t)n * 4;
             std::vector<uint8_t> vb = c.validity && n ? fetch_bits(ctx, c.validity->ptr, row0, n) : std::vector<uint8_t>((n + 7) / 8 + 8, 0xff);
             offs.resize((n + 1) * 4);
@@ -964,7 +1031,7 @@
             std::vector<uint8_t> raw(n * (size_t)w + 8);
             if (n) cuda_check(cudaMemcpyAsync(raw.data(), (const uint8_t*)c.data->ptr + r0 * (size_t)w, n * (size_t)w, cudaMemcpyDeviceToHost, ctx->stream), "D2H output");
             ctx->d2h_bytes += (int64_t)(n * (size_t)w);
-            cuda_check(cudaStreamSynchronize(ctx->stream), "D2H sync");
+            ctx->sync("D2H sync");
             if (c.validity) {
                 validity = fetch_bits(ctx, c.validity->ptr, row0, n);
                 for (size_t r = 0; r < n; r++) null_count += ((validity[r >> 3] >> (r & 7)) & 1) ? 0 : 1;
diff --git a/datafusion-comet_b200/csrc/exec.h b/datafusion-comet_b200/csrc/exec.h
--- a/datafusion-comet_b200/csrc/exec.h
+++ b/datafusion-comet_b200/csrc/exec.h
@@ -82,9 +82,14 @@
     int batch_size = 8192;
     int* d_err = nullptr;
     int* h_err = nullptr;
+    static constexpr size_t H_SCRATCH_OFF = 256, H_STAGING_OFF = 4096, H_PINNED_BYTES = 64 << 10;
+    void* h_scratch() const { return (char*)h_err + H_SCRATCH_OFF; }
+    char* h_staging() const { return (char*)h_err + H_STAGING_OFF; }
+    int64_t staging_epoch = -1;
     int64_t kernel_launches = 0;
-    cudaEvent_t ev0 = nullptr, ev1 = nullptr;
-    bool ev_pending = false;
+    std::vector<cudaEvent_t> events;
+    size_t events_used = 0;
+    int64_t host_syncs = 0;
     double pipeline_ms = 0;
     int64_t pipeline_launches = 0;
     int64_t pipeline_rows = 0;
@@ -92,8 +97,9 @@
     int64_t scan_pruned_row_groups = 0, scan_pruned_rows = 0;
     int64_t agg_strategies = 0;
     std::vector<int64_t> partition_starts;
+    void sync(const char* what);
     void check_device_errors();
-    void collect_timing();
+    void record_pipeline_launch(cudaKernel_t k, dim3 grid, dim3 block, size_t smem, void** args);
 };
 
 struct ExecNode {
diff --git a/datafusion-comet_b200/csrc/exec_internal.h b/datafusion-comet_b200/csrc/exec_internal.h
--- a/datafusion-comet_b200/csrc/exec_internal.h
+++ b/datafusion-comet_b200/csrc/exec_internal.h
@@ -113,12 +113,7 @@
     void launch(cudaKernel_t k, dim3 grid, dim3 block, size_t smem, void* params) {
         cuda_check(cudaFuncSetAttribute((const void*)k, cudaFuncAttributeMaxDynamicSharedMemorySize, (int)smem), "cudaFuncSetAttribute(smem)");
         void* args[] = {params};
-        if (ctx->ev_pending) { cuda_check(cudaStreamSynchronize(ctx->stream), "stream sync"); ctx->collect_timing(); }
-        cuda_check(cudaEventRecord(ctx->ev0, ctx->stream), "event record");
-        cuda_check(cudaLaunchKernel((const void*)k, grid, block, args, smem, ctx->stream), "kernel launch");
-        cuda_check(cudaEventRecord(ctx->ev1, ctx->stream), "event record");
-        ctx->ev_pending = true;
-        ctx->kernel_launches++;
+        ctx->record_pipeline_launch(k, grid, block, smem, args);
     }
 };
 
diff --git a/include/comet_b200.h b/include/comet_b200.h
--- a/include/comet_b200.h
+++ b/include/comet_b200.h
@@ -106,6 +106,7 @@
     int64_t scan_pruned_row_groups;
     int64_t scan_pruned_rows;
     int64_t agg_strategies;
+    int64_t host_syncs;
 } cb200_stats;
 #define CB200_AGG_DENSE 1
 #define CB200_AGG_TABLE 2
```

New measurement: 41.98 billion (median of 6 runs). +3.3%, better.
